# GATB/dsk

Measured on AMD Instinct MI355X. Metric: distinct k-mers counted/sec (whole node), k=31, higher is better.
Workload: dtype u64

## Files before the change

dsk_amd/csrc/dskgpu.hip:

```cpp
#include <algorithm>
#include <cstdio>
#include <cstring>
#include <cstdlib>
#include <cmath>
#include <string>
#include <vector>

#include <thread>
#include <system_error>
#include "engine.h"
#include "kernels.h"
#include "superkmer.h"
#include "rawparse.h"

#include <rocprim/device/device_radix_sort.hpp>

#define DSKGPU_VERSION "dskgpu 0.1 (gfx950)"

namespace {

thread_local std::string g_create_err;

__global__ __launch_bounds__(1024) void k_place_probe(unsigned long long* __restrict__ out, unsigned long long n) {
    const unsigned long long per_block = n / gridDim.x, per_stream = per_block / 512;
    unsigned long long* base = out + (unsigned long long)blockIdx.x * per_block;
    const int r = threadIdx.x >> 5, l = threadIdx.x & 31;
    for (unsigned long long off = 0; off + 32 <= per_stream; off += 32)
        for (int p = r; p < 512; p += 32) base[(unsigned long long)p * per_stream + off + l] = off;
}
int g_place_k = -1;
float place_probe_ms(void* p, size_t bytes) {
    hipEvent_t a, b;
    if (hipEventCreate(&a) != hipSuccess || hipEventCreate(&b) != hipSuccess) return 0.f;
    float best = 1e30f;
    for (int i = 0; i < 3; ++i) {
        (void)hipEventRecord(a, 0);
        hipLaunchKernelGGL(k_place_probe, dim3(256), dim3(1024), 0, 0, static_cast<unsigned long long*>(p), (unsigned long long)(bytes / 8));
        (void)hipEventRecord(b, 0);
        (void)hipEventSynchronize(b);
        float ms = 0.f; (void)hipEventElapsedTime(&ms, a, b);
        if (i && ms < best) best = ms;
    }
    (void)hipEventDestroy(a); (void)hipEventDestroy(b);
    return best;
}
}

hipError_t placed_malloc(void** out, size_t bytes) {
    if (g_place_k < 0) { const char* e = getenv("DSKGPU_PLACE"); g_place_k = e ? atoi(e) : 0; }
    size_t free_b = 0, total_b = 0;
    if (g_place_k < 2 || bytes < (size_t(1) << 28) || hipMemGetInfo(&free_b, &total_b) != hipSuccess) return hipMalloc(out, bytes);
    const int K = (int)std::min<size_t>((size_t)g_place_k, free_b / 2 / bytes);
    if (K < 2) return hipMalloc(out, bytes);
    std::vector<void*> cand; std::vector<float> ms;
    for (int i = 0; i < K; ++i) {
        void* q = nullptr;
        if (hipMalloc(&q, bytes) != hipSuccess) { (void)hipGetLastError(); break; }
        static const size_t probe_max = getenv("DSKGPU_PLACE_GB") ? (size_t)(atof(getenv("DSKGPU_PLACE_GB")) * (1ull << 30)) : ~size_t(0);
        cand.push_back(q); ms.push_back(place_probe_ms(q, std::min(bytes, probe_max)));
    }
    if (cand.empty()) return hipErrorOutOfMemory;
    size_t best = 0;
    for (size_t i = 1; i < cand.size(); ++i) if (ms[i] < ms[best]) best = i;
    for (size_t i = 0; i < cand.size(); ++i) if (i != best) (void)hipFree(cand[i]);
    if (getenv("DSKGPU_VERBOSE")) {
        fprintf(stderr, "[dskgpu] placement of %.2f GB: probe ms", bytes * 1e-9);
        for (size_t i = 0; i < cand.size(); ++i) fprintf(stderr, " %.3f%s", ms[i], i == best ? "*" : "");
        fprintf(stderr, "\n");
    }
    *out = cand[best];
    return hipSuccess;
}

namespace {

__global__ void k_gather_back(const u32* __restrict__ sc, const u32* __restrict__ nsolid_total, const u32* __restrict__ nk, const u64* __restrict__ gstats,
                              u64* __restrict__ out) {
    if (threadIdx.x == 0) {
        out[0] = sc[SC_OVERFLOW]; out[1] = *nsolid_total; out[2] = nk ? *nk : 0u; out[3] = sc[SC_OVF2]; out[4] = sc[SC_OVF1]; out[5] = sc[SC_EXT];
        out[6] = gstats[0]; out[7] = gstats[1]; out[8] = gstats[2]; out[9] = gstats[3];
    }
}
struct ScalarSet { u32 v[SC_COUNT]; };
__global__ __launch_bounds__(256) void k_setup_pass(u32* __restrict__ sc, ScalarSet h, u64* __restrict__ ghist, u32 nh, u64* __restrict__ gstats, u32 nstats,
                                                    u32* __restrict__ zero, u64 nzero) {
    const u32 t = blockIdx.x * 256 + threadIdx.x;
    if (t < SC_COUNT) sc[t] = h.v[t];
    if (t < nstats) gstats[t] = 0ull;
    for (u32 i = t; i < nh; i += gridDim.x * 256) ghist[i] = 0ull;
    for (u64 i = t; i < nzero; i += (u64)gridDim.x * 256) zero[i] = 0u;
}
}

namespace {

#define LAND_BYTES (64u << 10)
void* landing(dskgpu_ctx* ctx, size_t bytes) {
    if (bytes > LAND_BYTES) return nullptr;
    if (!ctx->land && hipHostMalloc(reinterpret_cast<void**>(&ctx->land), LAND_BYTES, hipHostMallocDefault) != hipSuccess) { ctx->land = nullptr; (void)hipGetLastError(); }
    return ctx->land;
}

bool sentinel_is_a_kmer(int W, unsigned k) {
    u64 v[4] = {0, 0, 0, 0};
    if (W == 1) v[0] = kunmix(~0ull);
    else if (W == 2) { KN<2> x; x.w[0] = x.w[1] = ~0ull; kunmixN(x); v[0] = x.w[0]; v[1] = x.w[1]; }
    else { KN<4> x; for (int i = 0; i < 4; ++i) x.w[i] = ~0ull; kunmixN(x); for (int i = 0; i < 4; ++i) v[i] = x.w[i]; }
    auto base = [&](const u64* a, unsigned i) { return (unsigned)((a[i >> 5] >> (2 * (i & 31))) & 3u); };
    for (unsigned i = k; i < 128; ++i) if (base(v, i)) return false;
    u64 r[4] = {0, 0, 0, 0};
    for (unsigned i = 0; i < k; ++i) { const unsigned c = base(v, i) ^ 2u, j = k - 1 - i; r[j >> 5] |= (u64)c << (2 * (j & 31)); }
    for (int x = 3; x >= 0; --x) if (v[x] != r[x]) return v[x] < r[x];
    return true;
}


int run_encode(dskgpu_ctx* ctx, const uint8_t* d_bytes, u64 n, u64* nwords_out) {
    const u64 nwords = (n + 31) / 32;
    ctx->enc_fresh = false;
    CK(ctx->packed.ensure((nwords + 1) * 8));
    CK(ctx->inval.ensure((nwords + 1) * 4));
    if (const int rc = encode_into(ctx, d_bytes, n, ctx->packed.as<u64>(), ctx->inval.as<u32>())) return rc;
    *nwords_out = nwords;
    return DSKGPU_OK;
}

int encode_current(dskgpu_ctx* ctx, u64* nwords_out) {
    if (ctx->enc_keep) { *nwords_out = (ctx->n_bytes + 31) / 32; ctx->enc_fresh = false; return DSKGPU_OK; }
    if (!ctx->d_reads && ctx->n_bytes) return fail(ctx, DSKGPU_E_STATE, "the reads were released (dskgpu_encode_reads) and their 2-bit form has been overwritten: set the reads again");
    return run_encode(ctx, ctx->d_reads, ctx->n_bytes, nwords_out);
}

}

int encode_into(dskgpu_ctx* ctx, const uint8_t* d_bytes, u64 n, u64* packed, u32* inval) {
    const u64 nwords = (n + 31) / 32;
    if (!nwords) return DSKGPU_OK;
    const u64 nb = (nwords + 255) / 256;
    const unsigned grid = (unsigned)std::min<u64>(nb, (u64)ctx->num_cu * 16);
    if ((reinterpret_cast<uintptr_t>(d_bytes) & 15) == 0)
        hipLaunchKernelGGL(k_encode<true>, dim3(grid), dim3(256), 0, ctx->stream, d_bytes, n, packed, inval, nwords);
    else
        hipLaunchKernelGGL(k_encode<false>, dim3(grid), dim3(256), 0, ctx->stream, d_bytes, n, packed, inval, nwords);
    CKL("k_encode");
    return DSKGPU_OK;
}

int run_scan(dskgpu_ctx* ctx, u32* a, const u32* d_len, u64 max_len) {
    const u64 nb = std::max<u64>(1, (max_len + SCAN_BLK - 1) / SCAN_BLK);
    CK(ctx->sums.ensure((nb + 1) * 4));
    hipLaunchKernelGGL(k_scan_reduce, dim3((unsigned)nb), dim3(SCAN_NT), 0, ctx->stream, a, d_len, ctx->sums.as<u32>());
    hipLaunchKernelGGL(k_scan_sums, dim3(1), dim3(1024), 0, ctx->stream, ctx->sums.as<u32>(), d_len, a);
    hipLaunchKernelGGL(k_scan_apply, dim3((unsigned)nb), dim3(SCAN_NT), 0, ctx->stream, a, d_len, ctx->sums.as<u32>());
    CKL("k_scan");
    return DSKGPU_OK;
}

int allow_big_lds(dskgpu_ctx* ctx, const void* fn, int bytes) {
    for (const void* f : ctx->big_lds_fns) if (f == fn) return DSKGPU_OK;
    CK(hipFuncSetAttribute(fn, hipFuncAttributeMaxDynamicSharedMemorySize, bytes));
    ctx->big_lds_fns.push_back(fn);
    return DSKGPU_OK;
}

namespace {

size_t scatter_lds(int W, u32 P, bool opt = false) { return (size_t)SC_NT * (16 / W) * 8 * W + (size_t)P * (opt ? 20 : 16) + 4 + 17 * 4 + 16 + (opt ? 8 + L0_MAX_PASSES * 8 : 0); }

template <int W, int SRC, int MODE>
int launch_hist_m(dskgpu_ctx* ctx, const typename KeyT<W>::T* keys, const ChunkDesc* descs, const u32* d_nch,
                  u64 max_chunks, u32* matrix, DigitSpec ds, u32 P) {
    const unsigned grid = (unsigned)std::max<u64>(1, std::min<u64>(max_chunks, (u64)ctx->num_cu));
    hipLaunchKernelGGL((k_hist<W, SRC, MODE>), dim3(grid), dim3(SC_NT), 0, ctx->stream, ctx->packed.as<u64>(),
                       ctx->inval.as<u32>(), keys, descs, d_nch, matrix, (int)ctx->cfg.kmer_size, ds, P);
    CKL("k_hist");
    return DSKGPU_OK;
}
template <int W, int SRC>
int launch_hist(dskgpu_ctx* ctx, const typename KeyT<W>::T* keys, const ChunkDesc* descs, const u32* d_nch,
                u64 max_chunks, u32* matrix, DigitSpec ds, u32 P) {
    const bool mp = ds.mode == 1 && ds.npass > 1;
    if (SRC == 0) return ds.mode == 0 ? launch_hist_m<W, 0, 0>(ctx, keys, descs, d_nch, max_chunks, matrix, ds, P)
                       : mp ? launch_hist_m<W, 0, 3>(ctx, keys, descs, d_nch, max_chunks, matrix, ds, P)
                            : launch_hist_m<W, 0, 1>(ctx, keys, descs, d_nch, max_chunks, matrix, ds, P);
    return ds.mode == 2 ? launch_hist_m<W, 1, 2>(ctx, keys, descs, d_nch, max_chunks, matrix, ds, P)
                   : mp ? launch_hist_m<W, 1, 3>(ctx, keys, descs, d_nch, max_chunks, matrix, ds, P)
                        : launch_hist_m<W, 1, 1>(ctx, keys, descs, d_nch, max_chunks, matrix, ds, P);
}

unsigned scatter_grid(const dskgpu_ctx* ctx, int W, u32 P, u64 max_chunks, bool opt = false) {
    const size_t lds = scatter_lds(W, P, opt);
    const u64 per_cu = std::max<u64>(1, std::min<u64>(2048 / SC_NT, (160 * 1024) / lds));
    return (unsigned)std::max<u64>(1, std::min<u64>(max_chunks, (u64)ctx->num_cu * per_cu));
}
template <int W, int SRC, int MODE, bool OPT = false, bool HEAVY = false>
int launch_scatter_m(dskgpu_ctx* ctx, const typename KeyT<W>::T* keys, const ChunkDesc* descs, const u32* d_nch,
                     u64 max_chunks, const u32* scanned, typename KeyT<W>::T* out, DigitSpec ds, u32 P, Opt1Spec o1 = Opt1Spec{nullptr, 0u, 0u, nullptr, nullptr, 0u, nullptr, nullptr, nullptr, 0u, nullptr, 0ull, {0ull, 0ull, 0ull, 0ull}, 0u}) {
    const size_t lds = scatter_lds(W, P, OPT && !o1.uslice);
    const unsigned grid = scatter_grid(ctx, W, P, max_chunks, OPT && !o1.uslice);
    { const int e = allow_big_lds(ctx, reinterpret_cast<const void*>(&k_scatter<W, SRC, MODE, OPT, HEAVY>)); if (e) return e; }
    hipLaunchKernelGGL((k_scatter<W, SRC, MODE, OPT, HEAVY>), dim3(grid), dim3(SC_NT), lds, ctx->stream, SRC == 2 ? ctx->rec_src : ctx->packed.as<u64>(),
                       SRC == 2 ? nullptr : ctx->inval.as<u32>(), keys, descs, d_nch, scanned, out, (int)ctx->cfg.kmer_size, ds, P, o1);
    CKL("k_scatter");
    return DSKGPU_OK;
}
template <int W, int MODE, bool OPT = false, bool SLICED = false>
int launch_scatter_al(dskgpu_ctx* ctx, const typename KeyT<W>::T* keys, const ChunkDesc* descs, const u32* d_nch,
                      u64 max_chunks, const u32* scanned, typename KeyT<W>::T* out, DigitSpec ds, u32 P, OptSpec os = OptSpec{0u, nullptr, nullptr, nullptr, 0u, 0u, 0ull, 0u, 0u, nullptr, nullptr, nullptr, nullptr, nullptr, nullptr}) {
    const size_t lds = ascatter_lds(W, P);
    const unsigned grid = (unsigned)std::max<u64>(1, std::min<u64>(max_chunks, (u64)ctx->num_cu));
    { const int e = allow_big_lds(ctx, reinterpret_cast<const void*>(&k_scatter_al<W, MODE, OPT, SLICED>)); if (e) return e; }
    hipLaunchKernelGGL((k_scatter_al<W, MODE, OPT, SLICED>), dim3(grid), dim3(SC_NT), lds, ctx->stream, keys, descs, d_nch, scanned, out, ds, P, os);
    CKL("k_scatter_al");
    return DSKGPU_OK;
}

template <int W, int SRC>
int launch_scatter(dskgpu_ctx* ctx, const typename KeyT<W>::T* keys, const ChunkDesc* descs, const u32* d_nch,
                   u64 max_chunks, const u32* scanned, typename KeyT<W>::T* out, DigitSpec ds, u32 P) {
    const bool mp = ds.mode == 1 && ds.npass > 1;
    if (SRC == 1 && ascatter_lds(W, P) <= 160 * 1024 && !ctx->tune.no_aligned)
        return ds.mode == 2 ? launch_scatter_al<W, 2>(ctx, keys, descs, d_nch, max_chunks, scanned, out, ds, P)
                       : mp ? launch_scatter_al<W, 3>(ctx, keys, descs, d_nch, max_chunks, scanned, out, ds, P)
                            : launch_scatter_al<W, 1>(ctx, keys, descs, d_nch, max_chunks, scanned, out, ds, P);
    if (SRC == 0) return ds.mode == 0 ? launch_scatter_m<W, 0, 0>(ctx, keys, descs, d_nch, max_chunks, scanned, out, ds, P)
                       : mp ? launch_scatter_m<W, 0, 3>(ctx, keys, descs, d_nch, max_chunks, scanned, out, ds, P)
                            : launch_scatter_m<W, 0, 1>(ctx, keys, descs, d_nch, max_chunks, scanned, out, ds, P);
    return ds.mode == 2 ? launch_scatter_m<W, 1, 2>(ctx, keys, descs, d_nch, max_chunks, scanned, out, ds, P)
                   : mp ? launch_scatter_m<W, 1, 3>(ctx, keys, descs, d_nch, max_chunks, scanned, out, ds, P)
                        : launch_scatter_m<W, 1, 1>(ctx, keys, descs, d_nch, max_chunks, scanned, out, ds, P);
}

inline void launch_count_impl(dskgpu_ctx* ctx, unsigned grid, u64* keys, u64* solid_keys, u32* solid_ab, u32* ovf, const CountParams& cp) {
    if (cp.cap && cp.cap <= CNT_V3_KEYS * CNT_NT) {
        hipLaunchKernelGGL((k_count1v3<CNT_NT, CNT_KPT, CNT_V3_KEYS>), dim3(grid), dim3(CNT_NT), 0, ctx->stream, keys, solid_keys, solid_ab,
                           ctx->nsolid.as<u32>(), ctx->ghist.as<u64>(), ctx->gstats.as<u64>(), ovf, cp, cp.subcnt);
        return;
    }
    if (cp.cap) hipLaunchKernelGGL(k_count1<true>, dim3(grid), dim3(CNT_NT), 0, ctx->stream, keys, solid_keys, ctx->fstart.as<u32>(), solid_ab,
                                   ctx->nsolid.as<u32>(), ctx->ghist.as<u64>(), ctx->gstats.as<u64>(), ovf, cp, cp.subcnt);
    else hipLaunchKernelGGL(k_count1<false>, dim3(grid), dim3(CNT_NT), 0, ctx->stream, keys, solid_keys, ctx->fstart.as<u32>(), solid_ab,
                            ctx->nsolid.as<u32>(), ctx->ghist.as<u64>(), ctx->gstats.as<u64>(), ovf, cp, (const u32*)ctx->fstart.as<u32>());
}
template <int W>
inline void launch_count_impl(dskgpu_ctx* ctx, unsigned grid, KN<W>* keys, KN<W>* solid_keys, u32* solid_ab, u32* ovf, const CountParams& cp) {
    if constexpr (W == 2) {
        if (cp.cap && cp.cap <= C2V_NKEYS * CNT_NT && !ctx->mw_v3_off) {
            CountParams c2 = cp; c2.maxload = std::min<u32>(cp.maxload, C2V_MAXLOAD);
            hipLaunchKernelGGL((k_count2v3<CNT_NT, C2V_KPT, C2V_NKEYS>), dim3(grid), dim3(CNT_NT), 0, ctx->stream, (const K2*)keys, solid_keys, solid_ab,
                               ctx->nsolid.as<u32>(), ctx->ghist.as<u64>(), ctx->gstats.as<u64>(), ovf, c2, cp.subcnt);
            return;
        }
    }
    if (cp.cap) hipLaunchKernelGGL((k_count_mw<W, true>), dim3(grid), dim3(CNT_NT), 0, ctx->stream, keys, solid_keys, ctx->fstart.as<u32>(), solid_ab,
                                   ctx->nsolid.as<u32>(), ctx->ghist.as<u64>(), ctx->gstats.as<u64>(), ovf, cp);
    else hipLaunchKernelGGL((k_count_mw<W, false>), dim3(grid), dim3(CNT_NT), 0, ctx->stream, keys, solid_keys, ctx->fstart.as<u32>(), solid_ab,
                            ctx->nsolid.as<u32>(), ctx->ghist.as<u64>(), ctx->gstats.as<u64>(), ovf, cp);
}
template <int W>
inline void launch_count(dskgpu_ctx* ctx, unsigned grid, typename KeyT<W>::T* keys, typename KeyT<W>::T* solid_keys, u32* solid_ab, u32* ovf, const CountParams& cp) {
    launch_count_impl(ctx, grid, keys, solid_keys, solid_ab, ovf, cp);
}

struct Plan {
    int levels;
    u32 P1, P2, F;
    DigitSpec d1, d2;
};

#define TARGET_KEYS 2900
#define TARGET_KEYS2 2560
#ifndef TARGET_KEYS4
#define TARGET_KEYS4 640
#endif
#ifndef OPT_GROUPS4
#define OPT_GROUPS4 OPT_GROUPS
#endif
#define MAX_LEVEL_BINS 2048
#define ONE_LEVEL_BINS 1024
#define CH2 65536u
#define OPT_GROUPS 545u
#define OPT_GROUPS2 1023u
inline u32 opt_groups(int W) { return W == 2 ? (AL_G2 == 8 ? 1022u : OPT_GROUPS2) : (W == 1 && AL_G1 == 16) ? 546u : W == 4 ? OPT_GROUPS4 : OPT_GROUPS; }
inline u64 target_keys(int W) { return W == 1 ? TARGET_KEYS : W == 2 ? TARGET_KEYS2 : TARGET_KEYS4; }
#define OPT_CAP 4360u

bool make_plan(u64 n_upper, int extra_bits, int W, u32 num_cu, Plan* pl) {
    const u64 target = target_keys(W);
    u64 F = ((n_upper + target - 1) / target) << extra_bits;
    if (F < 2) F = 2;
    if (F <= ONE_LEVEL_BINS) { pl->levels = 1; pl->P1 = (u32)F; pl->P2 = 1; }
    else {
        u64 p2max = MAX_LEVEL_BINS; while (p2max > 64 && ascatter_lds(W, (u32)p2max) > 160 * 1024) --p2max;
        u64 p1 = 1; while (p1 * p1 < F) ++p1;
        const bool large = F >= (u64)num_cu * 64;
        if (large) {
            p1 = std::max<u64>((F + p2max - 2) / (p2max - 1), num_cu);
            p1 = (p1 + num_cu - 1) / num_cu * num_cu;
            if (p1 > MAX_LEVEL_BINS - 8) p1 = MAX_LEVEL_BINS - 8;
        }
        u64 p2 = (F + p1 - 1) / p1;
        if (p2 % 2 == 0 && p2 + 1 <= p2max) ++p2;
        if (p1 > MAX_LEVEL_BINS || p2 > MAX_LEVEL_BINS) return false;
        pl->levels = 2; pl->P1 = (u32)p1; pl->P2 = (u32)p2;
    }
    pl->F = pl->P1 * pl->P2;
    pl->d1 = DigitSpec{1u, pl->P1, 0u, 1u, 1u, 0u};
    pl->d2 = DigitSpec{2u, pl->P1, pl->P2, 1u, 1u, 0u};
    return true;
}

void build_descs1(dskgpu_ctx* ctx, u64 n_units_total, u64 tile, u64 max_chunks, u32* nch_out) {
    const u64 ntiles = std::max<u64>(1, (n_units_total + tile - 1) / tile);
    u64 nch = std::min<u64>(ntiles, max_chunks);
    const u64 tpc = (ntiles + nch - 1) / nch;
    nch = (ntiles + tpc - 1) / tpc;
    ctx->h_descs1.resize(nch);
    for (u64 c = 0; c < nch; ++c) {
        ChunkDesc d;
        d.begin = c * tpc * tile;
        d.end = std::min<u64>(n_units_total, (c + 1) * tpc * tile);
        if (d.begin > d.end) d.begin = d.end;
        d.flat_base = (u32)c;
        d.stride = (u32)nch;
        ctx->h_descs1[c] = d;
    }
    *nch_out = (u32)nch;
}

void build_descs1_slices(dskgpu_ctx* ctx, u64 tile, u64 max_chunks, u32* nch_out) {
    const size_t S = ctx->rec_slice_end.size();
    ctx->h_descs1.clear(); ctx->h_slice_chunk.assign(S + 1, 0);
    const u64 per_slice = std::max<u64>(1, max_chunks / S);
    u64 rb = 0;
    for (size_t sl = 0; sl < S; ++sl) {
        const u64 re = ctx->rec_slice_end[sl];
        ctx->h_slice_chunk[sl] = (u32)ctx->h_descs1.size();
        if (re > rb) {
            const u64 ntiles = (re - rb + tile - 1) / tile;
            u64 nch = std::min<u64>(ntiles, per_slice);
            const u64 tpc = (ntiles + nch - 1) / nch;
            nch = (ntiles + tpc - 1) / tpc;
            for (u64 c = 0; c < nch; ++c) {
                ChunkDesc d;
                d.begin = rb + c * tpc * tile; d.end = std::min<u64>(re, rb + (c + 1) * tpc * tile);
                d.flat_base = 0; d.stride = 0;
                ctx->h_descs1.push_back(d);
            }
        }
        rb = re;
    }
    ctx->h_slice_chunk[S] = (u32)ctx->h_descs1.size();
    for (auto& d : ctx->h_descs1) d.stride = (u32)ctx->h_descs1.size();
    *nch_out = (u32)ctx->h_descs1.size();
}

#define REC_RESIZE 1001
int rec_gate_upto(dskgpu_ctx* ctx, u32 upto) {
    if (!ctx->rec_gate) return DSKGPU_OK;
    const u32 n = (u32)ctx->rec_slice_end.size();
    for (; ctx->rec_gated < std::min(upto, n); ++ctx->rec_gated)
        if (ctx->rec_gate(ctx->rec_gate_user, ctx->rec_gated) != 0) ctx->rec_gate_failed = true;
    return ctx->rec_gate_failed ? fail(ctx, DSKGPU_E_STATE, "a slice of the exchange did not arrive (the caller's gate failed)") : DSKGPU_OK;
}
int rec_gate_all(dskgpu_ctx* ctx) { return rec_gate_upto(ctx, 0xFFFFFFFFu); }

int sk_sizes(dskgpu_ctx* ctx, u64* total_out) {
    const u64 nrec = ctx->rec_n; const u32 R = ctx->sk_sp.R;
    { const int e = rec_gate_all(ctx); if (e) return e; }
    u64 nch = std::min<u64>((nrec + SKX_NT - 1) / SKX_NT, (u64)ctx->num_cu * 16);
    u64 rpc = (nrec + nch - 1) / nch;
    rpc = (rpc + SKX_NT - 1) / SKX_NT * SKX_NT;
    nch = (nrec + rpc - 1) / rpc;
    if (rpc * SK_MAXN >= 0xFFFFFFFFull) return fail(ctx, DSKGPU_E_ARG, "too many records per chunk");
    CK(ctx->sk_sums.ensure(nch * 4)); CK(ctx->sk_cbase.ensure(nch * 8));
    ctx->h_sk_sums.assign(nch, 0); ctx->h_sk_cbase.assign(nch, 0);
    hipLaunchKernelGGL(k_sk_count, dim3((unsigned)nch), dim3(SKX_NT), 0, ctx->stream, ctx->rec_src, nrec, R, (u32)rpc, ctx->sk_sums.as<u32>());
    CKL("k_sk_count");
    CK(hipMemcpyAsync(ctx->h_sk_sums.data(), ctx->sk_sums.p, nch * 4, hipMemcpyDeviceToHost, ctx->stream));
    CK(hipStreamSynchronize(ctx->stream));
    u64 total = 0;
    for (u64 c = 0; c < nch; ++c) { ctx->h_sk_cbase[c] = total; total += ctx->h_sk_sums[c]; }
    CK(hipMemcpyAsync(ctx->sk_cbase.p, ctx->h_sk_cbase.data(), nch * 8, hipMemcpyHostToDevice, ctx->stream));
    ctx->rec_nch = nch; ctx->rec_rpc = rpc; ctx->rec_sized = true;
    *total_out = total;
    return DSKGPU_OK;
}

template <int W>
int expand_records(dskgpu_ctx* ctx, u64 total) {
    typedef typename KeyT<W>::T Key;
    if (ctx->rec_expanded) return DSKGPU_OK;
    if (!ctx->rec_sized) {
        u64 real = 0;
        const int e = sk_sizes(ctx, &real);
        if (e) return e;
        if (real != total && ctx->rec_hint_est) { ctx->rec_hint = real; return REC_RESIZE; }
        if (real != total) return fail(ctx, DSKGPU_E_ARG, "dskgpu_mg_count_sized: n_kmers does not match the k-mers inside the records");
    }
    { const int e = rec_gate_all(ctx); if (e) return e; }
    CK(ctx->sk_keys.ensure((total + 1) * sizeof(Key)));
    hipLaunchKernelGGL(k_sk_expand<W>, dim3((unsigned)ctx->rec_nch), dim3(SKX_NT), 0, ctx->stream, ctx->rec_src, ctx->rec_n, ctx->sk_sp.R,
                       (int)ctx->cfg.kmer_size, (u32)ctx->rec_rpc, ctx->sk_cbase.as<u64>(), ctx->sk_keys.as<Key>());
    CKL("k_sk_expand");
    ctx->rec_expanded = true;
    ctx->mark("mg_expand");
    return DSKGPU_OK;
}
template <> int expand_records<4>(dskgpu_ctx*, u64) { return DSKGPU_E_STATE; }

template <int W> struct HvLayout { static constexpr size_t keys = 0, counts = (size_t)HV_KEYS * W, rows = (size_t)HV_KEYS * (W + 1), ab = (size_t)HV_KEYS * (2 * W + 1), words = (size_t)HV_KEYS * (2 * W + 2); };
template <int W>
int find_heavy(dskgpu_ctx* ctx, bool from_reads, const typename KeyT<W>::T* d_keys_in, u32 nts, const Plan& pl, std::vector<double>& load, u32* nheavy_out) {
    typedef typename KeyT<W>::T Key;
    struct HK { u64 w[W]; bool operator<(const HK& o) const { for (int x = W - 1; x >= 0; --x) if (w[x] != o.w[x]) return w[x] < o.w[x]; return false; }
                bool operator==(const HK& o) const { for (int x = 0; x < W; ++x) if (w[x] != o.w[x]) return false; return true; } };
    static_assert(sizeof(HK) == sizeof(Key), "host mirror of a device key");
    *nheavy_out = 0;
    const u32 P1 = pl.P1;
    std::vector<double> sorted(load);
    std::nth_element(sorted.begin(), sorted.begin() + P1 / 2, sorted.end());
    const double median = sorted[P1 / 2];
    std::vector<u32> flagged;
    for (u32 b = 0; b < P1; ++b) if (load[b] > 1.2 * median + 4096.0) flagged.push_back(b);
    if (ctx->tune.verbose) fprintf(stderr, "[dskgpu] find_heavy: median load %.0f, %zu bins above 1.2 x\n", median, flagged.size());
    if (flagged.empty()) return DSKGPU_OK;
    std::sort(flagged.begin(), flagged.end(), [&](u32 a, u32 b) { return load[a] > load[b]; });
    if (flagged.size() > HV_SLOTS) flagged.resize(HV_SLOTS);
    ctx->h_hv_lut.assign(P1, 0xFF);
    for (size_t f = 0; f < flagged.size(); ++f) ctx->h_hv_lut[flagged[f]] = (unsigned char)f;
    const size_t nf = flagged.size();
    CK(ctx->hv_lut.ensure(P1));
    const unsigned grid = (unsigned)std::min<u64>(nts, (u64)ctx->num_cu * 2);
    const size_t per_slot = (size_t)grid * HV_BLOCK_KEYS;
    CK(ctx->hv_collect.ensure((size_t)HV_SLOTS * per_slot * sizeof(Key) + (size_t)HV_SLOTS * grid * 4 + HV_SLOTS * 4));
    u32* d_kept = reinterpret_cast<u32*>(ctx->hv_collect.as<Key>() + (size_t)HV_SLOTS * per_slot);
    u32* d_step = d_kept + (size_t)HV_SLOTS * grid;
    ctx->h_hv_step.assign(HV_SLOTS, 1);
    for (size_t f = 0; f < flagged.size(); ++f) ctx->h_hv_step[f] = (u32)std::max<u64>(1, ctx->h_mom[2 * (size_t)flagged[f]] / HV_COLLECT);
    CK(hipMemcpyAsync(ctx->hv_lut.p, ctx->h_hv_lut.data(), P1, hipMemcpyHostToDevice, ctx->stream));
    CK(hipMemcpyAsync(d_step, ctx->h_hv_step.data(), HV_SLOTS * 4, hipMemcpyHostToDevice, ctx->stream));
    u32* sc = ctx->scalars.as<u32>();
    const bool mp = pl.d1.npass > 1;
    auto launch = [&](auto kern) {
        hipLaunchKernelGGL(kern, dim3(grid), dim3(SC_NT), 0, ctx->stream, (const u64*)ctx->packed.as<u64>(), (const u32*)ctx->inval.as<u32>(), d_keys_in,
                           (const ChunkDesc*)ctx->smp_descs.as<ChunkDesc>(), (const u32*)(sc + SC_NCH_S), (int)ctx->cfg.kmer_size, pl.d1, P1,
                           (const unsigned char*)ctx->hv_lut.as<unsigned char>(), d_kept, ctx->hv_collect.as<Key>(), (const u32*)d_step);
    };
    if (from_reads) { if (mp) launch(k_collect_heavy<W, 0, 3>); else launch(k_collect_heavy<W, 0, 1>); }
    else { if (mp) launch(k_collect_heavy<W, 1, 3>); else launch(k_collect_heavy<W, 1, 1>); }
    CKL("k_collect_heavy");
    ctx->h_hv_cnt.resize(nf * grid);
    ctx->h_hv_coll.resize(nf * per_slot * W);
    CK(hipMemcpyAsync(ctx->h_hv_cnt.data(), d_kept, nf * grid * 4, hipMemcpyDeviceToHost, ctx->stream));
    CK(hipMemcpyAsync(ctx->h_hv_coll.data(), ctx->hv_collect.p, nf * per_slot * sizeof(Key), hipMemcpyDeviceToHost, ctx->stream));
    CK(hipStreamSynchronize(ctx->stream));
    struct Cand { double est; HK key; u32 bin; };
    std::vector<Cand> cands;
    for (size_t f = 0; f < nf; ++f) {
        HK* kk = reinterpret_cast<HK*>(ctx->h_hv_coll.data()) + f * per_slot;
        u32 n = 0;
        for (unsigned g = 0; g < grid; ++g) {
            const u32 c = std::min<u32>(ctx->h_hv_cnt[f * grid + g], HV_BLOCK_KEYS);
            for (u32 i = 0; i < c; ++i) kk[n++] = kk[(size_t)g * HV_BLOCK_KEYS + i];
        }
        if (n < 256) continue;
        std::sort(kk, kk + n);
        const u32 bin = flagged[f];
        u32 found = 0;
        for (u32 i = 0; i < n;) {
            u32 j = i + 1;
            while (j < n && kk[j] == kk[i]) ++j;
            if ((u64)(j - i) * 20 >= n) { cands.push_back({load[bin] * (double)(j - i) / (double)n, kk[i], bin}); ++found; }
            i = j;
        }
        if (ctx->tune.verbose) fprintf(stderr, "[dskgpu]   bin %u load %.0f: %u keys collected, %u dominant\n", bin, load[bin], n, found);
    }
    std::sort(cands.begin(), cands.end(), [](const Cand& a, const Cand& b) { return a.est > b.est; });
    if (cands.size() > HV_KEYS) cands.resize(HV_KEYS);
    ctx->h_hv_keys.assign((size_t)HV_KEYS * W, DSK_EMPTY);
    for (size_t x = 0; x < cands.size(); ++x) {
        for (int y = 0; y < W; ++y) ctx->h_hv_keys[x * W + y] = cands[x].key.w[y];
        load[cands[x].bin] -= cands[x].est;
    }
    u32 nheavy = (u32)cands.size();
    if (nheavy) {
        CK(ctx->hv_buf.ensure(HvLayout<W>::words * 8));
        u64* hvb = ctx->hv_buf.as<u64>();
        CK(hipMemsetAsync(hvb + HvLayout<W>::keys, 0xFF, (size_t)HV_KEYS * W * 8, ctx->stream));
        CK(hipMemsetAsync(hvb + HvLayout<W>::counts, 0, HV_KEYS * 8, ctx->stream));
        CK(hipMemcpyAsync(hvb + HvLayout<W>::keys, ctx->h_hv_keys.data(), (size_t)HV_KEYS * W * 8, hipMemcpyHostToDevice, ctx->stream));
    }
    *nheavy_out = nheavy;
    return DSKGPU_OK;
}

template <int W> struct KeySource { bool from_reads, from_rec; const typename KeyT<W>::T* keys; u64 nkeys, nwords; };

template <int W>
struct PassState {
    typedef typename KeyT<W>::T Key;
    KeySource<W>& src;
    u32 pass, npass; u64 cap;
    u64 nvalid;
    u32* sc;
    Plan pl{};
    u32 opt_cap = 0, max_ext = 0; u64 nregions = 0;
    bool opt1 = false; Opt1Spec o1{}; unsigned grid1 = 0;
    u32 nch1 = 0, nheavy = 0;
    std::vector<double> load, spread;
    Key* fkeys = nullptr;
    DevBuf* scratch = nullptr;
    Key* solid_keys = nullptr; u32* solid_ab = nullptr;
    u32 flags = 0, nsolid = 0, nkeys = 0, ovf2 = 0, ovf1 = 0, ext = 0; u64 stats[4] = {0, 0, 0, 0};
    bool too_big = false; u64 rows = 0;
};

template <int W>
int upload_descs1(dskgpu_ctx* ctx, PassState<W>& ps) {
    const KeySource<W>& src = ps.src;
    const u64 max_chunks1 = (u64)ctx->num_cu * 8;
    if (src.from_reads) build_descs1(ctx, src.nwords, Tile<W>::WORDS, max_chunks1, &ps.nch1);
    else if (src.from_rec && ctx->rec_slice_end.size() > 1) build_descs1_slices(ctx, RecTile<W>::NR, max_chunks1, &ps.nch1);
    else if (src.from_rec) build_descs1(ctx, ctx->rec_n, RecTile<W>::NR, max_chunks1, &ps.nch1);
    else build_descs1(ctx, src.nkeys, Tile<W>::KEYS, max_chunks1, &ps.nch1);
    CK(ctx->descs1.ensure(ctx->h_descs1.size() * sizeof(ChunkDesc)));
    CK(hipMemcpyAsync(ctx->descs1.p, ctx->h_descs1.data(), ctx->h_descs1.size() * sizeof(ChunkDesc), hipMemcpyHostToDevice, ctx->stream));
    return DSKGPU_OK;
}

template <int W>
int records_to_keys(dskgpu_ctx* ctx, PassState<W>& ps) {
    const int e = expand_records<W>(ctx, ps.src.nkeys);
    if (e) return e;
    ps.src.keys = ctx->sk_keys.template as<typename KeyT<W>::T>(); ps.src.from_rec = false;
    return upload_descs1(ctx, ps);
}

template <class Hist>
int positional_sample(dskgpu_ctx* ctx, u64 units, u64 tile, u32 P, Hist&& hist, u64* ntiles_out, u64* nts_out, u64* stot_out) {
    u32* sc = ctx->scalars.as<u32>();
    const u64 ntiles = std::max<u64>(1, (units + tile - 1) / tile);
    const u64 nts = std::min<u64>(ntiles, 1024);
    ctx->h_descs_s.resize(nts);
    for (u64 i = 0; i < nts; ++i) {
        const u64 t = i * ntiles / nts;
        ChunkDesc d; d.begin = t * tile; d.end = std::min<u64>(units, (t + 1) * tile); d.flat_base = (u32)i; d.stride = (u32)nts;
        ctx->h_descs_s[i] = d;
    }
    const u64 Ms = (u64)P * nts;
    CK(ctx->smp_descs.ensure(nts * sizeof(ChunkDesc)));
    CK(ctx->smp_mat.ensure((Ms + 4) * 4 + (size_t)P * 16));
    CK(hipMemcpyAsync(ctx->smp_descs.p, ctx->h_descs_s.data(), nts * sizeof(ChunkDesc), hipMemcpyHostToDevice, ctx->stream));
    ctx->h_sc[SC_NCH_S] = (u32)nts;
    CK(hipMemcpyAsync(sc + SC_NCH_S, &ctx->h_sc[SC_NCH_S], 4, hipMemcpyHostToDevice, ctx->stream));
    { const int e = hist(ctx->smp_descs.as<ChunkDesc>(), (const u32*)(sc + SC_NCH_S), nts, ctx->smp_mat.as<u32>()); if (e) return e; }
    u64* mom = reinterpret_cast<u64*>(ctx->smp_mat.as<u32>() + ((Ms + 2) & ~(u64)1));
    hipLaunchKernelGGL(k_bin_moments, dim3((P + 3) / 4), dim3(256), 0, ctx->stream, (const u32*)ctx->smp_mat.as<u32>(), (u32)nts, P, mom);
    CKL("k_bin_moments");
    ctx->h_mom.resize((size_t)P * 2);
    void* lz = landing(ctx, (size_t)P * 16);
    CK(hipMemcpyAsync(lz ? lz : (void*)ctx->h_mom.data(), mom, (size_t)P * 16, hipMemcpyDeviceToHost, ctx->stream));
    CK(hipStreamSynchronize(ctx->stream));
    if (lz) std::memcpy(ctx->h_mom.data(), lz, (size_t)P * 16);
    u64 stot = 0;
    for (u32 b = 0; b < P; ++b) stot += ctx->h_mom[2 * b];
    *ntiles_out = ntiles; *nts_out = nts; *stot_out = stot;
    return DSKGPU_OK;
}

template <int W>
int pass_plan(dskgpu_ctx* ctx, PassState<W>& ps, int extra_bits) {
    typedef typename KeyT<W>::T Key;
    Plan& pl = ps.pl;
    const u64 plan_n = (ps.src.from_reads && ctx->have_nvalid) ? std::min<u64>(ps.cap, ps.npass == 1 ? ps.nvalid + 1 : ps.nvalid / ps.npass + ps.nvalid / ps.npass / 50 + 4096) : ps.cap;
    if (!make_plan(plan_n, extra_bits, W, (u32)ctx->num_cu, &pl))
        return fail(ctx, DSKGPU_E_OVERFLOW, "cannot partition finer (table overflow persists)");
    pl.d1.world = pl.d2.world = ctx->cfg.world_size; pl.d1.npass = pl.d2.npass = ps.npass; pl.d1.pass = pl.d2.pass = ps.pass;
    { const int e = upload_descs1(ctx, ps); if (e) return e; }
    if (pl.levels == 2 && ctx->sentinel_ok && !ctx->opt2_off && !ctx->tune.no_opt2 && ascatter_lds(W, pl.P2) <= 160 * 1024)
        ps.opt_cap = opt_groups(W) * (8u / W);
    if (ps.opt_cap && ctx->tune.opt_cap) ps.opt_cap = ctx->tune.opt_cap;
    if (W > 1 && (u64)pl.F * ps.opt_cap >= 0xFFFF0000ull) ps.opt_cap = 0;
    const u32 opt_cap = ps.opt_cap;
    if (opt_cap && W <= 2) {
        u64 want = std::min<u64>((u64)pl.F / 8 + 4096, 0x7FFFFFFFull / opt_cap - 1);
        if (ctx->tune.max_ext >= 0) want = (u64)ctx->tune.max_ext;
        if (W > 1) { const u64 room = 0xFFFF0000ull / opt_cap; want = room > (u64)pl.F + 1 ? std::min<u64>(want, room - pl.F - 1) : 0; }
        ps.max_ext = (u32)want;
    }
    ps.nregions = (u64)pl.F + ps.max_ext;
    if (!opt_cap) { CK(ctx->bufA.ensure((ps.cap + 1) * sizeof(Key))); CK(ctx->bufB.ensure((ps.cap + 1) * sizeof(Key))); }
    if (opt_cap) {
        const u64 slots = (u64)pl.F * opt_cap + ATile<W>::KEYS + 16;
        CK(ctx->bufA.ensure(std::max<u64>(W == 1 ? slots * 4 : slots * sizeof(Key), (ps.cap + 1) * sizeof(Key))));
        if (W > 1) CK(ctx->abund2.ensure(slots * 4));
    }
    ps.opt1 = opt_cap && !ctx->opt1_off && !ctx->tune.no_opt1 && (ps.npass == 1 || ps.src.from_reads || W <= 2);
    if (ps.src.from_rec && (!ps.opt1 || W > 2 || ctx->tune.no_recsrc)) { const int e = records_to_keys(ctx, ps); if (e) return e; }
    if (ps.opt1 && scatter_lds(W, pl.P1, false) > 160 * 1024) ps.opt1 = false;
    return DSKGPU_OK;
}

template <int W>
int pass_layout1(dskgpu_ctx* ctx, PassState<W>& ps) {
    typedef typename KeyT<W>::T Key;
    const KeySource<W>& src = ps.src;
    const Plan& pl = ps.pl;
    Opt1Spec& o1 = ps.o1;
    o1 = Opt1Spec{nullptr, 0u, 0u, ps.sc + SC_OVF1, nullptr, ctx->sk_sp.R, ctx->gstats.as<u64>() + 2, nullptr, nullptr, 0u, nullptr, 0ull, {0ull, 0ull, 0ull, 0ull}, 0u};
    const bool uniform1 = scatter_lds(W, pl.P1, true) > 160 * 1024;
    if (ps.opt1) {
        const u32 nch1 = ps.nch1;
        const unsigned grid1 = ps.grid1 = scatter_grid(ctx, W, pl.P1, nch1, !uniform1);
        const u64 cpb = (nch1 + grid1 - 1) / grid1;
        double share = (double)cpb / (double)nch1;
        if (src.from_rec && ctx->rec_slice_end.size() > 1) {
            share = 0.0;
            u64 rb = 0;
            for (size_t sl = 0; sl < ctx->rec_slice_end.size(); ++sl) {
                const u64 re = ctx->rec_slice_end[sl], nc = ctx->h_slice_chunk[sl + 1] - ctx->h_slice_chunk[sl];
                if (nc) share += (double)((nc + grid1 - 1) / grid1) / (double)nc * (double)(re - rb) / (double)ctx->rec_n;
                rb = re;
            }
        }
        const double pass_keys = (double)(ps.nvalid / ps.npass);
        ps.load.assign(pl.P1, pass_keys / pl.P1);
        ps.spread.assign(pl.P1, 0.0);
        bool sampled = false;
        const Key* d_keys_s = src.keys;
        double smp_density = 1.0;
        bool rec_sample_ok = ctx->sentinel_ok;
        u64 rec_units = 0;
        if constexpr (W <= 2) {
          if (src.from_rec && !ctx->tune.no_sample && !uniform1) {
            const u64 nrec_s = ctx->rec_slice_end.size() > 1 ? ctx->rec_slice_end[0] : ctx->rec_n;
            const u64 NR = RecTile<W>::NR;
            const u64 nchk_all = (nrec_s + NR - 1) / NR;
            const u64 nchk = std::min<u64>(nchk_all, 256);
            if (nchk == 0) rec_sample_ok = false;
            else {
                { const int e = rec_gate_upto(ctx, 1); if (e) return e; }
                std::vector<u64>& cbeg = ctx->h_cbeg;
                cbeg.resize(nchk);
                for (u64 i = 0; i < nchk; ++i) cbeg[i] = (i * nchk_all / nchk) * NR;
                rec_units = nchk * NR * SK_MAXN;
                CK(ctx->smp_keys.ensure(rec_units * sizeof(Key) + nchk * 8 + 64));
                u64* d_cbeg = reinterpret_cast<u64*>(ctx->smp_keys.as<char>() + rec_units * sizeof(Key));
                CK(hipMemcpyAsync(d_cbeg, cbeg.data(), nchk * 8, hipMemcpyHostToDevice, ctx->stream));
                hipLaunchKernelGGL(k_sk_sample_keys<W>, dim3((unsigned)nchk), dim3(SKX_NT), 0, ctx->stream, ctx->rec_src, ctx->rec_n, ctx->sk_sp.R, (int)ctx->cfg.kmer_size,
                                   (const u64*)d_cbeg, (u32)NR, ctx->smp_keys.as<Key>());
                CKL("k_sk_sample_keys");
                d_keys_s = ctx->smp_keys.as<Key>();
            }
          }
        }
        const bool smp_rec = src.from_rec && rec_units != 0;
        if ((!src.from_rec || smp_rec) && rec_sample_ok && !ctx->tune.no_sample && !uniform1) {
            const u64 units = src.from_reads ? src.nwords : smp_rec ? rec_units : src.nkeys, tile = src.from_reads ? Tile<W>::WORDS : Tile<W>::KEYS;
            auto hist = [&](const ChunkDesc* dd, const u32* d_nch, u64 n, u32* mat) {
                return src.from_reads ? launch_hist<W, 0>(ctx, nullptr, dd, d_nch, n, mat, pl.d1, pl.P1) : launch_hist<W, 1>(ctx, d_keys_s, dd, d_nch, n, mat, pl.d1, pl.P1);
            };
            u64 ntiles = 0, nts = 0, stot = 0;
            { const int e = positional_sample(ctx, units, tile, pl.P1, hist, &ntiles, &nts, &stot); if (e) return e; }
            if (stot >= (u64)pl.P1 * 64) {
                const double scale = (src.from_reads && ps.npass > 1) ? (double)ntiles / (double)nts : pass_keys / (double)stot;
                if (smp_rec) smp_density = std::max(0.05, (double)stot / ((double)nts * (double)Tile<W>::KEYS));
                const double tiles_per_block = smp_rec ? pass_keys * share / (double)Tile<W>::KEYS : (double)ntiles * share;
                for (u32 b = 0; b < pl.P1; ++b) {
                    const double sum = (double)ctx->h_mom[2 * b], sq = (double)ctx->h_mom[2 * b + 1];
                    const double mean = sum / (double)nts, var = std::max(mean, sq / (double)nts - mean * mean);
                    ps.load[b] = sum * scale;
                    ps.spread[b] = 5.0 * std::sqrt(tiles_per_block * var / smp_density) + 4.0 * std::sqrt((double)nts * var) * scale * share;
                }
                sampled = true;
            }
            if constexpr (W <= 2) {
                if (sampled && ps.opt_cap && !ctx->tune.no_heavy) { const int e = find_heavy<W>(ctx, src.from_reads, d_keys_s, (u32)nts, pl, ps.load, &ps.nheavy); if (e) return e; }
            }
            ctx->mark("sample1");
        }
        ctx->h_boff.resize(pl.P1 + 1);
        u64 area = 0;
        if (uniform1) o1.uslice = 1u;
        for (u32 b = 0; b < pl.P1; ++b) {
            double sl = ps.load[b] * share;
            const double few = (src.from_rec && share * (double)nch1 < 16.0) ? 0.08 : 0.0;
            sl += sampled ? ps.spread[b] + sl * 0.01 + 64.0 : sl * (0.06 + few) + 160.0;
            u64 slice = ((u64)sl + 8) & ~7ull;
            if (uniform1) o1.uslice = (u32)slice;
            if (ctx->tune.opt_slice) slice = ctx->tune.opt_slice;
            ctx->h_boff[b] = (u32)std::min<u64>(area, 0xFFFFFFFFull); area += slice;
        }
        ctx->h_boff[pl.P1] = (u32)std::min<u64>(area, 0xFFFFFFFFull);
        const u64 tail = 2 * Tile<W>::KEYS;
        const u64 cells = (u64)pl.P1 * grid1;
        if (ctx->tune.verbose) fprintf(stderr, "[dskgpu] pass %u/%u: P1 %u P2 %u, %u level-1 blocks, area %llu keys per block (%.2f GB of slices), sampled %d, keys %llu, %u chunks, share %.6f, %zu slices\n", ps.pass, ps.npass, pl.P1, pl.P2, grid1,
                                       (unsigned long long)area, (double)area * grid1 * sizeof(Key) * 1e-9, (int)sampled, (unsigned long long)ps.nvalid, nch1, share, ctx->rec_slice_end.size());
        if (area < 8 || area * grid1 + tail >= 0xFFFF0000ull) ps.opt1 = false;
        else {
            o1.area = (u32)area; o1.dump = (u32)(area * grid1);
            CK(ctx->boff.ensure(((size_t)pl.P1 + 1) * 4));
            CK(hipMemcpyAsync(ctx->boff.p, ctx->h_boff.data(), ((size_t)pl.P1 + 1) * 4, hipMemcpyHostToDevice, ctx->stream));
            o1.boff = ctx->boff.as<u32>();
            CK(ctx->mat1.ensure((cells + 1) * 4));
            o1.fill = ctx->mat1.as<u32>();
            if (grid1 + 1 > SLICED_MAX) ps.opt1 = false;
            CK(ctx->bufA.ensure((area * grid1 + tail + 1) * sizeof(Key)));
        }
    }
    if (src.from_rec && !ps.opt1) { const int e = records_to_keys(ctx, ps); if (e) return e; }
    return DSKGPU_OK;
}

template <int W, int SRC, int MODE, bool HEAVY>
int scatter1_m(dskgpu_ctx* ctx, const PassState<W>& ps, const ChunkDesc* dd1, const u32* d_nch) {
    return launch_scatter_m<W, SRC, MODE, true, HEAVY>(ctx, SRC == 1 ? ps.src.keys : nullptr, dd1, d_nch, ps.nch1, nullptr, ctx->bufA.template as<typename KeyT<W>::T>(),
                                                       ps.pl.d1, ps.pl.P1, ps.o1);
}
template <int W>
int launch_scatter1(dskgpu_ctx* ctx, const PassState<W>& ps, const ChunkDesc* dd1, const u32* d_nch) {
    const bool mp = ps.npass > 1, heavy = ps.nheavy != 0, rec = ps.src.from_rec, reads = ps.src.from_reads;
    if constexpr (W <= 2) {
        if (rec && heavy) return mp ? scatter1_m<W, 2, 3, true>(ctx, ps, dd1, d_nch) : scatter1_m<W, 2, 1, true>(ctx, ps, dd1, d_nch);
        if (rec) return mp ? scatter1_m<W, 2, 3, false>(ctx, ps, dd1, d_nch) : scatter1_m<W, 2, 1, false>(ctx, ps, dd1, d_nch);
        if (heavy && reads) return mp ? scatter1_m<W, 0, 3, true>(ctx, ps, dd1, d_nch) : scatter1_m<W, 0, 1, true>(ctx, ps, dd1, d_nch);
        if (heavy) return mp ? scatter1_m<W, 1, 3, true>(ctx, ps, dd1, d_nch) : scatter1_m<W, 1, 1, true>(ctx, ps, dd1, d_nch);
        if (!reads && mp) return scatter1_m<W, 1, 3, false>(ctx, ps, dd1, d_nch);
    } else if (rec || heavy || (!reads && mp)) return DSKGPU_E_STATE;
    if (reads) return mp ? scatter1_m<W, 0, 3, false>(ctx, ps, dd1, d_nch) : scatter1_m<W, 0, 1, false>(ctx, ps, dd1, d_nch);
    return scatter1_m<W, 1, 1, false>(ctx, ps, dd1, d_nch);
}

template <int W>
int pass_scatter1(dskgpu_ctx* ctx, PassState<W>& ps) {
    typedef typename KeyT<W>::T Key;
    const KeySource<W>& src = ps.src;
    const Plan& pl = ps.pl;
    const u32 nch1 = ps.nch1;
    const u64 M1 = (u64)pl.P1 * nch1;
    u32* h_sc = ctx->h_sc;
    std::memset(h_sc, 0, sizeof(ctx->h_sc));
    h_sc[SC_NCH1] = nch1; h_sc[SC_MLEN1] = (u32)M1; h_sc[SC_F] = pl.F;
    if (ps.opt1) h_sc[SC_NCH2] = pl.P1;
    h_sc[SC_WORK2] = (u32)std::min<u64>(pl.P1, (u64)ctx->num_cu);
    {
        static_assert(sizeof(ctx->h_sc) == sizeof(ScalarSet), "scalar block");
        ScalarSet hs; std::memcpy(hs.v, h_sc, sizeof hs.v);
        const u32 nh = ctx->cfg.histo_max + 1;
        u64 nzero = 0;
        if (pl.levels == 2 && ps.opt_cap) { nzero = ps.nregions + 1; CK(ctx->mat2.ensure((size_t)nzero * 4)); }
        const u64 work = std::max<u64>(nh, nzero);
        hipLaunchKernelGGL(k_setup_pass, dim3((unsigned)std::min<u64>(1024, (work + 255) / 256)), dim3(256), 0, ctx->stream, ps.sc, hs, ctx->ghist.as<u64>(), nh, ctx->gstats.as<u64>(), 4u,
                           nzero ? ctx->mat2.as<u32>() : (u32*)nullptr, nzero);
        CKL("k_setup_pass");
    }
    ctx->mark("setup");
    int rc;
    const ChunkDesc* dd1 = ctx->descs1.as<ChunkDesc>();
    if (ps.opt1) {
        Opt1Spec& o1 = ps.o1;
        if constexpr (W <= 2) { if (ps.nheavy) { o1.hv_keys = ctx->hv_buf.as<u64>() + HvLayout<W>::keys; o1.hv_cnt = reinterpret_cast<unsigned long long*>(ctx->hv_buf.as<u64>() + HvLayout<W>::counts); } }
        if (src.from_rec && ctx->rec_slice_end.size() > 1) {
            const size_t S = ctx->rec_slice_end.size();
            CK(ctx->cur_state.ensure((size_t)ps.grid1 * pl.P1 * 4));
            o1.cur_state = ctx->cur_state.as<u32>();
            rc = DSKGPU_OK;
            for (size_t sl = 0; sl < S && rc == DSKGPU_OK; ++sl) {
                if ((rc = rec_gate_upto(ctx, (u32)sl + 1))) break;
                o1.g0 = ctx->h_slice_chunk[sl]; o1.gn = ctx->h_slice_chunk[sl + 1] - ctx->h_slice_chunk[sl];
                o1.resume = sl > 0 ? 1u : 0u; o1.last = sl + 1 == S ? 1u : 0u;
                rc = launch_scatter1<W>(ctx, ps, dd1, ps.sc + SC_NCH1);
            }
        }
        else if (src.from_rec) { if (!(rc = rec_gate_all(ctx))) rc = launch_scatter1<W>(ctx, ps, dd1, ps.sc + SC_NCH1); }
        else rc = launch_scatter1<W>(ctx, ps, dd1, ps.sc + SC_NCH1);
        if (rc) return rc;
        ctx->mark("scatter1");
        return DSKGPU_OK;
    }
    CK(ctx->mat1.ensure((M1 + 1) * 4));
    if (src.from_reads) rc = launch_hist<W, 0>(ctx, nullptr, dd1, ps.sc + SC_NCH1, nch1, ctx->mat1.as<u32>(), pl.d1, pl.P1);
    else rc = launch_hist<W, 1>(ctx, src.keys, dd1, ps.sc + SC_NCH1, nch1, ctx->mat1.as<u32>(), pl.d1, pl.P1);
    if (rc) return rc;
    ctx->mark("hist1");
    if ((rc = run_scan(ctx, ctx->mat1.as<u32>(), ps.sc + SC_MLEN1, M1))) return rc;
    ctx->mark("scan1");
    if (ps.npass > 1) {
        CK(hipMemcpyAsync(&ps.nkeys, ctx->mat1.as<u32>() + M1, 4, hipMemcpyDeviceToHost, ctx->stream));
        CK(hipStreamSynchronize(ctx->stream));
        if ((u64)ps.nkeys > ps.cap) { ps.too_big = true; return DSKGPU_OK; }
    }
    if (src.from_reads) rc = launch_scatter<W, 0>(ctx, nullptr, dd1, ps.sc + SC_NCH1, nch1, ctx->mat1.as<u32>(), ctx->bufA.as<Key>(), pl.d1, pl.P1);
    else rc = launch_scatter<W, 1>(ctx, src.keys, dd1, ps.sc + SC_NCH1, nch1, ctx->mat1.as<u32>(), ctx->bufA.as<Key>(), pl.d1, pl.P1);
    if (rc) return rc;
    ctx->mark("scatter1");
    return DSKGPU_OK;
}

template <int W>
int pass_scatter2(dskgpu_ctx* ctx, PassState<W>& ps) {
    const Plan& pl = ps.pl;
    int rc;
    ps.fkeys = ctx->bufA.as<typename KeyT<W>::T>();
    ps.scratch = &ctx->bufB;
    CK(ctx->fstart.ensure(((size_t)pl.F + 2) * 4));
    CK(ctx->nsolid.ensure(((size_t)pl.F + 2) * 4));
    if (pl.levels == 2 && ps.opt_cap) {
        CK(ctx->bufB.ensure((ps.nregions * ps.opt_cap + ATile<W>::KEYS + 16) * sizeof(typename KeyT<W>::T)));
        CK(ctx->descs2.ensure(((size_t)pl.P1 * 2 + 1) * sizeof(ChunkDesc)));
        CK(ctx->seg.ensure((size_t)pl.P1 * sizeof(SegInfo)));
        CK(ctx->mat2.ensure(((size_t)ps.nregions + 1) * 4));
        CK(ctx->chain_next.ensure(((size_t)ps.nregions + 1 + ps.max_ext + 1) * 4));
        if (ps.opt1) {
            ctx->h_descs2.resize(pl.P1);
            std::vector<u32> order(pl.P1);
            for (u32 sgm = 0; sgm < pl.P1; ++sgm) order[sgm] = sgm;
            double mean_work = 0.0; for (double w : ps.load) mean_work += w; mean_work = std::max(1.0, mean_work / pl.P1);
            auto wclass = [&](u32 a) { return (long long)(ps.load[a] / (0.05 * mean_work)); };
            std::stable_sort(order.begin(), order.end(), [&](u32 a, u32 b) { return wclass(a) > wclass(b); });
            for (u32 i = 0; i < pl.P1; ++i) {
                const u32 sgm = order[i];
                ChunkDesc d; d.begin = ctx->h_boff[sgm]; d.end = ctx->h_boff[sgm + 1]; d.flat_base = sgm * pl.P2; d.stride = 1;
                ctx->h_descs2[i] = d;
            }
            CK(hipMemcpyAsync(ctx->descs2.p, ctx->h_descs2.data(), (size_t)pl.P1 * sizeof(ChunkDesc), hipMemcpyHostToDevice, ctx->stream));
        } else {
            hipLaunchKernelGGL(k_plan, dim3(1), dim3(1024), 0, ctx->stream, ctx->mat1.as<u32>(), ps.nch1, pl.P1, 0x7FFFFFFFu, pl.P2,
                               ctx->seg.as<SegInfo>(), ctx->descs2.as<ChunkDesc>(), ps.sc + SC_NCH2, ps.sc + SC_MLEN2, 1u);
            CKL("k_plan");
        }
        ctx->mark("plan2");
        OptSpec os{ps.opt_cap, ctx->mat2.as<u32>(), ps.sc + SC_OVF2, ps.opt1 ? ps.o1.fill : nullptr, 0u, ps.grid1, (u64)ps.o1.area,
                   pl.F, ps.max_ext, ctx->chain_next.as<u32>(), ps.sc + SC_EXT, ctx->chain_next.as<u32>() + ps.nregions + 1, ps.sc + SC_NCHAINED,
                   ps.sc + SC_WORK2, nullptr};
        if (ctx->tune.verbose && ps.opt1) { CK(ctx->dbg.ensure((size_t)pl.P1 * 24)); os.dbg = ctx->dbg.as<unsigned long long>(); }
        if (ps.opt1) rc = launch_scatter_al<W, 2, true, true>(ctx, ctx->bufA.as<typename KeyT<W>::T>(), ctx->descs2.as<ChunkDesc>(), ps.sc + SC_NCH2, (u64)pl.P1 * 2, nullptr,
                                                              ctx->bufB.as<typename KeyT<W>::T>(), pl.d2, pl.P2, os);
        else rc = launch_scatter_al<W, 2, true, false>(ctx, ctx->bufA.as<typename KeyT<W>::T>(), ctx->descs2.as<ChunkDesc>(), ps.sc + SC_NCH2, (u64)pl.P1 * 2, nullptr,
                                                       ctx->bufB.as<typename KeyT<W>::T>(), pl.d2, pl.P2, os);
        if (rc) return rc;
        ctx->mark("scatter2");
        if (ctx->tune.verbose && ps.opt1) {
            std::vector<unsigned long long> t((size_t)pl.P1 * 3);
            CK(hipMemcpyAsync(t.data(), ctx->dbg.p, t.size() * 8, hipMemcpyDeviceToHost, ctx->stream));
            CK(hipStreamSynchronize(ctx->stream));
            unsigned long long t0 = ~0ull, t1 = 0; for (u32 i = 0; i < pl.P1; ++i) { t0 = std::min(t0, t[3 * i]); t1 = std::max(t1, t[3 * i + 1]); }
            fprintf(stderr, "[dskgpu] level 2: %u segments, %.3f ms first start -> last end\n", pl.P1, (t1 - t0) * 1e-5);
            for (u32 i = 0; i < pl.P1; ++i)
                if (i < 6 || i + 3 >= pl.P1 || t[3 * i + 1] + 20000 > t1)
                    fprintf(stderr, "[dskgpu]   desc %u (segment %u, load %.0f) block %llu: %.3f .. %.3f ms\n", i, (u32)(ctx->h_descs2[i].flat_base / pl.P2),
                            ps.load[ctx->h_descs2[i].flat_base / pl.P2], t[3 * i + 2], (t[3 * i] - t0) * 1e-5, (t[3 * i + 1] - t0) * 1e-5);
        }
        ps.fkeys = ctx->bufB.as<typename KeyT<W>::T>();
        ps.scratch = &ctx->bufA;
    } else if (pl.levels == 2) {
        const u64 max_chunks2 = ps.cap / CH2 + pl.P1 + 1;
        const u64 M2 = max_chunks2 * pl.P2;
        if (M2 >= 0xFFFFFFFFull) return fail(ctx, DSKGPU_E_ARG, "level-2 matrix too large");
        CK(ctx->descs2.ensure(max_chunks2 * sizeof(ChunkDesc)));
        CK(ctx->seg.ensure((size_t)pl.P1 * sizeof(SegInfo)));
        CK(ctx->mat2.ensure((M2 + 1) * 4));
        hipLaunchKernelGGL(k_plan, dim3(1), dim3(1024), 0, ctx->stream, ctx->mat1.as<u32>(), ps.nch1, pl.P1, CH2, pl.P2,
                           ctx->seg.as<SegInfo>(), ctx->descs2.as<ChunkDesc>(), ps.sc + SC_NCH2, ps.sc + SC_MLEN2, 0u);
        CKL("k_plan");
        ctx->mark("plan2");
        const ChunkDesc* dd2 = ctx->descs2.as<ChunkDesc>();
        if ((rc = launch_hist<W, 1>(ctx, ctx->bufA.as<typename KeyT<W>::T>(), dd2, ps.sc + SC_NCH2, max_chunks2, ctx->mat2.as<u32>(), pl.d2, pl.P2))) return rc;
        ctx->mark("hist2");
        if ((rc = run_scan(ctx, ctx->mat2.as<u32>(), ps.sc + SC_MLEN2, M2))) return rc;
        ctx->mark("scan2");
        if ((rc = launch_scatter<W, 1>(ctx, ctx->bufA.as<typename KeyT<W>::T>(), dd2, ps.sc + SC_NCH2, max_chunks2, ctx->mat2.as<u32>(), ctx->bufB.as<typename KeyT<W>::T>(), pl.d2, pl.P2))) return rc;
        ctx->mark("scatter2");
        ps.fkeys = ctx->bufB.as<typename KeyT<W>::T>();
        ps.scratch = &ctx->bufA;
        hipLaunchKernelGGL(k_final_offsets, dim3((pl.F + 256) / 256), dim3(256), 0, ctx->stream, ctx->mat2.as<u32>(),
                           ctx->seg.as<SegInfo>(), pl.P2, 0u, ps.sc + SC_MLEN2, ctx->fstart.as<u32>(), pl.F);
    } else {
        hipLaunchKernelGGL(k_final_offsets, dim3((pl.F + 256) / 256), dim3(256), 0, ctx->stream, ctx->mat1.as<u32>(),
                           (const SegInfo*)nullptr, pl.P1, ps.nch1, ps.sc + SC_MLEN1, ctx->fstart.as<u32>(), pl.F);
    }
    CKL("k_final_offsets");
    ctx->mark("offsets");
    return DSKGPU_OK;
}

template <int W>
int count_and_sizes(dskgpu_ctx* ctx, PassState<W>& ps, const CountParams& cp) {
    typedef typename KeyT<W>::T Key;
    const Plan& pl = ps.pl;
    const unsigned cgrid = (unsigned)std::min<u64>(pl.F, (u64)ctx->num_cu * 2);
    launch_count<W>(ctx, cgrid, ps.fkeys, ps.solid_keys, ps.solid_ab, ps.sc + SC_OVERFLOW, cp);
    CKL("k_count");
    if constexpr (W <= 2) {
        if (ps.opt_cap && ps.max_ext) {
            auto kern = [] { if constexpr (W == 1) return k_count_chained; else return k_count_chained_mw<2>; }();
            hipLaunchKernelGGL(kern, dim3((unsigned)std::min<u64>(ps.max_ext, (u64)ctx->num_cu * 2)), dim3(CNT_NT), 0, ctx->stream, ps.fkeys, ps.solid_keys, ps.solid_ab,
                               ctx->nsolid.as<u32>(), ctx->ghist.as<u64>(), ctx->gstats.as<u64>(), ps.sc + SC_OVERFLOW, cp, (const u32*)cp.subcnt,
                               (const u32*)ctx->chain_next.as<u32>(), (const u32*)(ctx->chain_next.as<u32>() + ps.nregions + 1), (const u32*)(ps.sc + SC_NCHAINED), ps.max_ext);
            CKL(W == 1 ? "k_count_chained" : "k_count_chained_mw");
        }
        if (ps.nheavy) {
            const u32 slots = HV_KEYS;
            u64* hvb = ctx->hv_buf.as<u64>();
            hipLaunchKernelGGL(k_heavy_rows<W>, dim3((slots + 255) / 256), dim3(256), 0, ctx->stream, reinterpret_cast<const Key*>(hvb + HvLayout<W>::keys),
                               (const unsigned long long*)(hvb + HvLayout<W>::counts), slots, cp.amin, cp.amax, cp.histo_max, ctx->ghist.as<u64>(), ctx->gstats.as<u64>(),
                               hvb + HvLayout<W>::rows, reinterpret_cast<u32*>(hvb + HvLayout<W>::ab));
            CKL("k_heavy_rows");
        }
    }
    ctx->mark("count");
    if (int e = run_scan(ctx, ctx->nsolid.as<u32>(), ps.sc + SC_F, pl.F)) return e;
    ctx->mark("scan_solid");
    CK(ctx->back_dev.ensure(16 * 8));
    if (!ctx->back_host) CK(hipHostMalloc(reinterpret_cast<void**>(&ctx->back_host), 16 * 8, hipHostMallocDefault));
    const u32* nkp = ps.opt1 ? nullptr : (ps.opt_cap ? ctx->mat1.as<u32>() + (u64)pl.P1 * ps.nch1 : ctx->fstart.as<u32>() + pl.F);
    hipLaunchKernelGGL(k_gather_back, dim3(1), dim3(64), 0, ctx->stream, (const u32*)ps.sc, (const u32*)(ctx->nsolid.as<u32>() + pl.F), nkp,
                       (const u64*)ctx->gstats.as<u64>(), ctx->back_dev.as<u64>());
    CKL("k_gather_back");
    CK(hipMemcpyAsync(ctx->back_host, ctx->back_dev.p, 10 * 8, hipMemcpyDeviceToHost, ctx->stream));
    CK(hipStreamSynchronize(ctx->stream));
    const u64* bh = ctx->back_host;
    ps.flags = (u32)bh[0]; ps.nsolid = (u32)bh[1]; if (!ps.opt1) ps.nkeys = (u32)bh[2];
    ps.ovf2 = (u32)bh[3]; ps.ovf1 = (u32)bh[4]; ps.ext = (u32)bh[5];
    for (int x = 0; x < 4; ++x) ps.stats[x] = bh[6 + x];
    return DSKGPU_OK;
}

template <int W>
int pass_count(dskgpu_ctx* ctx, PassState<W>& ps) {
    CountParams cp;
    cp.F = ps.pl.F;
    cp.maxload = W == 1 ? CNT_MAXLOAD : C2_MAXLOAD;
    if (ctx->tune.table_maxload) cp.maxload = std::min<u32>(cp.maxload, ctx->tune.table_maxload);
    cp.amin = ctx->cfg.abundance_min; cp.amax = ctx->cfg.abundance_max; cp.histo_max = ctx->cfg.histo_max;
    cp.cap = ps.opt_cap; cp.subcnt = ps.opt_cap ? ctx->mat2.as<u32>() : nullptr;
    ps.solid_keys = W == 1 ? ps.fkeys : ps.scratch->template as<typename KeyT<W>::T>();
    ps.solid_ab = W == 1 ? ps.scratch->template as<u32>() : ctx->abund2.as<u32>();
    if constexpr (W == 2) CK(hipMemcpyAsync(ctx->gstats.as<u64>() + 3, ctx->gstats.as<u64>() + 2, 8, hipMemcpyDeviceToDevice, ctx->stream));
    if (int e = count_and_sizes<W>(ctx, ps, cp)) return e;
    if constexpr (W == 2) {
        if ((ps.flags & (CNT_OVF_VERIFY | CNT_OVF_SENTINEL)) && !((ps.opt_cap && ps.ovf2) || (ps.opt1 && ps.ovf1))) {
            if (ctx->tune.verbose) fprintf(stderr, "[dskgpu] pass %u/%u: the top-word table met k-mers it cannot tell apart (flags %u): counting again with k_count_mw\n", ps.pass, ps.npass, ps.flags);
            ctx->mw_v3_off = true;
            ctx->stats.n_retries += 1;
            CK(hipMemsetAsync(ctx->ghist.p, 0, ((size_t)ctx->cfg.histo_max + 1) * 8, ctx->stream));
            CK(hipMemsetAsync(ctx->gstats.p, 0, 2 * 8, ctx->stream));
            CK(hipMemcpyAsync(ctx->gstats.as<u64>() + 2, ctx->gstats.as<u64>() + 3, 8, hipMemcpyDeviceToDevice, ctx->stream));
            CK(hipMemsetAsync(ps.sc + SC_OVERFLOW, 0, 4, ctx->stream));
            if (int e = count_and_sizes<W>(ctx, ps, cp)) return e;
        }
    }
    if (ps.opt1) ps.nkeys = (u32)ps.stats[2];
    return DSKGPU_OK;
}

template <int W>
SparseRows sparse_rows(dskgpu_ctx* ctx, const PassState<W>& ps, const RowsOut& ro, const u32* rows_ab, u32 n_tail) {
    SparseRows r;
    r.W = W; r.keys = ps.solid_keys; r.ab = (const u32*)ps.solid_ab; r.soff = ctx->nsolid.as<u32>(); r.fstart = ctx->fstart.as<u32>(); r.cap = ps.opt_cap; r.F = ps.pl.F;
    r.n_sparse = ps.nsolid; r.n_tail = W <= 2 ? n_tail : 0u;
    if (r.n_tail) { for (int x = 0; x < W; ++x) r.tail_w.w[x] = ro.w[x] + r.n_sparse; r.tail_ab = rows_ab + r.n_sparse; }
    return r;
}

template <int W>
int pass_rows(dskgpu_ctx* ctx, PassState<W>& ps) {
    typedef typename KeyT<W>::T Key;
    const Plan& pl = ps.pl;
    const u32 h_nsolid = ps.nsolid;
    const u64 nhs = ps.nheavy ? ps.stats[1] : 0;
    const u64 ns = ps.rows = h_nsolid + nhs;
    const bool to_sink = ctx->sink.active && ctx->sink.rows + ns + 1 <= ctx->sink.cap;
    RowsOut ro{};
    u32* rows_ab = nullptr;
    if (to_sink) {
        rows_ab = ctx->sink.ab + ctx->sink.rows;
        for (int x = 0; x < W; ++x) ro.w[x] = ctx->sink.w[x] + ctx->sink.rows;
        ctx->sink.took = true;
    } else {
        CK(ctx->out_ab.ensure((ns + 1) * 4));
        rows_ab = ctx->out_ab.as<u32>();
        for (int x = 0; x < W; ++x) { CK(ctx->out_w[x].ensure((ns + 1) * 8)); ro.w[x] = ctx->out_w[x].as<u64>(); }
    }
    if constexpr (W <= 2) {
      if (nhs) {
        for (int x = 0; x < W; ++x)
            CK(hipMemcpyAsync(ro.w[x] + h_nsolid, ctx->hv_buf.as<u64>() + HvLayout<W>::rows + (size_t)x * HV_KEYS, nhs * 8, hipMemcpyDeviceToDevice, ctx->stream));
        CK(hipMemcpyAsync(rows_ab + h_nsolid, ctx->hv_buf.as<u64>() + HvLayout<W>::ab, nhs * 4, hipMemcpyDeviceToDevice, ctx->stream));
      }
    }
    ctx->stats.n_heavy += ps.nheavy;
    bool sparse_sort = false;
    if constexpr (W <= 2) {
        sparse_sort = ps.npass == 1 && ctx->job_passes == 1 && ns > 0 && ns <= rs_max_rows(ctx) && !(ctx->cfg.flags & DSKGPU_F_NO_SORT) &&
                      !ctx->tune.rs_slab_rows && !ctx->bank_job.active && (W == 1 || 2u * ctx->cfg.kmer_size > 64u);
    } else {
        sparse_sort = (ctx->cfg.flags & DSKGPU_F_PARTITION_ORDER) && ps.npass == 1 && ctx->job_passes == 1 && ns > 0 && ns < 0xFFFF0000ull &&
                      !(ctx->cfg.flags & DSKGPU_F_NO_SORT) && !ctx->tune.rs_slab_rows && !ctx->bank_job.active;
    }
    if (sparse_sort) ctx->sp_rows = sparse_rows<W>(ctx, ps, ro, rows_ab, (u32)nhs);
    PartPasses& mp = ctx->rs.mp;
    bool mp_part = false;
    {
        mp_part = !sparse_sort && ctx->job_passes > 1 && mp.ok && ns > 0 && h_nsolid < 0xFFFF0000ull && (W == 1 || 2u * ctx->cfg.kmer_size > 64u);
        if (!sparse_sort && ctx->job_passes > 1 && ns > 0 && !mp_part) mp.ok = false;
        if (mp_part) {
            const SparseRows rows = sparse_rows<W>(ctx, ps, ro, rows_ab, (u32)nhs);
            if (mp.part_off.ensure_keep(((size_t)mp.off_used + part_sort_nparts(rows) + 2) * 4, (size_t)mp.off_used * 4, ctx->stream)) return fail(ctx, DSKGPU_E_NOMEM, "partition offsets");
            u32 np = 0;
            if (const int prc = launch_part_sort(ctx, rows, ro, rows_ab, mp.part_off.as<u32>() + mp.off_used, mp.flag.as<u32>(), &np)) return prc;
            mp.passes.push_back(PartPasses::Pass{mp.row_base, np, mp.off_used});
            mp.off_used += np + 1;
        }
    }
    if (!sparse_sort && !mp_part) {
        hipLaunchKernelGGL(k_compact<W>, dim3((pl.F + 3) / 4), dim3(256), 0, ctx->stream, (const Key*)ps.solid_keys, (const u32*)ps.solid_ab,
                           ctx->fstart.as<u32>(), ctx->nsolid.as<u32>(), pl.F, ro, rows_ab, ps.opt_cap);
        CKL("k_compact");
    }
    ctx->mark("compact");
    ctx->stats.n_ext_regions += std::min<u32>(ps.ext, ps.max_ext);
    return DSKGPU_OK;
}

struct PassResult { u64 rows = 0, kmers = 0, distinct = 0, keys_seen = 0; Plan plan{}; bool too_big = false; };

template <int W>
int run_one_pass(dskgpu_ctx* ctx, bool from_reads, const typename KeyT<W>::T* d_keys_in, u64 nkeys_in, u64 nwords,
                 u32 pass, u32 npass, u64 cap, PassResult* res) {
    ctx->take_sparse_rows();
    KeySource<W> src{from_reads, !from_reads && d_keys_in == nullptr, d_keys_in, nkeys_in, nwords};
    const u64 nvalid = from_reads ? ctx->h_nvalid : nkeys_in;
    int extra_bits = 0, table_retries = 0;
    for (;;) {
        PassState<W> ps{src, pass, npass, cap, nvalid, ctx->scalars.as<u32>()};
        int e;
        if ((e = pass_plan<W>(ctx, ps, extra_bits)) || (e = pass_layout1<W>(ctx, ps)) || (e = pass_scatter1<W>(ctx, ps))) return e;
        if (ps.too_big) { ctx->resolve_marks(); res->too_big = true; res->keys_seen = ps.nkeys; return DSKGPU_OK; }
        if ((e = pass_scatter2<W>(ctx, ps)) || (e = pass_count<W>(ctx, ps))) return e;
        const bool ovf1 = ps.opt1 && ps.ovf1, ovf2 = ps.opt_cap && ps.ovf2;
        if (ovf1 || ovf2) {
            ctx->resolve_marks();
            if (ctx->tune.verbose) fprintf(stderr, "[dskgpu] pass %u/%u: %s overflowed: the exact path takes over\n", pass, npass, ovf1 ? "a level-1 slice" : "the level-2 extension pool");
            if (ovf1) ctx->opt1_off = true;
            else { ctx->opt2_off = true; ctx->opt1_off = true; }
            ctx->stats.n_retries += 1;
            ctx->mark("start");
            continue;
        }
        if (ps.flags & 1u) {
            ctx->resolve_marks();
            if (table_retries >= 3) return fail(ctx, DSKGPU_E_OVERFLOW, "hash table overflow after 3 retries");
            ++table_retries; extra_bits += 1;
            ctx->stats.n_retries += 1;
            ctx->mark("start");
            continue;
        }
        if ((e = pass_rows<W>(ctx, ps))) return e;
        res->rows = ps.rows; res->kmers = res->keys_seen = ps.nkeys; res->distinct = ps.stats[0]; res->plan = ps.pl;
        return DSKGPU_OK;
    }
}

int level0_materialise(dskgpu_ctx* ctx, u64 nwords, u32 lo, u32 npass, u64 reserve_bytes, u32* G_out, u64 (&region_keys)[L0_MAX_PASSES], u64 (&obase)[L0_MAX_PASSES]) {
    *G_out = 0;
    const u64 nper = ctx->h_nvalid / npass + 1;
    u32 nch1 = 0;
    build_descs1(ctx, nwords, Tile<1>::WORDS, (u64)ctx->num_cu * 8, &nch1);
    const unsigned grid = (unsigned)std::max<u64>(1, std::min<u64>(nch1, (u64)ctx->num_cu));
    const u64 cpb = (nch1 + grid - 1) / grid;
    const double share = (double)cpb / (double)nch1;
    const u64 tail = 2 * Tile<1>::KEYS;
    const u64 uslice = (((u64)((double)nper * share * 1.02) + 4096) + 7) & ~7ull;
    const u64 uregion = uslice * grid + tail;
    if (uregion >= 0xFFFF0000ull) return DSKGPU_OK;
    size_t free_b = 0, total_b = 0;
    CK(hipMemGetInfo(&free_b, &total_b));
    const u64 have = ctx->bufA.cap + ctx->bufB.cap + ctx->l0buf.cap;
    const u64 need = nper * 30ull + (4ull << 30) + reserve_bytes;
    const u64 room = free_b + have > need ? free_b + have - need : 0;
    u32 G = (u32)std::min<u64>(std::min<u64>(L0_MAX_PASSES, npass - lo), room / (uregion * 8));
    if (ctx->tune.l0_passes) G = std::min<u32>(std::min<u32>(ctx->tune.l0_passes, L0_MAX_PASSES), npass - lo);
    if (G < 2 && !(ctx->tune.l0_passes)) return DSKGPU_OK;
    if (G == 0) return DSKGPU_OK;
    CK(ctx->descs1.ensure(ctx->h_descs1.size() * sizeof(ChunkDesc)));
    CK(hipMemcpyAsync(ctx->descs1.p, ctx->h_descs1.data(), ctx->h_descs1.size() * sizeof(ChunkDesc), hipMemcpyHostToDevice, ctx->stream));
    u32* sc = ctx->scalars.as<u32>();
    DigitSpec ds{4u, G, 0u, ctx->cfg.world_size, npass, lo};
    std::vector<u64> slice(G, uslice);
    if (!ctx->tune.no_sample) {
        auto hist = [&](const ChunkDesc* dd, const u32* d_nch, u64 n, u32* mat) { return launch_hist_m<1, 0, 4>(ctx, nullptr, dd, d_nch, n, mat, ds, G); };
        u64 ntiles = 0, nts = 0, stot = 0;
        { const int e = positional_sample(ctx, nwords, Tile<1>::WORDS, G, hist, &ntiles, &nts, &stot); if (e) return e; }
        if (stot >= (u64)G * 4096) {
            const double scale = (double)ntiles / (double)nts, tiles_per_block = (double)ntiles * share;
            for (u32 b = 0; b < G; ++b) {
                const double sum = (double)ctx->h_mom[2 * b], sq = (double)ctx->h_mom[2 * b + 1];
                const double mean = sum / (double)nts, var = std::max(mean, sq / (double)nts - mean * mean);
                const double sl = sum * scale * share * 1.01 + 5.0 * std::sqrt(tiles_per_block * var) + 4.0 * std::sqrt((double)nts * var) * scale * share + 64.0;
                slice[b] = ((u64)sl + 8) & ~7ull;
            }
        }
        ctx->mark("sample0");
    }
    for (;;) {
        u64 tot = 0; bool ok = true;
        for (u32 b = 0; b < G; ++b) { const u64 region = slice[b] * grid + tail; if (region >= 0xFFFF0000ull) ok = false; obase[b] = tot; region_keys[b] = slice[b] * grid; tot += region; }
        if (ok && (tot * 8 <= room || ctx->tune.l0_passes)) { CK(ctx->l0buf.ensure(tot * 8 + 64)); break; }
        if (--G < 2) return DSKGPU_OK;
    }
    ds.pa = G;
    ctx->h_sc[SC_NCH1] = nch1; ctx->h_sc[SC_OVF1] = 0;
    CK(hipMemcpyAsync(sc + SC_NCH1, &ctx->h_sc[SC_NCH1], 4, hipMemcpyHostToDevice, ctx->stream));
    CK(hipMemsetAsync(sc + SC_OVF1, 0, 4, ctx->stream));
    ctx->h_boff.assign(L0_MAX_PASSES + 1 + 3 + 2 * L0_MAX_PASSES, 0);
    u64 hob[L0_MAX_PASSES];
    for (u32 i = 0; i < L0_MAX_PASSES; ++i) { ctx->h_boff[i] = (u32)slice[std::min(i, G - 1)]; hob[i] = obase[std::min(i, G - 1)]; }
    std::memcpy(&ctx->h_boff[L0_MAX_PASSES + 4], hob, sizeof hob);
    CK(ctx->boff.ensure(ctx->h_boff.size() * 4));
    CK(hipMemcpyAsync(ctx->boff.p, ctx->h_boff.data(), ctx->h_boff.size() * 4, hipMemcpyHostToDevice, ctx->stream));
    const u32* d_slen = ctx->boff.as<u32>();
    const u64* d_obase = reinterpret_cast<const u64*>(ctx->boff.as<u32>() + L0_MAX_PASSES + 4);
    hipLaunchKernelGGL(k_level0, dim3(grid), dim3(SC_NT), 0, ctx->stream, (const u64*)ctx->packed.as<u64>(), (const u32*)ctx->inval.as<u32>(), (const ChunkDesc*)ctx->descs1.as<ChunkDesc>(),
                       (const u32*)(sc + SC_NCH1), ctx->l0buf.as<u64>(), (int)ctx->cfg.kmer_size, ds, G, d_slen, d_obase, sc + SC_OVF1);
    CKL("k_level0");
    ctx->mark("level0");
    CK(hipMemcpyAsync(&ctx->h_ovf1, sc + SC_OVF1, 4, hipMemcpyDeviceToHost, ctx->stream));
    CK(hipStreamSynchronize(ctx->stream));
    if (ctx->tune.verbose) {
        u64 tot = 0; for (u32 b = 0; b < G; ++b) tot += region_keys[b];
        fprintf(stderr, "[dskgpu] level 0: passes %u..%u of %u materialised, %.2f GB in all (%.2f GB free before)%s\n", lo, lo + G - 1, npass, (double)tot * 8e-9, (double)free_b * 1e-9,
                ctx->h_ovf1 ? " -- a slice overflowed: these passes read the reads" : "");
    }
    if (ctx->h_ovf1) return DSKGPU_OK;
    *G_out = G;
    return DSKGPU_OK;
}

void sk_geometry(dskgpu_ctx* ctx, u64 nwords);
#define SK_DISPATCH(ctx_, SP_, CALL) do { \
        if (!(ctx_)->tune.sk_generic && (SP_).k == 31 && (SP_).m == 10) { CALL(31, 10); } \
        else if (!(ctx_)->tune.sk_generic && (SP_).k == 63 && (SP_).m == 10) { CALL(63, 10); } \
        else { CALL(0, 0); } } while (0)
int upload_table(dskgpu_ctx* ctx);
struct RecL0 { u32 G = 0; u64 nch = 0; u32 slice[SK_MAX_OWNERS] = {0}; u64 region[SK_MAX_OWNERS] = {0}; };
#define REC_L0_NO 2001

int rec_l0_prepare(dskgpu_ctx* ctx, u64 nwords, u32 G, RecL0* rl) {
    SkParams& sp = ctx->sk_sp;
    sk_geometry(ctx, nwords);
    sp.G = G; sp.olo = 0; sp.ohi = G; sp.oslice = nullptr; sp.obase = nullptr;
    const u64 nch = sp.nchunks, tpc = sp.tiles_per_chunk;
    const u32 step = tpc >= 16 ? 16u : 1u;
    {
        SkParams ss = sp; ss.sample_step = step; ss.table = nullptr;
        CK(ctx->sk_load.ensure((size_t)SK_BUCKETS * 8));
        CK(hipMemsetAsync(ctx->sk_load.p, 0, (size_t)SK_BUCKETS * 8, ctx->stream));
#define SK_CALL(K_, M_) hipLaunchKernelGGL((k_sk_sample<K_, M_>), dim3(ss.nchunks), dim3(SK_NT), 0, ctx->stream, ctx->packed.as<u64>(), ctx->inval.as<u32>(), ss, ctx->sk_load.as<unsigned long long>())
        SK_DISPATCH(ctx, ss, SK_CALL);
#undef SK_CALL
        CKL("k_sk_sample");
        std::vector<uint64_t> loads(SK_BUCKETS);
        CK(hipMemcpyAsync(loads.data(), ctx->sk_load.p, (size_t)SK_BUCKETS * 8, hipMemcpyDeviceToHost, ctx->stream));
        CK(hipStreamSynchronize(ctx->stream));
        ctx->h_table.resize(SK_BUCKETS);
        dskgpu_mg_make_table(loads.data(), G, ctx->h_table.data());
        ctx->table_dirty = true;
        const int rc = upload_table(ctx);
        if (rc) return rc;
    }
    const u64 M = (u64)G * nch;
    CK(ctx->mat1.ensure((M + 1) * 4));
    CK(ctx->sk_sent.ensure(3 * SK_MAX_OWNERS * 8));
    CK(hipMemsetAsync(ctx->sk_sent.as<u64>() + SK_MAX_OWNERS, 0, SK_MAX_OWNERS * 8, ctx->stream));
    sp.sample_step = step;
#define SK_CALL(K_, M_) hipLaunchKernelGGL((k_sk_hist<K_, M_>), dim3((unsigned)nch), dim3(SK_NT), 0, ctx->stream, ctx->packed.as<u64>(), ctx->inval.as<u32>(), sp, ctx->mat1.as<u32>(), \
                                          ctx->sk_sent.as<unsigned long long>() + SK_MAX_OWNERS)
    SK_DISPATCH(ctx, sp, SK_CALL);
#undef SK_CALL
    CKL("k_sk_hist");
    std::vector<u32> cells(M);
    CK(hipMemcpyAsync(cells.data(), ctx->mat1.p, M * 4, hipMemcpyDeviceToHost, ctx->stream));
    CK(hipStreamSynchronize(ctx->stream));
    const u64 sampled_tiles = (tpc + step - 1) / step;
    rl->G = G; rl->nch = nch;
    for (u32 o = 0; o < G; ++o) {
        u64 tot = 0, mx = 0;
        for (u64 c = 0; c < nch; ++c) { const u64 v = cells[(size_t)o * nch + c]; tot += v; mx = std::max(mx, v); }
        u64 sl;
        if (step == 1) sl = mx + 8;
        else { sl = tot * tpc / (sampled_tiles * nch) + 1; sl += sl * 2 / 25 + 128; }
        if (ctx->tune.sk_slice) sl = ctx->tune.sk_slice;
        if (sl * nch >= 0xFFFF0000ull) return REC_L0_NO;
        rl->slice[o] = (u32)sl; rl->region[o] = sl * nch;
    }
    ctx->mark("level0_size");
    return DSKGPU_OK;
}

int rec_l0_sweep(dskgpu_ctx* ctx, const RecL0& rl, u32 olo, u32 ohi, u64 (&base_words)[SK_MAX_OWNERS]) {
    SkParams sp = ctx->sk_sp;
    u64 obase[SK_MAX_OWNERS] = {0}; u32 osl[SK_MAX_OWNERS] = {0};
    u64 tot = 0;
    for (u32 o = 0; o < rl.G; ++o) { osl[o] = rl.slice[o]; obase[o] = tot; if (o >= olo && o < ohi) tot += rl.region[o]; base_words[o] = obase[o] * sp.R; }
    CK(ctx->l0buf.ensure(tot * sp.R * 8 + 64));
    CK(ctx->sk_lay.ensure(SK_MAX_OWNERS * 12));
    CK(hipMemcpyAsync(ctx->sk_lay.p, obase, sizeof obase, hipMemcpyHostToDevice, ctx->stream));
    CK(hipMemcpyAsync(ctx->sk_lay.as<u64>() + SK_MAX_OWNERS, osl, sizeof osl, hipMemcpyHostToDevice, ctx->stream));
    sp.olo = olo; sp.ohi = ohi; sp.obase = ctx->sk_lay.as<unsigned long long>(); sp.oslice = reinterpret_cast<const u32*>(ctx->sk_lay.as<u64>() + SK_MAX_OWNERS);
    sp.c0 = 0; sp.c0g = 0; sp.clen = (u32)rl.nch; sp.rbase = 0; sp.slice = 0;
    u32* sc = ctx->scalars.as<u32>();
    CK(hipMemsetAsync(ctx->sk_sent.p, 0, SK_MAX_OWNERS * 8, ctx->stream));
    CK(hipMemsetAsync(sc + SC_OVF1, 0, 4, ctx->stream));
#define SK_CALL(K_, M_) hipLaunchKernelGGL((k_sk_scatter<true, K_, M_>), dim3(sp.nchunks), dim3(SK_NT), 0, ctx->stream, ctx->packed.as<u64>(), ctx->inval.as<u32>(), sp, \
                                          (const unsigned long long*)nullptr, ctx->l0buf.as<u64>(), sc + SC_OVF1, ctx->sk_sent.as<unsigned long long>())
    SK_DISPATCH(ctx, sp, SK_CALL);
#undef SK_CALL
    CKL("k_sk_scatter(passes)");
    ctx->mark("level0");
    CK(hipMemcpyAsync(&ctx->h_ovf1, sc + SC_OVF1, 4, hipMemcpyDeviceToHost, ctx->stream));
    CK(hipMemcpyAsync(ctx->h_sk_sent, ctx->sk_sent.p, SK_MAX_OWNERS * 8, hipMemcpyDeviceToHost, ctx->stream));
    CK(hipStreamSynchronize(ctx->stream));
    if (ctx->tune.verbose) fprintf(stderr, "[dskgpu] level 0 (records): passes %u..%u of %u materialised, %.2f GB%s\n", olo, ohi - 1, rl.G, (double)tot * sp.R * 8e-9,
                                   ctx->h_ovf1 ? " -- a slice overflowed: starting over on the key-array path" : "");
    return ctx->h_ovf1 ? REC_L0_NO : DSKGPU_OK;
}

template <int W>
int run_pipeline(dskgpu_ctx* ctx, bool from_reads, const typename KeyT<W>::T* d_keys_in, u64 nkeys_in) {
    typedef typename KeyT<W>::T Key;
    ctx->drop_result();
    ctx->sink = dskgpu_ctx::RowSink{};
    if (from_reads) { ctx->st_names.clear(); ctx->st_ms.clear(); }
    ctx->marks.clear(); ctx->ev_used = 0;
    const u64 n_upper = from_reads ? ctx->n_bytes : nkeys_in;
    u64 nwords = 0;
    ctx->mark("start");
    if (from_reads) {
        int rc = encode_current(ctx, &nwords);
        if (rc) return rc;
        ctx->mark("encode");
    }
    CK(ctx->scalars.ensure(SC_COUNT * 4));
    CK(ctx->ghist.ensure(((size_t)ctx->cfg.histo_max + 1 + 2) * 8));
    CK(ctx->gstats.ensure(4 * 8));
    ctx->have_nvalid = false;
    if (from_reads && nwords) {
        CK(hipMemsetAsync(ctx->gstats.p, 0, 4 * 8, ctx->stream));
        hipLaunchKernelGGL(k_count_valid, dim3((unsigned)std::min<u64>((nwords + 255) / 256, (u64)ctx->num_cu * 8)), dim3(256), 0, ctx->stream,
                           ctx->inval.as<u32>(), nwords, (int)ctx->cfg.kmer_size, ctx->gstats.as<u64>() + 3);
        CKL("k_count_valid");
        {
            void* lz = landing(ctx, 8);
            CK(hipMemcpyAsync(lz ? lz : (void*)&ctx->h_nvalid, ctx->gstats.as<u64>() + 3, 8, hipMemcpyDeviceToHost, ctx->stream));
            CK(hipStreamSynchronize(ctx->stream));
            if (lz) std::memcpy(&ctx->h_nvalid, lz, 8);
        }
        ctx->have_nvalid = true;
    }
    const u64 max_keys = ctx->max_keys_per_pass ? ctx->max_keys_per_pass : 0xD0000000ull;
    const u64 n_keys = (from_reads && ctx->have_nvalid) ? std::max<u64>(1, ctx->h_nvalid) : n_upper;
    u64 pass_keys = max_keys;
    if (W == 1 && from_reads && ctx->have_nvalid && n_keys > max_keys && !ctx->max_keys_per_pass && !ctx->tune.no_level0)
        pass_keys = ctx->tune.mp_pass_mkeys ? (u64)ctx->tune.mp_pass_mkeys * 1000000ull : 1000000000ull;
    const u64 hard_max = W == 2 && !ctx->max_keys_per_pass ? std::min<u64>(max_keys, 2400000000ull) : max_keys;
    u32 npass = (u32)std::max<u64>(1, (n_keys + pass_keys - 1) / pass_keys);
    bool rec_l0 = W <= 2 && from_reads && ctx->have_nvalid && ctx->sk_mode && ctx->cfg.world_size == 1 && !ctx->tune.no_level0 && !ctx->tune.l0_keys && !ctx->rec_l0_off &&
                  (npass > 1 || n_keys > hard_max);
    RecL0 rl;
    struct SenderStateGuard {
        dskgpu_ctx* c; SkParams sp; std::vector<uint8_t> table; bool armed = false;
        ~SenderStateGuard() { if (armed) { c->sk_sp = sp; c->h_table.swap(table); c->table_dirty = true; c->sk_prepared = false; c->enc_fresh = false; } }
    } sender_guard{ctx, ctx->sk_sp, ctx->h_table};
    if (rec_l0) {
        sender_guard.armed = true;
        u64 want = ctx->max_keys_per_pass ? max_keys : ctx->tune.mp_pass_mkeys ? (u64)ctx->tune.mp_pass_mkeys * 1000000ull : (W == 1 ? 1200000000ull : 1000000000ull);
        u64 G = (n_keys + want - 1) / want;
        if (G < 2) G = 2;
        if (G > SK_MAX_OWNERS) G = SK_MAX_OWNERS;
        if (n_keys / G + n_keys / G / 7 > hard_max && !ctx->max_keys_per_pass) rec_l0 = false;
        else {
            const int rc = rec_l0_prepare(ctx, nwords, (u32)G, &rl);
            if (rc == REC_L0_NO) rec_l0 = false; else if (rc) return rc;
            else npass = (u32)G;
        }
    }
    u64 cap_floor = 0;
    for (;;) {
        if (npass > 4096) return fail(ctx, DSKGPU_E_OVERFLOW, "too many passes (one k-mer alone exceeds a pass)");
        const u64 cap = npass == 1 ? n_upper : std::min<u64>(n_upper, std::max<u64>(cap_floor, n_keys / npass + n_keys / npass / 16 + (1u << 20)));
        if (cap >= 0xFFFF0000ull) { npass *= 2; cap_floor = 0; continue; }
        if (W > 1) CK(ctx->abund2.ensure((cap + 1) * 4));
        ctx->hist.assign((size_t)ctx->cfg.histo_max + 1, 0);
        std::vector<u64> pass_hist(ctx->hist.size());
        u64 tot_rows = 0, tot_kmers = 0, tot_distinct = 0;
        Plan pl{};
        bool too_big = false; u64 seen = 0;
        u32 l0_lo = 0, l0_n = 0; u64 l0_keys[L0_MAX_PASSES] = {0}; u64 l0_base[L0_MAX_PASSES] = {0};
        bool l0_try = W == 1 && from_reads && npass > 1 && ctx->have_nvalid && !ctx->tune.no_level0 && !rec_l0;
        u32 r_hi = 0; u64 r_base[SK_MAX_OWNERS] = {0};
        bool restart = false;
        u64 sweeps = 0;
        bool rows_sized = false;
        ctx->job_passes = npass;
        PartPasses& mp = ctx->rs.mp;
        mp.passes.clear(); mp.off_used = 0;
        mp.ok = npass > 1 && (ctx->cfg.flags & DSKGPU_F_PARTITION_ORDER) && !(ctx->cfg.flags & DSKGPU_F_NO_SORT) && !ctx->bank_job.active;
        if (mp.ok) { CK(mp.flag.ensure(256)); CK(hipMemsetAsync(mp.flag.p, 0, 4, ctx->stream)); }
        for (u32 p = 0; p < npass; ++p) {
            PassResult r{};
            r.plan = pl;
            int rc;
            mp.row_base = tot_rows;
            ctx->sink = dskgpu_ctx::RowSink{};
            if (npass > 1 && rows_sized) {
                ctx->sink.active = true; ctx->sink.rows = tot_rows; ctx->sink.ab = ctx->acc_ab.as<u32>();
                u64 cap_rows = ctx->acc_ab.cap / 4;
                for (int x = 0; x < W; ++x) { ctx->sink.w[x] = ctx->acc_w[x].as<u64>(); cap_rows = std::min<u64>(cap_rows, ctx->acc_w[x].cap / 8); }
                ctx->sink.cap = cap_rows;
            }
            if (npass > 1) { ctx->opt1_off = false; ctx->opt2_off = false; ctx->mw_v3_off = false; }
            if (rec_l0) {
                if (p >= r_hi) {
                    size_t free_b = 0, total_b = 0;
                    CK(hipMemGetInfo(&free_b, &total_b));
                    const u64 nper = n_keys / npass + 1;
                    const u64 have = ctx->bufA.cap + ctx->bufB.cap + ctx->l0buf.cap;
                    const u64 rows_have = ctx->acc_ab.cap + ctx->acc_w[0].cap + (W > 1 ? ctx->acc_w[1].cap : 0);
                    const u64 rows_want = rows_sized ? 0 : n_keys / 16 * (8ull * W + 4);
                    const u64 need = nper * (W == 1 ? 30ull : 50ull) + (4ull << 30) + (rows_want > rows_have ? rows_want - rows_have : 0);
                    const u64 room = free_b + have > need ? free_b + have - need : 0;
                    const u64 R8 = (u64)ctx->sk_sp.R * 8;
                    u64 left = 0; for (u32 o = p; o < npass; ++o) left += rl.region[o] * R8;
                    const u64 nsw = std::max<u64>(1, (left + std::max<u64>(room, 1) - 1) / std::max<u64>(room, 1));
                    const u64 target = (left + nsw - 1) / nsw;
                    u64 acc = 0; u32 hi = p;
                    while (hi < npass && (hi == p || (acc + rl.region[hi] * R8 <= room && acc < target))) { acc += rl.region[hi] * R8; ++hi; }
                    if (ctx->tune.l0_passes) hi = std::min<u32>(npass, p + ctx->tune.l0_passes);
                    rc = rec_l0_sweep(ctx, rl, p, hi, r_base);
                    if (rc == REC_L0_NO) { restart = true; break; }
                    if (rc) return rc;
                    r_hi = hi; ++sweeps;
                }
                const u64 nk_in = ctx->h_sk_sent[p];
                ctx->rec_src = ctx->l0buf.as<u64>() + r_base[p]; ctx->rec_n = rl.region[p]; ctx->rec_expanded = false; ctx->rec_sized = false;
                ctx->rec_hint = 0; ctx->rec_hint_est = false; ctx->rec_slice_end.clear(); ctx->rec_gate = nullptr;
                if (nk_in == 0) { rc = DSKGPU_OK; CK(hipMemsetAsync(ctx->ghist.p, 0, ((size_t)ctx->cfg.histo_max + 1) * 8, ctx->stream)); }
                else rc = run_one_pass<W>(ctx, false, nullptr, nk_in, 0, 0u, 1u, nk_in, &r);
                ctx->rec_src = nullptr;
            } else
            if (l0_try && p >= l0_lo + l0_n) {
                const u64 reserve = rows_sized ? 0 : n_keys / 16 * 12;
                if constexpr (W == 1) { if ((rc = level0_materialise(ctx, nwords, p, npass, reserve, &l0_n, l0_keys, l0_base))) return rc; }
                l0_lo = p;
                if (l0_n == 0) l0_try = false;
                else ++sweeps;
            }
            if (rec_l0) {  }
            else if (l0_try && p < l0_lo + l0_n) {
                const u64 nk_in = l0_keys[p - l0_lo];
                rc = run_one_pass<W>(ctx, false, reinterpret_cast<const Key*>(ctx->l0buf.as<u64>() + l0_base[p - l0_lo]), nk_in, 0, 0u, 1u, nk_in, &r);
            } else { rc = run_one_pass<W>(ctx, from_reads, d_keys_in, nkeys_in, nwords, p, npass, cap, &r); if (from_reads) ++sweeps; }
            if (rc) return rc;
            if (r.too_big) { too_big = true; seen = r.keys_seen; break; }
            pl = r.plan;
            const u64 ns = r.rows;
            tot_kmers += r.kmers; tot_distinct += r.distinct;
            if (npass > 1) {
                CK(hipMemcpyAsync(pass_hist.data(), ctx->ghist.p, pass_hist.size() * 8, hipMemcpyDeviceToHost, ctx->stream));
                const u64 want_rows = std::max<u64>(tot_rows + ns + 1, p == 0 ? (ns + ns / 8 + 1024) * npass : 0);
                const bool took = ctx->sink.took;
                const u64 keep_rows = tot_rows + (took ? ns : 0);
                ctx->sink = dskgpu_ctx::RowSink{};
                auto grow_rows = [&]() {
                    bool ok = ctx->acc_ab.ensure_keep(want_rows * 4, keep_rows * 4, ctx->stream) == 0;
                    for (int x = 0; x < W && ok; ++x) ok = ctx->acc_w[x].ensure_keep(want_rows * 8, keep_rows * 8, ctx->stream) == 0;
                    return ok;
                };
                if (!grow_rows()) {
                    (void)hipGetLastError();
                    if (l0_n && ctx->l0buf.p) { ctx->l0buf.release(); l0_n = p + 1 - l0_lo; }
                    if (rec_l0 && ctx->l0buf.p) { ctx->l0buf.release(); r_hi = p + 1; }
                    if (!grow_rows()) return fail(ctx, DSKGPU_E_NOMEM, "row accumulation");
                }
                rows_sized = true;
                if (ns && !took) {
                    CK(hipMemcpyAsync(ctx->acc_ab.as<u32>() + tot_rows, ctx->out_ab.p, ns * 4, hipMemcpyDeviceToDevice, ctx->stream));
                    for (int x = 0; x < W; ++x)
                        CK(hipMemcpyAsync(ctx->acc_w[x].as<u64>() + tot_rows, ctx->out_w[x].p, ns * 8, hipMemcpyDeviceToDevice, ctx->stream));
                }
                CK(hipStreamSynchronize(ctx->stream));
                for (size_t i = 0; i < pass_hist.size(); ++i) ctx->hist[i] += pass_hist[i];
                ctx->resolve_marks();
                ctx->mark("start");
            }
            tot_rows += ns;
        }
        if (rec_l0) { ctx->sk_prepared = false; ctx->enc_fresh = false; }
        if (restart) {
            ctx->rec_l0_off = true;
            ctx->resolve_marks();
            return run_pipeline<W>(ctx, from_reads, d_keys_in, nkeys_in);
        }
        if (too_big) {
            if (seen + (1u << 20) < 0xFFFF0000ull && seen > cap_floor) cap_floor = seen + (1u << 20); else { npass *= 2; cap_floor = 0; }
// ... 357 lines not shown
            CK(ctx->srt_tmp.ensure(tmp));
            CK(rocprim::radix_sort_pairs(ctx->srt_tmp.p, tmp, ctx->u_w[0].as<u64>(), ctx->s_w[0].as<u64>(), ctx->u_val.as<u64>(), ctx->s_val.as<u64>(), (size_t)nu, 0u, end_bit, ctx->stream));
        } else {
            const u64* rows[4] = {nullptr, nullptr, nullptr, nullptr};
            for (int x = 0; x < W; ++x) rows[x] = ctx->u_w[x].as<u64>();
            if ((rc = sort_index_multiword(ctx, rows, nu, W))) return rc;
            const u32* idx = ctx->srt_idx.as<u32>();
            for (int x = 0; x < W; ++x) {
                CK(ctx->s_w[x].ensure((nu + 1) * 8));
                hipLaunchKernelGGL(k_gather<u64>, dim3(gb), dim3(256), 0, ctx->stream, ctx->s_w[x].as<u64>(), ctx->u_w[x].as<u64>(), idx, nu);
            }
            CK(ctx->s_val.ensure((nu + 1) * 8));
            hipLaunchKernelGGL(k_gather<u64>, dim3(gb), dim3(256), 0, ctx->stream, ctx->s_val.as<u64>(), ctx->u_val.as<u64>(), idx, nu);
        }
        CKL("bank sort");
    }
    const size_t nh = (size_t)ctx->cfg.histo_max + 1;
    CK(ctx->m_flag.ensure((nu + 2) * 4)); CK(ctx->m_pos.ensure((nu + 2) * 4)); CK(ctx->m_sum.ensure((nu + 2) * 4));
    CK(ctx->gh2d.ensure(nh * 11 * 8));
    CK(hipMemsetAsync(ctx->ghist.p, 0, nh * 8, ctx->stream));
    CK(hipMemsetAsync(ctx->gh2d.p, 0, nh * 11 * 8, ctx->stream));
    CK(hipMemsetAsync(ctx->gstats.p, 0, 32, ctx->stream));
    MergeParams mp{B, ctx->cfg.solidity_kind, ctx->cfg.solidity_custom, ctx->cfg.abundance_min, ctx->cfg.abundance_max, ctx->cfg.histo_max,
                   (ctx->cfg.flags & DSKGPU_F_HISTO2D) ? 1u : 0u};
    u64 n_solid = 0;
    if (nu) {
        RowsIn ri{}; RowsOut ro{};
        for (int x = 0; x < W; ++x) ri.w[x] = ctx->s_w[x].as<u64>();
        hipLaunchKernelGGL(k_merge_banks<W>, dim3(gb), dim3(256), 0, ctx->stream, ri,
                           ctx->s_val.as<u64>(), nu, mp, ctx->m_flag.as<u32>(), ctx->m_sum.as<u32>(), ctx->ghist.as<u64>(), ctx->gh2d.as<u64>(), ctx->gstats.as<u64>());
        hipLaunchKernelGGL(k_copy_u32, dim3(gb), dim3(256), 0, ctx->stream, ctx->m_pos.as<u32>(), ctx->m_flag.as<u32>(), nu);
        CKL("k_merge_banks");
        ctx->h_sc[SC_F] = (u32)nu;
        CK(hipMemcpyAsync(ctx->scalars.as<u32>() + SC_F, &ctx->h_sc[SC_F], 4, hipMemcpyHostToDevice, ctx->stream));
        if ((rc = run_scan(ctx, ctx->m_pos.as<u32>(), ctx->scalars.as<u32>() + SC_F, nu))) return rc;
        CK(hipMemcpyAsync(&ctx->h_back[1], ctx->m_pos.as<u32>() + nu, 4, hipMemcpyDeviceToHost, ctx->stream));
        CK(hipStreamSynchronize(ctx->stream));
        n_solid = ctx->h_back[1];
        CK(ctx->out_ab.ensure((n_solid + 1) * 4));
        for (int x = 0; x < W; ++x) { CK(ctx->out_w[x].ensure((n_solid + 1) * 8)); ro.w[x] = ctx->out_w[x].as<u64>(); }
        hipLaunchKernelGGL(k_pick_rows<W>, dim3(gb), dim3(256), 0, ctx->stream, ri,
                           ctx->m_sum.as<u32>(), ctx->m_flag.as<u32>(), ctx->m_pos.as<u32>(), nu, ro, ctx->out_ab.as<u32>());
        CKL("k_pick_rows");
    }
    ctx->hist.assign(nh, 0); ctx->hist2d.assign(nh * 11, 0);
    CK(hipMemcpyAsync(ctx->hist.data(), ctx->ghist.p, nh * 8, hipMemcpyDeviceToHost, ctx->stream));
    CK(hipMemcpyAsync(ctx->hist2d.data(), ctx->gh2d.p, nh * 11 * 8, hipMemcpyDeviceToHost, ctx->stream));
    CK(hipMemcpyAsync(&ctx->h_stats[0], ctx->gstats.p, 32, hipMemcpyDeviceToHost, ctx->stream));
    CK(hipStreamSynchronize(ctx->stream));
    for (int x = 0; x < 4; ++x) ctx->res_w[x] = x < W ? ctx->out_w[x].as<u64>() : nullptr;
    ctx->res_ab = ctx->out_ab.as<u32>();
    ctx->n_rows = n_solid;
    ctx->stats.n_bytes = total; ctx->stats.n_kmers = tot_kmers; ctx->stats.n_distinct = ctx->h_stats[0]; ctx->stats.n_solid = n_solid;
    ctx->stats.n_passes = passes; ctx->stats.n_retries = retries;
    ctx->stats.n_partitions = ctx->cfg.nb_partitions ? ctx->cfg.nb_partitions : 4u;
    ctx->have_result = true;
    return DSKGPU_OK;
}
template <int W>
int run_banks(dskgpu_ctx* ctx) {
    int rc = banks_begin(ctx);
    if (rc) return rc;
    const u32 B = (u32)ctx->bank_job.ends.size();
    for (u32 b = 0; b < B; ++b) {
        banks_select(ctx, b);
        if ((rc = run_pipeline<W>(ctx, true, nullptr, 0)) || (rc = banks_add<W>(ctx, b))) { banks_abort(ctx); return rc; }
    }
    return banks_finish<W>(ctx);
}

}

__attribute__((visibility("hidden"))) bool dskgpu_i_per_bank(dskgpu_ctx* ctx) {
    const bool banks = ctx->bank_ends.size() > 1 || (!ctx->bank_ends.empty() && ctx->bank_ends.back() < ctx->n_bytes);
    return banks && (ctx->cfg.solidity_kind != DSKGPU_SOLIDITY_SUM || (ctx->cfg.flags & DSKGPU_F_HISTO2D));
}
__attribute__((visibility("hidden"))) uint32_t dskgpu_i_banks(dskgpu_ctx* ctx) { return banks_of(ctx); }
__attribute__((visibility("hidden"))) int dskgpu_i_banks_begin(dskgpu_ctx* ctx) { return banks_begin(ctx); }
__attribute__((visibility("hidden"))) void dskgpu_i_banks_select(dskgpu_ctx* ctx, uint32_t b) { banks_select(ctx, b); }
__attribute__((visibility("hidden"))) void dskgpu_i_banks_abort(dskgpu_ctx* ctx) { banks_abort(ctx); }
__attribute__((visibility("hidden"))) int dskgpu_i_banks_add(dskgpu_ctx* ctx, uint32_t b) {
    return ctx->W == 1 ? banks_add<1>(ctx, b) : ctx->W == 2 ? banks_add<2>(ctx, b) : banks_add<4>(ctx, b);
}
__attribute__((visibility("hidden"))) int dskgpu_i_banks_finish(dskgpu_ctx* ctx) {
    return ctx->W == 1 ? banks_finish<1>(ctx) : ctx->W == 2 ? banks_finish<2>(ctx) : banks_finish<4>(ctx);
}

static_assert(((size_t)32 << 20) / RP_BLOCK <= (size_t)RP_NT * RP_SCAN_PER, "k_rp_scan walks the block summaries of one staging piece (PIN_CHUNK) with RP_SCAN_PER per thread");
template <int FMT>
static void launch_raw_chunk(dskgpu_ctx* ctx, u32 n, uint8_t* out) {
    const u32 nb = (n + RP_BLOCK - 1) / RP_BLOCK;
    const unsigned char* in = ctx->raw_in.as<unsigned char>();
    RawState* st = ctx->raw_state.as<RawState>();
    hipLaunchKernelGGL((k_rp_count<FMT>), dim3(nb), dim3(RP_NT), 0, ctx->stream, in, n, ctx->raw_blk.as<RpBlock>());
    hipLaunchKernelGGL((k_rp_scan<FMT>), dim3(1), dim3(RP_NT), 0, ctx->stream, in, n, nb, ctx->raw_blk.as<RpBlock>(), st,
                       ctx->raw_boff.as<unsigned long long>(), ctx->raw_bstate.as<u32>(), out);
    hipLaunchKernelGGL((k_rp_write<FMT>), dim3(nb), dim3(RP_NT), 0, ctx->stream, in, n, ctx->raw_boff.as<unsigned long long>(),
                       ctx->raw_bstate.as<u32>(), st, out);
}

extern "C" {

const char* dskgpu_version(void) { return DSKGPU_VERSION; }

int dskgpu_device_count(void) { int n = 0; return hipGetDeviceCount(&n) == hipSuccess ? n : 0; }

const char* dskgpu_last_error(const dskgpu_ctx* ctx) { return ctx ? ctx->err.c_str() : g_create_err.c_str(); }

int dskgpu_create(const dskgpu_config* cfg, dskgpu_ctx** out) {
    if (!cfg || !out) { g_create_err = "null argument"; return DSKGPU_E_ARG; }
    *out = nullptr;
    if (cfg->kmer_size < 1 || cfg->kmer_size > 128) { g_create_err = "kmer_size must be in 1..128"; return DSKGPU_E_ARG; }
    if (cfg->solidity_kind > DSKGPU_SOLIDITY_CUSTOM) { g_create_err = "unknown solidity_kind"; return DSKGPU_E_ARG; }
    if (g_place_k < 0) { const char* e = getenv("DSKGPU_PLACE"); g_place_k = e ? atoi(e) : 0; }
    if ((cfg->flags & DSKGPU_F_PLACE) && g_place_k < 2) g_place_k = 8;
    const u32 ws = cfg->world_size ? cfg->world_size : 1;
    if ((ws & (ws - 1)) != 0 || ws > 64 || cfg->rank >= ws) { g_create_err = "world_size must be a power of two <= 64 and rank < world_size"; return DSKGPU_E_ARG; }
    int ndev = 0;
    hipError_t e = hipGetDeviceCount(&ndev);
    if (e != hipSuccess || ndev == 0) { g_create_err = std::string("no HIP device: ") + hipGetErrorString(e); return DSKGPU_E_DEVICE; }
    if (cfg->device < 0 || cfg->device >= ndev) { g_create_err = "bad device ordinal"; return DSKGPU_E_ARG; }
    e = hipSetDevice(cfg->device);
    if (e != hipSuccess) { g_create_err = std::string("hipSetDevice: ") + hipGetErrorString(e); return DSKGPU_E_DEVICE; }
    dskgpu_ctx* ctx = new dskgpu_ctx();
    ctx->cfg = *cfg;
    ctx->cfg.world_size = ws;
    if (ctx->cfg.histo_max == 0) ctx->cfg.histo_max = 10000;
    if (ctx->cfg.abundance_max == 0) ctx->cfg.abundance_max = 0x7FFFFFFFu;
    if (ctx->cfg.minimizer_size == 0) ctx->cfg.minimizer_size = 10;
    ctx->W = cfg->kmer_size <= 32 ? 1 : cfg->kmer_size <= 64 ? 2 : 4;
    ctx->words_out = (int)((cfg->kmer_size + 31) / 32);
    ctx->sentinel_ok = !sentinel_is_a_kmer(ctx->W, cfg->kmer_size);
    ctx->max_keys_per_pass = (u64)cfg->max_pass_mkeys * 1000000ull;
    ctx->tune.read();
    ctx->sk_mode = cfg->kmer_size >= 20 && cfg->kmer_size <= 64 && !(cfg->flags & DSKGPU_F_MG_EXPLICIT);
    if (ctx->sk_mode) {
        ctx->sk_sp.k = cfg->kmer_size; ctx->sk_sp.G = ws;
        ctx->sk_sp.m = std::min<u32>(std::min<u32>(ctx->cfg.minimizer_size, 16u), cfg->kmer_size - 15u);
        ctx->sk_sp.R = sk_record_words(cfg->kmer_size);
    }
    { int cus = 0; if (hipDeviceGetAttribute(&cus, hipDeviceAttributeMultiprocessorCount, cfg->device) == hipSuccess && cus > 0) ctx->num_cu = cus; }
    e = hipStreamCreateWithFlags(&ctx->stream, hipStreamNonBlocking);
    if (e != hipSuccess) { g_create_err = std::string("hipStreamCreate: ") + hipGetErrorString(e); delete ctx; return DSKGPU_E_DEVICE; }
    ctx->own_stream = true;
    *out = ctx;
    return DSKGPU_OK;
}

void dskgpu_destroy(dskgpu_ctx* ctx) {
    if (!ctx) return;
    (void)hipSetDevice(ctx->cfg.device);
    (void)hipStreamSynchronize(ctx->stream);
    DevBuf* bufs[] = {&ctx->reads_own, &ctx->raw_in, &ctx->raw_blk, &ctx->raw_boff, &ctx->raw_bstate, &ctx->raw_state, &ctx->packed, &ctx->inval, &ctx->bufA, &ctx->bufB, &ctx->mat1, &ctx->mat2, &ctx->sums,
                      &ctx->descs1, &ctx->descs2, &ctx->seg, &ctx->fstart, &ctx->nsolid, &ctx->scalars, &ctx->ghist, &ctx->gstats, &ctx->chain_next, &ctx->smp_mat, &ctx->smp_descs, &ctx->boff, &ctx->hv_lut, &ctx->hv_collect, &ctx->hv_buf, &ctx->dbg, &ctx->l0buf,
                      &ctx->out_ab, &ctx->srt_ab, &ctx->srt_tmp,
                      &ctx->srt_idx, &ctx->srt_idx2, &ctx->srt_k, &ctx->srt_k2, &ctx->abund2, &ctx->acc_ab, &ctx->u_val,
                      &ctx->s_val, &ctx->m_flag, &ctx->m_pos, &ctx->m_sum, &ctx->gh2d,
                      &ctx->sk_sums, &ctx->sk_cbase, &ctx->sk_keys, &ctx->sk_table, &ctx->sk_load, &ctx->sk_sent, &ctx->cur_state, &ctx->smp_keys, &ctx->sk_lay, &ctx->sk_cb64, &ctx->back_dev};
    if (ctx->back_host) (void)hipHostFree(ctx->back_host);
    ctx->rs.release();
    ctx->query.release();
    ctx->unitigs.release();
    if (ctx->land) (void)hipHostFree(ctx->land);
    for (DevBuf* b : bufs) b->release();
    for (int i = 0; i < 4; ++i) { ctx->out_w[i].release(); ctx->srt_w[i].release(); ctx->acc_w[i].release(); ctx->u_w[i].release(); ctx->s_w[i].release(); }
    for (hipEvent_t e : ctx->ev_pool) (void)hipEventDestroy(e);
    for (int i = 0; i < 2; ++i) { if (ctx->pin[i]) (void)hipHostFree(ctx->pin[i]); if (ctx->pin_ev[i]) (void)hipEventDestroy(ctx->pin_ev[i]); }
    if (ctx->own_stream) (void)hipStreamDestroy(ctx->stream);
    delete ctx;
}

int dskgpu_set_stream(dskgpu_ctx* ctx, void* hip_stream) {
    if (!ctx) return DSKGPU_E_ARG;
    CK(hipSetDevice(ctx->cfg.device));
    CK(hipStreamSynchronize(ctx->stream));
    if (hip_stream) {
        if (ctx->own_stream) { (void)hipStreamDestroy(ctx->stream); ctx->own_stream = false; }
        ctx->stream = reinterpret_cast<hipStream_t>(hip_stream);
    } else if (!ctx->own_stream) {
        CK(hipStreamCreateWithFlags(&ctx->stream, hipStreamNonBlocking));
        ctx->own_stream = true;
    }
    return DSKGPU_OK;
}

#define PIN_CHUNK ((size_t)32 << 20)
static_assert(PIN_CHUNK == ((size_t)32 << 20), "launch_raw_chunk's capacity check is written for 32 MB pieces");
static void stage_copy(void* dst, const void* src, size_t n) {
    const unsigned T = n >= ((size_t)16 << 20) ? 8u : n >= ((size_t)8 << 20) ? 4u : n >= ((size_t)2 << 20) ? 2u : 1u;
    if (T == 1) { std::memcpy(dst, src, n); return; }
    const size_t per = (((n + T - 1) / T) + 4095) & ~(size_t)4095;
    auto part = [=](unsigned t) { const size_t a = (size_t)t * per; if (a < n) std::memcpy((char*)dst + a, (const char*)src + a, std::min(per, n - a)); };
    std::thread th[7];
    unsigned started = 1;
    try { for (; started < T; ++started) th[started - 1] = std::thread(part, started); }
    catch (const std::system_error&) {}
    part(0);
    for (unsigned t = started; t < T; ++t) part(t);
    for (unsigned t = 1; t < started; ++t) th[t - 1].join();
}

static int ensure_pinned(dskgpu_ctx* ctx) {
    if (ctx->pin[0] && ctx->pin[1]) return DSKGPU_OK;
    for (int i = 0; i < 2; ++i) {
        if (!ctx->pin[i]) CK(hipHostMalloc(&ctx->pin[i], PIN_CHUNK, hipHostMallocDefault));
        if (!ctx->pin_ev[i]) CK(hipEventCreateWithFlags(&ctx->pin_ev[i], hipEventDisableTiming));
    }
    return DSKGPU_OK;
}

static int raw_finish(dskgpu_ctx* ctx, u64* lines);
int dskgpu_push_reads(dskgpu_ctx* ctx, const char* bytes, uint64_t nbytes) {
    if (!ctx || (!bytes && nbytes)) return DSKGPU_E_ARG;
    CK(hipSetDevice(ctx->cfg.device));
    if (ctx->raw_pending) { const int e = raw_finish(ctx, nullptr); if (e) return e; }
    const u64 need = ctx->reads_len + nbytes + 1;
    if (need > ctx->reads_own.cap) {
        DevBuf nb;
        CK(nb.ensure(std::max<u64>(need, std::max<u64>(ctx->reads_own.cap * 2, (u64)256 << 20))));
        if (ctx->reads_len) CK(hipMemcpyAsync(nb.p, ctx->reads_own.p, ctx->reads_len, hipMemcpyDeviceToDevice, ctx->stream));
        CK(hipStreamSynchronize(ctx->stream));
        ctx->reads_own.release();
        ctx->reads_own = nb;
    }
    uint8_t* dst = ctx->reads_own.as<uint8_t>();
    if (nbytes) {
        const size_t CH = PIN_CHUNK;
        { const int e = ensure_pinned(ctx); if (e) return e; }
        for (u64 off = 0; off < nbytes; off += CH, ctx->pin_next ^= 1) {
            const int slot = ctx->pin_next;
            const size_t len = (size_t)std::min<u64>(CH, nbytes - off);
            if (ctx->pin_used[slot]) CK(hipEventSynchronize(ctx->pin_ev[slot]));
            stage_copy(ctx->pin[slot], bytes + off, len);
            CK(hipMemcpyAsync(dst + ctx->reads_len + off, ctx->pin[slot], len, hipMemcpyHostToDevice, ctx->stream));
            CK(hipEventRecord(ctx->pin_ev[slot], ctx->stream));
            ctx->pin_used[slot] = true;
        }
    }
    CK(hipMemsetAsync(dst + ctx->reads_len + nbytes, '\n', 1, ctx->stream));
    ctx->reads_len += nbytes + 1;
    ctx->d_reads = dst; ctx->n_bytes = ctx->reads_len; ctx->enc_keep = false; ctx->enc_fresh = false; ctx->sk_prepared = false; ctx->sk_exact = false; ctx->opt2_off = false; ctx->opt1_off = false; ctx->mw_v3_off = false; ctx->rec_l0_off = false; ctx->last_rows = 0;
    return DSKGPU_OK;
}

static int raw_finish(dskgpu_ctx* ctx, u64* lines) {
    if (!ctx->raw_pending) return DSKGPU_OK;
    RawState s;
    CK(hipMemcpyAsync(&s, ctx->raw_state.p, sizeof(RawState), hipMemcpyDeviceToHost, ctx->stream));
    CK(hipStreamSynchronize(ctx->stream));
    ctx->raw_pending = false;
    uint8_t* dst = ctx->reads_own.as<uint8_t>();
    if (!rp_file_ok(s)) s.bad = 1;
    if (s.bad) {
        ctx->reads_len = ctx->raw_base;
        ctx->d_reads = dst; ctx->n_bytes = ctx->reads_len;
        return fail(ctx, DSKGPU_E_FORMAT, "dskgpu_push_raw: the text is not 4-line FASTQ / FASTA as declared (the raw pushes were dropped: parse on the host and push the reads)");
    }
    if (s.out_len + 1 > ctx->reads_own.cap) return fail(ctx, DSKGPU_E_STATE, "dskgpu_push_raw: stream longer than its bound");
    CK(hipMemsetAsync(dst + s.out_len, '\n', 1, ctx->stream));
    ctx->reads_len = s.out_len + 1;
    if (lines) *lines = s.recs;
    ctx->d_reads = dst; ctx->n_bytes = ctx->reads_len; ctx->enc_keep = false; ctx->enc_fresh = false; ctx->sk_prepared = false; ctx->sk_exact = false; ctx->opt2_off = false; ctx->opt1_off = false; ctx->mw_v3_off = false; ctx->rec_l0_off = false; ctx->last_rows = 0;
    return DSKGPU_OK;
}
#define RAW_SYNC(ctx) do { if ((ctx)->raw_pending) { const int e_ = raw_finish(ctx, nullptr); if (e_) return e_; } } while (0)

int dskgpu_raw_finish(dskgpu_ctx* ctx, uint64_t* stream_bytes, uint64_t* records) {
    if (!ctx) return DSKGPU_E_ARG;
    CK(hipSetDevice(ctx->cfg.device));
    u64 ln = 0;
    const int rc = raw_finish(ctx, &ln);
    if (stream_bytes) *stream_bytes = ctx->reads_len;
    if (records) *records = ln;
    return rc;
}

int dskgpu_push_raw(dskgpu_ctx* ctx, const char* text, uint64_t nbytes, int format, int new_file) {
    if (!ctx || (!text && nbytes) || (format != DSKGPU_RAW_FASTA && format != DSKGPU_RAW_FASTQ)) return DSKGPU_E_ARG;
    CK(hipSetDevice(ctx->cfg.device));
    if (!ctx->raw_pending) {
        CK(ctx->raw_state.ensure(sizeof(RawState)));
        CK(ctx->raw_in.ensure(PIN_CHUNK));
        const u64 maxb = PIN_CHUNK / RP_BLOCK;
        CK(ctx->raw_blk.ensure(maxb * sizeof(RpBlock)));
        CK(ctx->raw_boff.ensure(maxb * 8));
        CK(ctx->raw_bstate.ensure((maxb + 1) * 4));
        ctx->raw_base = ctx->raw_ub = ctx->reads_len;
        hipLaunchKernelGGL(k_rp_init, dim3(1), dim3(1), 0, ctx->stream, ctx->raw_state.as<RawState>(), (unsigned long long)ctx->reads_len);
        CKL("k_rp_init");
        ctx->raw_pending = true;
    } else if (new_file) {
        hipLaunchKernelGGL(k_rp_fresh, dim3(1), dim3(1), 0, ctx->stream, ctx->raw_state.as<RawState>());
        CKL("k_rp_fresh");
    }
    const u64 need = ctx->raw_ub + nbytes + 2;
    if (need > ctx->reads_own.cap) {
        DevBuf nb;
        CK(nb.ensure(std::max<u64>(need, std::max<u64>(ctx->reads_own.cap * 2, (u64)256 << 20))));
        if (ctx->raw_ub) CK(hipMemcpyAsync(nb.p, ctx->reads_own.p, ctx->raw_ub, hipMemcpyDeviceToDevice, ctx->stream));
        CK(hipStreamSynchronize(ctx->stream));
        ctx->reads_own.release();
        ctx->reads_own = nb;
    }
    uint8_t* out = ctx->reads_own.as<uint8_t>();
    if (nbytes) {
        const size_t CH = PIN_CHUNK;
        { const int e = ensure_pinned(ctx); if (e) return e; }
        for (u64 off = 0; off < nbytes; off += CH, ctx->pin_next ^= 1) {
            const int slot = ctx->pin_next;
            const size_t len = (size_t)std::min<u64>(CH, nbytes - off);
            if (ctx->pin_used[slot]) CK(hipEventSynchronize(ctx->pin_ev[slot]));
            stage_copy(ctx->pin[slot], text + off, len);
            CK(hipMemcpyAsync(ctx->raw_in.p, ctx->pin[slot], len, hipMemcpyHostToDevice, ctx->stream));
            CK(hipEventRecord(ctx->pin_ev[slot], ctx->stream));
            ctx->pin_used[slot] = true;
            if (format == DSKGPU_RAW_FASTQ) launch_raw_chunk<RP_FASTQ>(ctx, (u32)len, out);
// ... 427 lines not shown
```

dsk_amd/csrc/engine.h:

```cpp
#pragma once
#include <algorithm>
#include <cstring>
#include <string>
#include <vector>

#include "../../include/dskgpu.h"
#include "layouts.h"

hipError_t placed_malloc(void** out, size_t bytes);

struct DevBuf {
    void* p = nullptr;
    size_t cap = 0;
    hipError_t ensure(size_t bytes) {
        if (bytes <= cap) return hipSuccess;
        size_t want = ((p ? bytes + bytes / 16 : bytes) + 255) & ~size_t(255);
        if (p) { (void)hipFree(p); p = nullptr; cap = 0; }
        hipError_t e = placed_malloc(&p, want);
        if (e == hipSuccess) cap = want; else p = nullptr;
        return e;
    }
    int ensure_keep(size_t bytes, size_t keep, hipStream_t stream) {
        if (bytes <= cap) return 0;
        void* np = nullptr;
        size_t want = ((std::max(bytes, cap + cap / 2) + 255) & ~size_t(255));
        if (hipMalloc(&np, want) != hipSuccess) return -1;
        if (keep && p) {
            if (hipMemcpyAsync(np, p, keep, hipMemcpyDeviceToDevice, stream) != hipSuccess || hipStreamSynchronize(stream) != hipSuccess) { (void)hipFree(np); return -1; }
        }
        if (p) (void)hipFree(p);
        p = np; cap = want;
        return 0;
    }
    void release() { if (p) (void)hipFree(p); p = nullptr; cap = 0; }
    template <class T> T* as() const { return reinterpret_cast<T*>(p); }
};

enum Scalar { SC_NCH1 = 0, SC_MLEN1, SC_NCH2, SC_MLEN2, SC_OVERFLOW, SC_F, SC_SORTFLAG, SC_OVF2, SC_OVF1, SC_RSLEN, SC_RSWORK, SC_RSWORK2, SC_RSTIES, SC_EXT, SC_NCHAINED, SC_NCH_S, SC_MLEN_S, SC_WORK2, SC_COUNT = 24 };

struct Stage { const char* name; hipEvent_t ev; };

struct Tuning {
    bool no_opt1 = false, no_opt2 = false;
    bool no_aligned = false;
    u32 rs_heavy = 0;
    u32 rs_bbits = 0;
    u32 rs_block_rows = 0;
    bool sk_exact = false, no_recsrc = false;
    u32 opt_cap = 0;
    u64 opt_slice = 0;
    u64 sk_slice = 0, sk_minslice = 2000;
    u32 table_maxload = 0;
    long long max_ext = -1;
    bool no_sample = false;
    bool no_heavy = false;
    bool verbose = false;
    bool no_level0 = false; u32 l0_passes = 0;
    u64 rs_max_rows = 0;
    u32 ps_maxc = 0;
    bool sk_generic = false;
    bool l0_keys = false;
    u32 mp_pass_mkeys = 0;
    u64 rs_slab_rows = 0;
    bool unitig_stages = false;
    void read() {
        auto on = [](const char* n) { return getenv(n) != nullptr; };
        auto num = [](const char* n, u64 dflt) { const char* e = getenv(n); return e ? (u64)atoll(e) : dflt; };
        no_opt1 = on("DSKGPU_NO_OPT1"); no_opt2 = on("DSKGPU_NO_OPT2"); no_aligned = on("DSKGPU_NO_ALIGNED");
        sk_exact = on("DSKGPU_SK_EXACT");
        no_recsrc = on("DSKGPU_NO_RECSRC");
        opt_cap = (u32)num("DSKGPU_OPT_CAP", 0) & ~7u; opt_slice = num("DSKGPU_OPT_SLICE", 0) & ~7ull;
        sk_slice = num("DSKGPU_SK_SLICE", 0); sk_minslice = num("DSKGPU_SK_MINSLICE", 2000);
        table_maxload = (u32)num("DSKGPU_TABLE_MAXLOAD", 0);
        max_ext = getenv("DSKGPU_MAX_EXT") ? atoll(getenv("DSKGPU_MAX_EXT")) : -1;
        no_sample = on("DSKGPU_NO_SAMPLE"); no_heavy = on("DSKGPU_NO_HEAVY"); verbose = on("DSKGPU_VERBOSE"); no_level0 = on("DSKGPU_NO_LEVEL0"); l0_passes = (u32)num("DSKGPU_L0_PASSES", 0); mp_pass_mkeys = (u32)num("DSKGPU_MP_PASS_MKEYS", 0); rs_max_rows = num("DSKGPU_RS_MAX_ROWS", 0); l0_keys = on("DSKGPU_L0_KEYS"); sk_generic = on("DSKGPU_SK_GENERIC"); ps_maxc = (u32)num("DSKGPU_PS_MAXC", 0);
        rs_slab_rows = num("DSKGPU_RS_SLAB_ROWS", 0);
        unitig_stages = on("DSKGPU_UNITIG_STAGES");
        rs_block_rows = (u32)num("DSKGPU_RS_BLOCK_ROWS", 0); rs_bbits = (u32)num("DSKGPU_RS_BBITS", 0); rs_heavy = (u32)num("DSKGPU_RS_HEAVY", 0);
    }
};

struct SparseRows {
    int W = 0;
    const void* keys = nullptr; const u32 *ab = nullptr, *soff = nullptr, *fstart = nullptr; u32 cap = 0, F = 0;
    u64 n_sparse = 0; u32 n_tail = 0; RowsIn tail_w{}; const u32* tail_ab = nullptr;
    template <class S> S as(u32 qpc = 0) const { return S{static_cast<decltype(S::keys)>(keys), ab, soff, fstart, cap, F, qpc}; }
    Rows2C tail2() const { return Rows2C{tail_w.w[1], tail_w.w[0], tail_ab}; }
};

struct PartPasses {
    struct Pass { u64 row_base; u32 nparts, off_index; };
    std::vector<Pass> passes; DevBuf part_off, flag; u32 off_used = 0; bool ok = false; u64 row_base = 0;
    std::vector<u32> h_off;
};

struct RowSort {
    DevBuf fix_list;
    DevBuf g[4];
    DevBuf del, lens;
    std::vector<u64> h_del; std::vector<u32> h_lens, h_lin;
    DevBuf ovs;
    u32 flag = 0, listed = 0;
    u64* hist_pin = nullptr; size_t hist_pin_n = 0;
    bool part_mode = false; u32 n_parts = 0; u32* h_part_off = nullptr; size_t h_part_cap = 0; DevBuf part_off;
    std::vector<u64> h_part_off64;
    PartPasses mp;
    void release() {
        for (DevBuf* b : {&fix_list, &g[0], &g[1], &g[2], &g[3], &del, &lens, &ovs, &part_off, &mp.part_off, &mp.flag}) b->release();
        if (hist_pin) (void)hipHostFree(hist_pin);
        if (h_part_off) (void)hipHostFree(h_part_off);
        hist_pin = nullptr; h_part_off = nullptr;
    }
};

struct Query {
    DevBuf table, packed, inval, deg;
    u64 cap = 0;
    bool valid = false;
    void release() { table.release(); packed.release(); inval.release(); deg.release(); cap = 0; valid = false; }
};

struct Unitigs {
    DevBuf unitig, pos, offsets, ab_sum, kind;
    DevBuf ends, e_offsets, e_targets;
    dskgpu_unitig_stats stats{};
    dskgpu_unitig_edge_stats e_stats{};
    bool valid = false;
    bool e_valid = false;
    void release_edges() { for (DevBuf* b : {&ends, &e_offsets, &e_targets}) b->release(); e_stats = dskgpu_unitig_edge_stats{}; e_valid = false; }
    void release() { for (DevBuf* b : {&unitig, &pos, &offsets, &ab_sum, &kind}) b->release(); stats = dskgpu_unitig_stats{}; valid = false; release_edges(); }
};

struct BankJob { dskgpu_config cfg; const uint8_t* base; u64 total; std::vector<u64> ends; u64 nu, tot_kmers; u32 passes, retries; bool active = false; };

struct dskgpu_ctx {
    dskgpu_config cfg{};
    BankJob bank_job{};
    Tuning tune;
    int W = 1;
    int words_out = 1;
    hipStream_t stream = nullptr;
    bool own_stream = false;
    int num_cu = 256;
    std::string err;

    DevBuf reads_own; u64 reads_len = 0;
    void* pin[2] = {nullptr, nullptr}; hipEvent_t pin_ev[2] = {nullptr, nullptr}; bool pin_used[2] = {false, false}; int pin_next = 0;
    const uint8_t* d_reads = nullptr; u64 n_bytes = 0;
    DevBuf raw_in, raw_blk, raw_boff, raw_bstate, raw_state;
    bool raw_pending = false; u64 raw_base = 0, raw_ub = 0;

    DevBuf packed, inval;
    DevBuf bufA, bufB;
    DevBuf mat1, mat2, sums, descs1, descs2, seg, fstart, nsolid, scalars, ghist, gstats, chain_next;
    RowSort rs;
    DevBuf smp_keys;
    DevBuf smp_mat, smp_descs, boff;
    DevBuf dbg, l0buf; DevBuf hv_lut, hv_collect, hv_buf;
    std::vector<unsigned char> h_hv_lut; std::vector<u32> h_hv_cnt, h_hv_step; std::vector<u64> h_hv_coll, h_hv_keys;
    std::vector<ChunkDesc> h_descs_s, h_descs1, h_descs2; std::vector<u64> h_cbeg; std::vector<u32> h_boff; std::vector<u64> h_mom;
    DevBuf out_w[4], srt_w[4], acc_w[4];
    DevBuf out_ab, srt_ab, srt_tmp, srt_idx, srt_idx2, srt_k, srt_k2, abund2, acc_ab;
    u64 max_keys_per_pass = 0;
    std::vector<u64> bank_ends;
    DevBuf u_w[4], s_w[4], u_val, s_val, m_flag, m_pos, m_sum, gh2d;
    std::vector<u64> hist2d;
    std::vector<u32> h_starts;
    std::vector<u64> h_rstart;
    std::vector<u32> h_sk_cells;
    std::vector<u64> h_sk_cb64;
    DevBuf sk_cb64;
    bool enc_keep = false;
    bool enc_fresh = false;
    bool sk_mode = false, sk_prepared = false;
    bool sk_slices = false;
    bool sk_exact = false;
    SkParams sk_sp{};
    DevBuf sk_sums, sk_cbase, sk_keys, sk_table, sk_load, sk_sent, sk_lay;
    u64 last_rows = 0;
    bool rec_l0_off = false;
    u64 h_sk_sent[SK_MAX_OWNERS] = {0};
    u64 h_sk_est[SK_MAX_OWNERS] = {0};
    u32 sk_nslices = 0;
    u64 rec_hint = 0;
    bool rec_hint_est = false;
    std::vector<u64> rec_slice_end;
    dskgpu_slice_gate rec_gate = nullptr; void* rec_gate_user = nullptr; u32 rec_gated = 0;
    bool rec_gate_failed = false;
    std::vector<u32> h_slice_chunk;
    DevBuf cur_state;
    bool rec_sized = false;
    std::vector<uint8_t> h_table;
    bool table_dirty = true;
    std::vector<u32> h_sk_sums; std::vector<u64> h_sk_cbase;
    const u64* rec_src = nullptr; u64 rec_n = 0; u64 rec_nch = 0, rec_rpc = 0; bool rec_expanded = false;
    u64* land = nullptr;
    DevBuf back_dev; u64* back_host = nullptr;
    u32 h_back[3] = {0}; u64 h_stats[4] = {0}; u32 h_ovf1 = 0; u64 h_nvalid = 0; bool have_nvalid = false;
    bool sentinel_ok = true;
    bool opt1_off = false;
    bool mw_v3_off = false;
    bool opt2_off = false;
    std::vector<const void*> big_lds_fns;
    u32 h_sc[SC_COUNT] = {0};

    u32 job_passes = 1;
    SparseRows sp_rows;
    SparseRows take_sparse_rows() { const SparseRows r = sp_rows; sp_rows = SparseRows{}; return r; }
    struct RowSink { bool active = false, took = false; u32* ab = nullptr; u64* w[4] = {nullptr, nullptr, nullptr, nullptr}; u64 rows = 0, cap = 0; } sink;
    bool have_result = false;
    u64 n_rows = 0;
    const u64* res_w[4] = {nullptr, nullptr, nullptr, nullptr}; const u32* res_ab = nullptr;
    dskgpu_stats stats{};
    std::vector<u64> hist;
    Query query;
    Unitigs unitigs;
    void drop_result() { have_result = false; query.release(); unitigs.release(); }

    std::vector<Stage> marks;
    std::vector<hipEvent_t> ev_pool; size_t ev_used = 0;
    std::vector<const char*> st_names; std::vector<float> st_ms;

    void mark(const char* name) {
        if (!(cfg.flags & DSKGPU_F_TIMING)) return;
        if (ev_used == ev_pool.size()) { hipEvent_t e; (void)hipEventCreate(&e); ev_pool.push_back(e); }
        hipEvent_t e = ev_pool[ev_used++];
        (void)hipEventRecord(e, stream);
        marks.push_back({name, e});
    }
    void resolve_marks() {
        for (size_t i = 0; i + 1 < marks.size(); ++i) {
            float ms = 0; (void)hipEventElapsedTime(&ms, marks[i].ev, marks[i + 1].ev);
            size_t at = 0;
            while (at < st_names.size() && std::strcmp(st_names[at], marks[i + 1].name) != 0) ++at;
            if (at == st_names.size()) { st_names.push_back(marks[i + 1].name); st_ms.push_back(ms); } else st_ms[at] += ms;
        }
        marks.clear(); ev_used = 0;
    }
};

#define CK(expr)                                                                             \
    do {                                                                                     \
        hipError_t e_ = (expr);                                                              \
        if (e_ != hipSuccess) {                                                              \
            ctx->err = std::string(#expr) + ": " + hipGetErrorString(e_);                    \
            return (e_ == hipErrorOutOfMemory) ? DSKGPU_E_NOMEM : DSKGPU_E_DEVICE;           \
        }                                                                                    \
    } while (0)

#define CKL(what)                                                                            \
    do {                                                                                     \
        hipError_t e_ = hipGetLastError();                                                   \
        if (e_ != hipSuccess) {                                                              \
            ctx->err = std::string(what) + ": " + hipGetErrorString(e_);                     \
            return DSKGPU_E_DEVICE;                                                          \
        }                                                                                    \
    } while (0)

inline int fail(dskgpu_ctx* ctx, int code, const std::string& msg) { ctx->err = msg; return code; }

int encode_into(dskgpu_ctx* ctx, const uint8_t* d_bytes, u64 n, u64* packed, u32* inval);
int run_scan(dskgpu_ctx* ctx, u32* a, const u32* d_len, u64 max_len);
int allow_big_lds(dskgpu_ctx* ctx, const void* fn, int bytes = 160 * 1024);

int order_rows(dskgpu_ctx* ctx, u64 n, u32 npass);
u64 rs_max_rows(const dskgpu_ctx* ctx);
int sort_index_multiword(dskgpu_ctx* ctx, const u64* const* rows, u64 n, int W);
u32 part_sort_nparts(const SparseRows& rows);
int launch_part_sort(dskgpu_ctx* ctx, const SparseRows& rows, RowsOut out, u32* out_ab, u32* d_part_off, u32* d_flag, u32* nparts_out);
u32 rows_partitions(const dskgpu_ctx* ctx);
void rows_partition_range(const dskgpu_ctx* ctx, u32 p, u64* b, u64* e);

struct QTable;
int ensure_index(dskgpu_ctx* ctx);
QTable query_table(const dskgpu_ctx* ctx);
int query_ensure(dskgpu_ctx* ctx, DevBuf& b, size_t bytes, const char* what);
void query_begin(dskgpu_ctx* ctx);
int query_finish(dskgpu_ctx* ctx);
```

dsk_amd/csrc/kernels.h:

```cpp
#pragma once
#include "layouts.h"

#ifndef SC_NT
#define SC_NT 1024
#endif
template <int W> struct Tile {
    static constexpr int KPT = 16 / W;
    static constexpr int KEYS = SC_NT * KPT;
    static constexpr int WORDS = KEYS / 32;
};
#define MAX_BINS 2048


template <bool ALIGNED>
__global__ __launch_bounds__(256) void k_encode(const uint8_t* __restrict__ s, u64 n,
                                                u64* __restrict__ packed, u32* __restrict__ inval, u64 nwords) {
    const u64 stride = (u64)gridDim.x * blockDim.x;
    for (u64 w = (u64)blockIdx.x * blockDim.x + threadIdx.x; w < nwords; w += stride) {
        const u64 base = w * 32;
        u32 x[8];
        if (ALIGNED && base + 32 <= n) {
            const uint4 a = *reinterpret_cast<const uint4*>(s + base);
            const uint4 b = *reinterpret_cast<const uint4*>(s + base + 16);
            x[0] = a.x; x[1] = a.y; x[2] = a.z; x[3] = a.w; x[4] = b.x; x[5] = b.y; x[6] = b.z; x[7] = b.w;
        } else {
#pragma unroll
            for (int q = 0; q < 8; ++q) {
                u32 v = 0;
#pragma unroll
                for (int b = 0; b < 4; ++b) {
                    const u64 p = base + q * 4 + b;
                    const u32 c = p < n ? s[p] : (u32)'\n';
                    v |= c << (8 * b);
                }
                x[q] = v;
            }
        }
        u64 pk = 0; u32 iv = 0;
        constexpr u32 BASES = (1u << 1) | (1u << 3) | (1u << 7) | (1u << 20);
#pragma unroll
        for (int q = 0; q < 8; ++q) {
            const u32 xx = x[q];
            const u32 codes = ((((xx >> 1) & 0x03030303u) * 0x40100401u) >> 24);
            const u32 hi = (xx & 0xC0C0C0C0u) ^ 0x40404040u;
            u32 ok = 0;
#pragma unroll
            for (int b = 0; b < 4; ++b) ok |= ((BASES >> ((xx >> (8 * b)) & 31u)) & 1u) << (8 * b);
            const u32 hz = (((hi & 0x7F7F7F7Fu) + 0x7F7F7F7Fu) | hi) >> 7;
            const u32 good = ok & ~hz & 0x01010101u;
            const u32 bad4 = (((good ^ 0x01010101u) * 0x08040201u) >> 24) & 0xFu;
            pk |= (u64)codes << (56 - 8 * q);
            iv |= bad4 << (28 - 4 * q);
        }
        packed[w] = pk;
        inval[w] = iv;
    }
}

template <int W> struct KeyT { typedef KN<W> T; };
template <> struct KeyT<1> { typedef u64 T; };

__device__ __forceinline__ u64 digit_word(u64 h) { return h; }
template <int W> __device__ __forceinline__ u64 digit_word(const KN<W>& h) { return h.w[W - 1]; }

struct DigitSpec { u32 mode, pa, pb, world, npass, pass; };
__device__ __forceinline__ u32 key_pass(u64 w, const DigitSpec& ds) {
    const u32 frac = (((u32)(w >> 12) & 0xFFFFFu) * ds.world) & 0xFFFFFu;
    return (frac * ds.npass) >> 20;
}
template <int MODE>
__device__ __forceinline__ u32 key_digit(u64 w, const DigitSpec& ds) {
    if (MODE == 1 || MODE == 3) return __umulhi((u32)(w >> 32), ds.pa);
    if (MODE == 2) return __umulhi((u32)(w >> 32) * ds.pa, ds.pb);
    if (MODE == 4) return key_pass(w, ds) - ds.pass;
    return (((u32)(w >> 12) & 0xFFFFFu) * ds.pa) >> 20;
}
template <int MODE>
__device__ __forceinline__ bool key_in_pass(u64 w, const DigitSpec& ds) {
    if (MODE == 3) return key_pass(w, ds) == ds.pass;
    if (MODE == 4) return key_pass(w, ds) - ds.pass < ds.pa;
    return true;
}

template <int NP>
__device__ __forceinline__ u32 gen_kmers_multi(const u64* __restrict__ packed, const u32* __restrict__ inval, u64 wi, int t0, int k, K2 (&c)[NP]) {
    return gen_kmers2<NP>(packed, inval, wi, t0, k, c);
}
template <int W, int NP>
__device__ __forceinline__ u32 gen_kmers_multi(const u64* __restrict__ packed, const u32* __restrict__ inval, u64 wi, int t0, int k, KN<W> (&c)[NP]) {
    return gen_kmersN<W, NP>(packed, inval, wi, t0, k, c);
}

template <int W>
__device__ __forceinline__ u32 tile_keys_reads(const u64* __restrict__ packed, const u32* __restrict__ inval,
                                               u64 w0, u64 wend, int k, KN<W> (&h)[Tile<W>::KPT]) {
    constexpr int KPT = Tile<W>::KPT, TPW = 32 / KPT;
    const u64 wi = w0 + (threadIdx.x / TPW);
    if (wi >= wend) return 0u;
    const u32 vm = gen_kmers_multi(packed, inval, wi, (int)(threadIdx.x % TPW) * KPT, k, h);
#pragma unroll
    for (int j = 0; j < KPT; ++j) kmixN(h[j]);
    return vm;
}
__device__ __forceinline__ u32 tile_keys_reads(const u64* __restrict__ packed, const u32* __restrict__ inval,
                                               u64 w0, u64 wend, int k, u64 (&h)[16]) {
    const u64 wi = w0 + (threadIdx.x >> 1);
    if (wi >= wend) return 0u;
    const u32 vm = gen_kmers1<16>(packed, inval, wi, (threadIdx.x & 1) * 16, k, h);
#pragma unroll
    for (int j = 0; j < 16; ++j) h[j] = kmix(h[j]);
    return vm;
}

__device__ __forceinline__ bool is_pad_key(u64 h) { return h == DSK_EMPTY; }
template <int W> __device__ __forceinline__ bool is_pad_key(const KN<W>& h) {
    bool e = true;
#pragma unroll
    for (int x = 0; x < W; ++x) e = e && (h.w[x] == DSK_EMPTY);
    return e;
}
__device__ __forceinline__ bool keys_same(u64 a, u64 b) { return a == b; }
template <int W> __device__ __forceinline__ bool keys_same(const KN<W>& a, const KN<W>& b) { return key_eq(a, b); }
template <int W>
__device__ __forceinline__ u32 tile_keys_array(const typename KeyT<W>::T* __restrict__ in, u64 k0, u64 kend,
                                               typename KeyT<W>::T (&h)[Tile<W>::KPT]) {
    const typename KeyT<W>::T* base = in + k0;
    const u64 left = kend - k0;
    const u32 n = left < (u64)Tile<W>::KEYS ? (u32)left : (u32)Tile<W>::KEYS;
    u32 vm = 0;
#pragma unroll
    for (int j = 0; j < Tile<W>::KPT; ++j) {
        const u32 o = threadIdx.x + (u32)j * SC_NT;
        const bool ok = o < n;
        h[j] = base[ok ? o : n - 1];
        vm |= ((ok && !is_pad_key(h[j])) ? 1u : 0u) << j;
    }
    return vm;
}

template <int W, int SRC, int MODE>
__global__ __launch_bounds__(SC_NT) void k_hist(const u64* __restrict__ packed, const u32* __restrict__ inval,
                                                const typename KeyT<W>::T* __restrict__ keys,
                                                const ChunkDesc* __restrict__ descs, const u32* __restrict__ d_nchunks,
                                                u32* __restrict__ matrix, int k, DigitSpec ds, u32 P) {
    __shared__ u32 lh[MAX_BINS + 1];
    constexpr int KPT = Tile<W>::KPT;
    const u32 nchunks = *d_nchunks;
    for (u32 g = blockIdx.x; g < nchunks; g += gridDim.x) {
        const ChunkDesc d = descs[g];
        for (u32 b = threadIdx.x; b <= P; b += SC_NT) lh[b] = 0;
        __syncthreads();
        const u64 step = SRC == 0 ? Tile<W>::WORDS : Tile<W>::KEYS;
        typename KeyT<W>::T ha[KPT], hb[KPT]; u32 vma = 0, vmb = 0;
        auto process = [&](typename KeyT<W>::T (&h)[KPT], u32 vm) {
            u32 dg[KPT];
#pragma unroll
            for (int j = 0; j < KPT; ++j)
                dg[j] = ((vm & (1u << j)) && key_in_pass<MODE>(digit_word(h[j]), ds)) ? key_digit<MODE>(digit_word(h[j]), ds) : P;
#pragma unroll
            for (int j = 0; j < KPT; ++j) atomicAdd(&lh[dg[j]], 1u);
        };
        if (SRC == 0) {
            for (u64 t0 = d.begin; t0 < d.end; t0 += step) {
                vma = tile_keys_reads(packed, inval, t0, d.end, k, ha);
                process(ha, vma);
            }
        } else {
            if (d.begin < d.end) vma = tile_keys_array<W>(keys, d.begin, d.end, ha);
            for (u64 t0 = d.begin; t0 < d.end; t0 += 2 * step) {
                if (t0 + step < d.end) vmb = tile_keys_array<W>(keys, t0 + step, d.end, hb);
                process(ha, vma);
                const u64 t1 = t0 + step;
                if (t1 >= d.end) break;
                if (t1 + step < d.end) vma = tile_keys_array<W>(keys, t1 + step, d.end, ha);
                process(hb, vmb);
            }
        }
        __syncthreads();
        for (u32 b = threadIdx.x; b < P; b += SC_NT) matrix[d.flat_base + (u64)b * d.stride] = lh[b];
        __syncthreads();
    }
}

#define SCAN_NT 256
#define SCAN_IPT 16
#define SCAN_BLK (SCAN_NT * SCAN_IPT)

__global__ __launch_bounds__(SCAN_NT) void k_scan_reduce(const u32* __restrict__ a, const u32* __restrict__ d_len,
                                                         u32* __restrict__ sums) {
    __shared__ u32 ws[SCAN_NT / 64];
    const u64 len = *d_len;
    const u64 b0 = (u64)blockIdx.x * SCAN_BLK;
    if (b0 >= len) return;
    u32 s = 0;
#pragma unroll
    for (int j = 0; j < SCAN_IPT; ++j) {
        const u64 i = b0 + threadIdx.x + (u64)j * SCAN_NT;
        if (i < len) s += a[i];
    }
#pragma unroll
    for (int d = 32; d >= 1; d >>= 1) s += __shfl_down(s, d);
    if ((threadIdx.x & 63) == 0) ws[threadIdx.x >> 6] = s;
    __syncthreads();
    if (threadIdx.x == 0) { u32 t = 0; for (int i = 0; i < SCAN_NT / 64; ++i) t += ws[i]; sums[blockIdx.x] = t; }
}

__global__ __launch_bounds__(1024) void k_scan_sums(u32* __restrict__ sums, const u32* __restrict__ d_len,
                                                    u32* __restrict__ a) {
    __shared__ u32 ws[16]; __shared__ u32 carry_s;
    const u64 len = *d_len;
    const u32 nb = (u32)((len + SCAN_BLK - 1) / SCAN_BLK);
    const int lane = threadIdx.x & 63, wave = threadIdx.x >> 6;
    if (threadIdx.x == 0) carry_s = 0;
    __syncthreads();
    for (u32 c0 = 0; c0 < nb; c0 += 1024) {
        const u32 i = c0 + threadIdx.x;
        const u32 x = i < nb ? sums[i] : 0u;
        u32 y = x;
#pragma unroll
        for (int d = 1; d < 64; d <<= 1) { const u32 t = __shfl_up(y, d); if (lane >= d) y += t; }
        if (lane == 63) ws[wave] = y;
        __syncthreads();
        if (wave == 0) {
            const u32 wx = lane < 16 ? ws[lane] : 0u; u32 wy = wx;
#pragma unroll
            for (int d = 1; d < 16; d <<= 1) { const u32 t = __shfl_up(wy, d); if (lane >= d) wy += t; }
            if (lane < 16) ws[lane] = wy - wx;
        }
        __syncthreads();
        const u32 carry = carry_s;
        const u32 excl = carry + ws[wave] + y - x;
        if (i < nb) sums[i] = excl;
        __syncthreads();
        if (threadIdx.x == 1023) carry_s = excl + x;
        __syncthreads();
    }
    if (threadIdx.x == 0) a[len] = carry_s;
}

__global__ __launch_bounds__(SCAN_NT) void k_scan_apply(u32* __restrict__ a, const u32* __restrict__ d_len,
                                                        const u32* __restrict__ sums) {
    __shared__ u32 ws[SCAN_NT / 64];
    const u64 len = *d_len;
    const u64 b0 = (u64)blockIdx.x * SCAN_BLK;
    if (b0 >= len) return;
    const u64 i0 = b0 + (u64)threadIdx.x * SCAN_IPT;
    u32 v[SCAN_IPT]; u32 s = 0;
#pragma unroll
    for (int j = 0; j < SCAN_IPT; ++j) { v[j] = (i0 + j < len) ? a[i0 + j] : 0u; s += v[j]; }
    const int lane = threadIdx.x & 63, wave = threadIdx.x >> 6;
    u32 y = s;
#pragma unroll
    for (int d = 1; d < 64; d <<= 1) { const u32 t = __shfl_up(y, d); if (lane >= d) y += t; }
    if (lane == 63) ws[wave] = y;
    __syncthreads();
    u32 wpre = 0;
    for (int w = 0; w < wave; ++w) wpre += ws[w];
    u32 run = sums[blockIdx.x] + wpre + y - s;
#pragma unroll
    for (int j = 0; j < SCAN_IPT; ++j) { if (i0 + j < len) a[i0 + j] = run; run += v[j]; }
}


struct OptSpec { u32 cap; u32* subcnt; u32* ovf; const u32* fill; u32 slice, nsl; u64 sstride;
                 u32 F, max_ext; u32* next; u32* ext_cursor; u32* chain_list; u32* chain_cnt;
                 u32* work;
                 unsigned long long* dbg; };
#define CHAIN_BIT 0x80000000u
#define HV_KEYS 4
__device__ __forceinline__ bool is_empty_key(u64 h) { return h == DSK_EMPTY; }
template <int W> __device__ __forceinline__ bool is_empty_key(const KN<W>& h) {
    bool e = true;
#pragma unroll
    for (int x = 0; x < W; ++x) e = e && (h.w[x] == DSK_EMPTY);
    return e;
}
template <int W> __device__ __forceinline__ typename KeyT<W>::T empty_key();
template <> __device__ __forceinline__ u64 empty_key<1>() { return DSK_EMPTY; }
template <> __device__ __forceinline__ K2 empty_key<2>() { K2 k; k.w[0] = k.w[1] = DSK_EMPTY; return k; }
template <> __device__ __forceinline__ KN<4> empty_key<4>() { KN<4> k; k.w[0] = k.w[1] = k.w[2] = k.w[3] = DSK_EMPTY; return k; }


__device__ __forceinline__ u64 sk_key1(const u64* r, int j, int k);
__device__ __forceinline__ K2 sk_key2(const u64* r, int j, int k);
__device__ __forceinline__ void sk_key(const u64* r, int j, int k, u64& out) { out = sk_key1(r, j, k); }
__device__ __forceinline__ void sk_key(const u64* r, int j, int k, K2& out) { out = sk_key2(r, j, k); }
template <int W> __device__ __forceinline__ void sk_key(const u64*, int, int, KN<W>&) {}

template <int W> struct RecTile { static constexpr int NR = W == 1 ? 3 * SC_NT : SC_NT; static constexpr int RPT = NR / SC_NT;
                                  static constexpr int RS = W == 1 ? 2 : 3; };
template <int W> struct RecPre { u64 w[RecTile<W>::RPT * RecTile<W>::RS]; };
template <int W>
__device__ __forceinline__ void rec_prefetch(RecPre<W>& pre, const u64* __restrict__ rec, u32 R, u64 r0, u64 rend) {
    constexpr int RPT = RecTile<W>::RPT, RS = RecTile<W>::RS;
#pragma unroll
    for (int u = 0; u < RPT; ++u) {
        const u64 r = r0 + (u64)threadIdx.x * RPT + u;
        const u64* p = rec + (r < rend ? r : r0) * R;
        pre.w[u * RS] = p[0]; pre.w[u * RS + 1] = p[1];
        if (RS == 3) pre.w[u * RS + 2] = (R == 3) ? p[2] : 0ull;
    }
}
template <int W>
__device__ __forceinline__ u32 tile_keys_records(const RecPre<W>& pre, u32 R, u64 r0, u64 rend, int k,
                                                 typename KeyT<W>::T (&h)[Tile<W>::KPT], char* scratch, u32* wsum, u32* taken) {
    constexpr int KPT = Tile<W>::KPT, KEYS = Tile<W>::KEYS, NR = RecTile<W>::NR, RPT = RecTile<W>::RPT, RS = RecTile<W>::RS;
    u64* srec = reinterpret_cast<u64*>(scratch);
    u32* first = reinterpret_cast<u32*>(srec + (size_t)NR * RS);
    u32* info = first + SC_NT;
    const int tid = threadIdx.x, lane = tid & 63, wave = tid >> 6;
    const u64 left = rend - r0;
    u32 n[RPT], s = 0;
#pragma unroll
    for (int u = 0; u < RPT; ++u) {
        const u32 l = (u32)tid * RPT + u;
        n[u] = l < left ? (u32)(pre.w[u * RS + ((RS == 3 && R == 3) ? 2 : 1)] & 0xFFu) : 0u;
        s += n[u] + (n[u] ? 0x40000u : 0u);
    }
    const u32 inc = wave_incl_scan(s);
    if (lane == 63) wsum[wave] = inc;
    lds_barrier();
    u32 run = inc - s;
#pragma unroll
    for (int x = 0; x < SC_NT / 64; ++x) { const u32 v = wsum[x]; if (x < wave) run += v; }
#pragma unroll
    for (int u = 0; u < RPT; ++u) {
        const u32 l = (u32)tid * RPT + u;
        const u32 start = run & 0x3FFFFu, dense = run >> 18;
        const bool exists = l < left;
        const bool fit = exists && start + n[u] <= (u32)KEYS;
        if (!fit && start <= (u32)KEYS && (exists || l == left)) *info = (l << 16) | start;
        if (fit && n[u]) {
#pragma unroll
            for (int x = 0; x < RS; ++x) srec[dense * RS + x] = pre.w[u * RS + x];
            const u32 bnd = (start + KPT - 1) & ~(u32)(KPT - 1);
            for (u32 q = bnd; q < start + n[u]; q += KPT) first[q / KPT] = (dense << 5) | (q - start);
        }
        run += n[u] + (n[u] ? 0x40000u : 0u);
        if (u == RPT - 1 && tid == SC_NT - 1 && fit) *info = ((u32)NR << 16) | (run & 0x3FFFFu);
    }
    lds_barrier();
    const u32 inf = *info;
    *taken = inf >> 16;
    const u32 nkeys = inf & 0xFFFFu;
    u32 vm = 0;
    const u32 slot0 = (u32)tid * KPT;
    if (slot0 < nkeys) {
        const u32 e = first[tid];
        u32 rl = e >> 5, jj = e & 31u;
        u64 r[3]; r[2] = 0ull;
#pragma unroll
        for (int x = 0; x < RS; ++x) r[x] = srec[rl * RS + x];
        u32 nn = (u32)(r[(RS == 3 && R == 3) ? 2 : 1] & 0xFFu);
#pragma unroll
        for (int j = 0; j < KPT; ++j) {
            if (slot0 + j < nkeys) {
                if (jj == nn) {
                    ++rl; jj = 0;
#pragma unroll
                    for (int x = 0; x < RS; ++x) r[x] = srec[rl * RS + x];
                    nn = (u32)(r[(RS == 3 && R == 3) ? 2 : 1] & 0xFFu);
                }
                sk_key(r, (int)jj, k, h[j]);
                ++jj;
                vm |= 1u << j;
            }
        }
    }
    return vm;
}

struct Opt1Spec { const u32* boff; u32 area, dump; u32* ovf; u32* fill; u32 R; u64* nkeys;
                  const u64* hv_keys; unsigned long long* hv_cnt; u32 slice_len; const u64* obase; u64 obase0;
                  u64 anchor[4];
                  u32 uslice;
                  u32* cur_state; u32 g0, gn, resume, last;
                  };
#define L0_MAX_PASSES 16

template <int W, int SRC, int MODE, bool OPT = false, bool HEAVY = false>
__global__ __launch_bounds__(SC_NT, 4) void k_scatter(const u64* __restrict__ packed, const u32* __restrict__ inval,
                                                   const typename KeyT<W>::T* __restrict__ keys,
                                                   const ChunkDesc* __restrict__ descs, const u32* __restrict__ d_nchunks,
                                                   const u32* __restrict__ scanned,
                                                   typename KeyT<W>::T* __restrict__ out, int k, DigitSpec ds, u32 P, Opt1Spec o1) {
    typedef typename KeyT<W>::T Key;
    constexpr int KPT = Tile<W>::KPT;
    extern __shared__ __attribute__((aligned(16))) char smem[];
    Key* stage = reinterpret_cast<Key*>(smem);
    u32* cnt = reinterpret_cast<u32*>(smem + sizeof(Key) * Tile<W>::KEYS);
    u32* off = cnt + (P + 1);
    u32* cur = off + (P + 1);
    u32* delta = cur + P;
    u32* wsum = delta + P;
    u32* tot = wsum + 16;
    u32* lim = tot + 1;
    u64* lob = MODE == 4 ? reinterpret_cast<u64*>(smem + ((reinterpret_cast<char*>(lim + P) - smem + 7) & ~size_t(7))) : nullptr;
    const u32 nchunks = *d_nchunks;
    const u32 first = OPT ? blockIdx.x * o1.area : 0u;
    if (OPT && o1.uslice) for (u32 b = threadIdx.x; b < P; b += SC_NT) cur[b] = first + b * o1.uslice;
    else if (OPT && MODE == 4) for (u32 b = threadIdx.x; b < P; b += SC_NT) { const u32 sl = o1.boff[b]; cur[b] = blockIdx.x * sl; lim[b] = cur[b] + sl; lob[b] = o1.obase[b]; }
    else if (OPT) for (u32 b = threadIdx.x; b < P; b += SC_NT) { cur[b] = first + o1.boff[b]; lim[b] = first + o1.boff[b + 1]; }
    u32 gbeg = blockIdx.x, gend = nchunks;
    if constexpr (SRC == 2 && OPT) {
        if (o1.cur_state) { gbeg += o1.g0; gend = o1.g0 + o1.gn; }
        if (o1.resume) for (u32 b = threadIdx.x; b < P; b += SC_NT) cur[b] = o1.cur_state[(u64)blockIdx.x * P + b];
    }
    Key hvk[HV_KEYS]; u32 hc[HV_KEYS]; int nhk = 0;
    if constexpr (HEAVY) {
#pragma unroll
        for (int x = 0; x < HV_KEYS; ++x) { hvk[x] = reinterpret_cast<const Key*>(o1.hv_keys)[x]; hc[x] = 0; if (!is_empty_key(hvk[x])) nhk = x + 1; }
    }
    for (u32 g = gbeg; g < gend; g += gridDim.x) {
// ... 1488 lines not shown
__global__ __launch_bounds__(256) void k_enumerate(const u64* __restrict__ packed, const u32* __restrict__ inval,
                                                   u64 nwords, u64 nbytes, int k, u64* __restrict__ out, uint8_t* __restrict__ valid, int ow) {
    const u64 t = (u64)blockIdx.x * blockDim.x + threadIdx.x;
    const u64 wi = t >> 1;
    if (wi >= nwords) return;
    const int t0 = (int)(t & 1) * 16;
    u32 vm;
    if (W == 1) {
        u64 c[16];
        vm = gen_kmers1<16>(packed, inval, wi, t0, k, c);
        for (int j = 0; j < 16; ++j) {
            const u64 p = wi * 32 + t0 + j;
            if (p < nbytes) { const bool v = vm & (1u << j); out[p] = v ? c[j] : 0ull; valid[p] = v; }
        }
    } else {
        constexpr int WW = W > 1 ? W : 2;
        KN<WW> c[16];
        vm = gen_kmers_multi(packed, inval, wi, t0, k, c);
        for (int j = 0; j < 16; ++j) {
            const u64 p = wi * 32 + t0 + j;
            if (p < nbytes) {
                const bool v = vm & (1u << j);
                for (int x = 0; x < WW; ++x) if (x < ow) out[(u64)ow * p + x] = v ? c[j].w[x] : 0ull;
                valid[p] = v;
            }
        }
    }
}

__global__ __launch_bounds__(256) void k_minimizers(const u64* __restrict__ packed, const u32* __restrict__ inval,
                                                    u64 nwords, u64 nbytes, int k, int m,
                                                    u32* __restrict__ minim, uint8_t* __restrict__ valid) {
    const u64 t = (u64)blockIdx.x * blockDim.x + threadIdx.x;
    const u64 p0 = t * 16;
    if (p0 >= nbytes) return;
    const u32 mmask = (m == 16) ? 0xFFFFFFFFu : ((1u << (2 * m)) - 1);
    const int halo = k - 1;
    const long long s0 = (long long)p0 - halo;
    u32 cm[16 + 127];
    u32 f = 0, r = 0; int run = 0;
    int runs[16];
    for (int i = 0; i < halo + 16; ++i) {
        const long long pos = s0 + i;
        bool ok = false; u32 c = 0;
        if (pos >= 0 && (u64)pos < nbytes) {
            const u64 w = (u64)pos >> 5; const int j = (int)(pos & 31);
            ok = !((inval[w] >> (31 - j)) & 1u);
            c = (u32)(packed[w] >> (62 - 2 * j)) & 3u;
        }
        if (!ok) { run = 0; f = 0; r = 0; }
        else { f = ((f << 2) | c) & mmask; r = (r >> 2) | ((c ^ 2u) << (2 * (m - 1))); ++run; }
        cm[i] = f < r ? f : r;
        if (i >= halo) runs[i - halo] = run;
    }
    for (int j = 0; j < 16; ++j) {
        const u64 p = p0 + j;
        if (p >= nbytes) break;
        const bool v = runs[j] >= k;
        u32 best = 0xFFFFFFFFu;
        if (v) for (int e = halo + j - (k - m); e <= halo + j; ++e) best = cm[e] < best ? cm[e] : best;
        minim[p] = v ? best : 0u;
        valid[p] = v ? 1 : 0;
    }
}

struct MergeParams { u32 nbanks, kind, mask, amin, amax, hmax, want2d; };
#define MB_LH 256
#define MB_L2 32
template <int W>
__device__ __forceinline__ bool rows_same(const RowsIn& r, u64 a, u64 b) {
    bool e = true;
#pragma unroll
    for (int x = 0; x < W; ++x) e = e && (r.w[x][a] == r.w[x][b]);
    return e;
}
template <int W>
__global__ __launch_bounds__(256) void k_merge_banks(RowsIn rows, const u64* __restrict__ val,
                                                     u64 n, MergeParams mp, u32* __restrict__ flag, u32* __restrict__ sumv,
                                                     u64* __restrict__ ghist, u64* __restrict__ gh2d, u64* __restrict__ gstats) {
    __shared__ u32 lh[MB_LH];
    __shared__ u32 l2[MB_L2 * 11];
    for (int b = threadIdx.x; b < MB_LH; b += 256) lh[b] = 0;
    for (int b = threadIdx.x; b < MB_L2 * 11; b += 256) l2[b] = 0;
    __syncthreads();
    const u64 i = (u64)blockIdx.x * 256 + threadIdx.x;
    u32 ndist = 0;
    if (i < n) {
        const bool head = i == 0 || !rows_same<W>(rows, i - 1, i);
        u32 f = 0, sv = 0;
        if (head) {
            u64 sum = 0; u32 mx = 0, genome = 0, present = 0, inwin = 0, nonzero = 0, nb = 0; u32 mn = 0xFFFFFFFFu;
            for (u64 j = i; j < n && rows_same<W>(rows, i, j) && nb < mp.nbanks; ++j, ++nb) {
                const u64 v = val[j]; const u32 bank = (u32)(v >> 32), c = (u32)v;
                sum += c; mx = c > mx ? c : mx; mn = c < mn ? c : mn;
                if (bank == 0) genome = c;
                nonzero |= 1u << bank;
                if (c >= mp.amin) present |= 1u << bank;
                if (c >= mp.amin && c <= mp.amax) inwin |= 1u << bank;
            }
            if (nb < mp.nbanks) mn = 0;
            const u32 all = mp.nbanks >= 32 ? 0xFFFFFFFFu : ((1u << mp.nbanks) - 1);
            const u32 s32 = sum > 0xFFFFFFFFull ? 0xFFFFFFFFu : (u32)sum;
            bool solid;
            switch (mp.kind) {
                case 1: solid = mn >= mp.amin && mn <= mp.amax; break;
                case 2: solid = mx >= mp.amin && mx <= mp.amax; break;
                case 3: solid = inwin != 0; break;
                case 4: solid = inwin == all; break;
                case 5: solid = (present & mp.mask) == (mp.mask & all) && (nonzero & ~mp.mask) == 0; break;
                default: solid = s32 >= mp.amin && s32 <= mp.amax;
            }
            f = solid ? 1u : 0u; sv = s32; ndist = 1;
            const u32 hb = s32 < mp.hmax ? s32 : mp.hmax;
            if (hb < MB_LH) atomicAdd(&lh[hb], 1u); else atomicAdd(&ghist[hb], 1ull);
            if (mp.want2d) {
                const u64 reads = sum - genome;
                const u32 r = reads < mp.hmax ? (u32)reads : mp.hmax, gcol = genome < 10 ? genome : 10u;
                if (r < MB_L2) atomicAdd(&l2[r * 11 + gcol], 1u); else atomicAdd(&gh2d[(u64)r * 11 + gcol], 1ull);
            }
        }
        flag[i] = f; sumv[i] = sv;
    }
    for (int d = 32; d >= 1; d >>= 1) ndist += __shfl_down(ndist, d);
    if ((threadIdx.x & 63) == 0 && ndist) atomicAdd(&gstats[0], (u64)ndist);
    __syncthreads();
    for (int b = threadIdx.x; b < MB_LH; b += 256) if (lh[b]) atomicAdd(&ghist[b < (int)mp.hmax ? b : (int)mp.hmax], (u64)lh[b]);
    if (mp.want2d) for (int b = threadIdx.x; b < MB_L2 * 11; b += 256) if (l2[b]) atomicAdd(&gh2d[b], (u64)l2[b]);
}

template <int W>
__global__ __launch_bounds__(256) void k_pick_rows(RowsIn rows, const u32* __restrict__ sumv,
                                                   const u32* __restrict__ flag_in, const u32* __restrict__ posx, u64 n,
                                                   RowsOut out, u32* __restrict__ out_ab) {
    const u64 i = (u64)blockIdx.x * 256 + threadIdx.x;
    if (i >= n || !flag_in[i]) return;
    const u32 p = posx[i];
#pragma unroll
    for (int x = 0; x < W; ++x) out.w[x][p] = rows.w[x][i];
    out_ab[p] = sumv[i];
}
__global__ void k_pack_bank(u64* __restrict__ dst, const u32* __restrict__ ab, u64 n, u32 bank) {
    const u64 i = (u64)blockIdx.x * blockDim.x + threadIdx.x;
    if (i < n) dst[i] = ((u64)bank << 32) | ab[i];
}
__global__ __launch_bounds__(256) void k_bin_moments(const u32* __restrict__ matrix, u32 nch, u32 P, u64* __restrict__ mom) {
    const u32 b = blockIdx.x * 4 + (threadIdx.x >> 6), lane = threadIdx.x & 63;
    if (b >= P) return;
    u64 s = 0, q = 0;
    for (u32 c = lane; c < nch; c += 64) { const u64 x = matrix[(u64)b * nch + c]; s += x; q += x * x; }
#pragma unroll
    for (int d = 32; d >= 1; d >>= 1) { s += __shfl_down(s, d); q += __shfl_down(q, d); }
    if (lane == 0) { mom[2 * b] = s; mom[2 * b + 1] = q; }
}
#define HV_SLOTS 16
#define HV_COLLECT 2048
#define HV_BLOCK_KEYS 32
template <int W, int SRC, int MODE>
__global__ __launch_bounds__(SC_NT) void k_collect_heavy(const u64* __restrict__ packed, const u32* __restrict__ inval, const typename KeyT<W>::T* __restrict__ keys,
                                                         const ChunkDesc* __restrict__ descs, const u32* __restrict__ d_nchunks, int k, DigitSpec ds, u32 P,
                                                         const unsigned char* __restrict__ lut, u32* __restrict__ kept, typename KeyT<W>::T* __restrict__ out, const u32* __restrict__ keep_step) {
    typedef typename KeyT<W>::T Key;
    constexpr int KPT = Tile<W>::KPT;
    __shared__ unsigned char slut[MAX_BINS + 8];
    __shared__ u32 lcnt[HV_SLOTS], lstep[HV_SLOTS];
    const int lane = threadIdx.x & 63;
    for (u32 b = threadIdx.x; b < P; b += SC_NT) slut[b] = lut[b];
    if (threadIdx.x < HV_SLOTS) { const u32 st = keep_step[threadIdx.x]; lstep[threadIdx.x] = st; lcnt[threadIdx.x] = (blockIdx.x * 7919u) % st; }
    __syncthreads();
    const u32 nchunks = *d_nchunks;
    for (u32 g = blockIdx.x; g < nchunks; g += gridDim.x) {
        const ChunkDesc d = descs[g];
        const u64 step = SRC == 0 ? Tile<W>::WORDS : Tile<W>::KEYS;
        for (u64 t0 = d.begin; t0 < d.end; t0 += step) {
            Key h[KPT];
            u32 vm;
            if constexpr (SRC == 0) vm = tile_keys_reads(packed, inval, t0, d.end, k, h); else vm = tile_keys_array<W>(keys, t0, d.end, h);
#pragma unroll
            for (int j = 0; j < KPT; ++j) {
                u32 f = 0xFFu;
                if ((vm & (1u << j)) && key_in_pass<MODE>(digit_word(h[j]), ds)) f = slut[key_digit<MODE>(digit_word(h[j]), ds)];
                u64 todo = __ballot(f != 0xFFu);
                while (todo) {
                    const int lead = __ffsll((unsigned long long)todo) - 1;
                    const u32 fl = (u32)__shfl((int)f, lead);
                    const u64 grp = __ballot(f == fl);
                    u32 base = 0;
                    if (lane == lead) base = atomicAdd(&lcnt[fl], (u32)__popcll(grp));
                    base = (u32)__shfl((int)base, lead);
                    if (f == fl) {
                        const u32 idx = base + (u32)__popcll(grp & ((1ull << lane) - 1)), st = lstep[fl];
                        const u32 p0 = ((blockIdx.x * 7919u) % st + st - 1) / st;
                        if (idx % st == 0u && idx / st - p0 < HV_BLOCK_KEYS) out[((u64)fl * gridDim.x + blockIdx.x) * HV_BLOCK_KEYS + idx / st - p0] = h[j];
                    }
                    todo &= ~grp;
                }
            }
        }
    }
    __syncthreads();
    if (threadIdx.x < HV_SLOTS) {
        const u32 st = lstep[threadIdx.x];
        const u32 n = (lcnt[threadIdx.x] + st - 1) / st - ((blockIdx.x * 7919u) % st + st - 1) / st;
        kept[threadIdx.x * gridDim.x + blockIdx.x] = n < HV_BLOCK_KEYS ? n : HV_BLOCK_KEYS;
    }
}
template <int W>
__global__ void k_heavy_rows(const typename KeyT<W>::T* __restrict__ hv_keys, const unsigned long long* __restrict__ hv_cnt, u32 nslots, u32 amin, u32 amax, u32 histo_max,
                             u64* __restrict__ ghist, u64* __restrict__ gstats, u64* __restrict__ rows_k , u32* __restrict__ rows_ab) {
    const u32 i = blockIdx.x * blockDim.x + threadIdx.x;
    if (i >= nslots) return;
    const typename KeyT<W>::T key = hv_keys[i];
    const unsigned long long c64 = hv_cnt[i];
    if (is_empty_key(key) || c64 == 0ull) return;
    const u32 c = c64 > 0xFFFFFFFFull ? 0xFFFFFFFFu : (u32)c64;
    atomicAdd(&ghist[c < histo_max ? c : histo_max], 1ull);
    atomicAdd(&gstats[0], 1ull);
    atomicAdd(&gstats[2], c64);
    if (c >= amin && c <= amax) {
        const u64 at = atomicAdd(&gstats[1], 1ull);
        if constexpr (W == 1) rows_k[at] = kunmix(key);
        else {
            KN<W> kx = key; kunmixN(kx);
#pragma unroll
            for (int x = 0; x < W; ++x) rows_k[(u64)x * nslots + at] = kx.w[x];
        }
        rows_ab[at] = c;
    }
}
__global__ void k_copy_u32(u32* __restrict__ dst, const u32* __restrict__ src, u64 n) {
    const u64 i = (u64)blockIdx.x * blockDim.x + threadIdx.x;
    if (i < n) dst[i] = src[i];
}
```

Before: 26.97 billion.

## Plan level-1 bins on device and fuse sample, readback and descriptor uploads

Moves the level-1 partition planning to a device kernel that reads the valid-window count directly, so the level-1 positional sample histogram and its moments can run in the same round trip as the nvalid readback instead of needing a separate host sync. Level-1 and sample chunk descriptors are staged together in one pinned upload and reused when the host later asks for them. The stats gather kernel is folded into the scan-apply kernel, and level-2 segment descriptors are built and uploaded alongside the bin offsets. This adds state that must stay consistent between the device plan and the host plan, with a fallback that samples again when the two disagree.

```diff
diff --git a/dsk_amd/csrc/dskgpu.hip b/dsk_amd/csrc/dskgpu.hip
--- a/dsk_amd/csrc/dskgpu.hip
+++ b/dsk_amd/csrc/dskgpu.hip
@@ -74,12 +74,15 @@
 
 namespace {
 
-__global__ void k_gather_back(const u32* __restrict__ sc, const u32* __restrict__ nsolid_total, const u32* __restrict__ nk, const u64* __restrict__ gstats,
-                              u64* __restrict__ out) {
-    if (threadIdx.x == 0) {
-        out[0] = sc[SC_OVERFLOW]; out[1] = *nsolid_total; out[2] = nk ? *nk : 0u; out[3] = sc[SC_OVF2]; out[4] = sc[SC_OVF1]; out[5] = sc[SC_EXT];
-        out[6] = gstats[0]; out[7] = gstats[1]; out[8] = gstats[2]; out[9] = gstats[3];
-    }
+struct CountBack { const u32* sc; const u32* total; const u32* nk; const u64* gstats; u64* out; };
+__global__ __launch_bounds__(SCAN_NT) void k_scan_apply_back(u32* __restrict__ a, const u32* __restrict__ d_len,
+                                                             const u32* __restrict__ sums, CountBack cb) {
+    if (blockIdx.x == 0 && threadIdx.x == 0) {
+        u64* out = cb.out;
+        out[0] = cb.sc[SC_OVERFLOW]; out[1] = *cb.total; out[2] = cb.nk ? *cb.nk : 0u; out[3] = cb.sc[SC_OVF2]; out[4] = cb.sc[SC_OVF1]; out[5] = cb.sc[SC_EXT];
+        out[6] = cb.gstats[0]; out[7] = cb.gstats[1]; out[8] = cb.gstats[2]; out[9] = cb.gstats[3];
+    }
+    scan_apply_block(a, d_len, sums);
 }
 struct ScalarSet { u32 v[SC_COUNT]; };
 __global__ __launch_bounds__(256) void k_setup_pass(u32* __restrict__ sc, ScalarSet h, u64* __restrict__ ghist, u32 nh, u64* __restrict__ gstats, u32 nstats,
@@ -99,6 +102,17 @@
     if (bytes > LAND_BYTES) return nullptr;
     if (!ctx->land && hipHostMalloc(reinterpret_cast<void**>(&ctx->land), LAND_BYTES, hipHostMallocDefault) != hipSuccess) { ctx->land = nullptr; (void)hipGetLastError(); }
     return ctx->land;
+}
+
+char* upload_block(dskgpu_ctx* ctx, size_t bytes) {
+    if (bytes > ctx->up_pin_cap) {
+        if (ctx->up_pin) (void)hipHostFree(ctx->up_pin);
+        ctx->up_pin = nullptr; ctx->up_pin_cap = 0;
+        const size_t want = std::max<size_t>(bytes * 2, 128u << 10);
+        if (hipHostMalloc(reinterpret_cast<void**>(&ctx->up_pin), want, hipHostMallocDefault) != hipSuccess) { ctx->up_pin = nullptr; (void)hipGetLastError(); return nullptr; }
+        ctx->up_pin_cap = want;
+    }
+    return ctx->up_pin;
 }
 
 bool sentinel_is_a_kmer(int W, unsigned k) {
@@ -152,6 +166,15 @@
     hipLaunchKernelGGL(k_scan_reduce, dim3((unsigned)nb), dim3(SCAN_NT), 0, ctx->stream, a, d_len, ctx->sums.as<u32>());
     hipLaunchKernelGGL(k_scan_sums, dim3(1), dim3(1024), 0, ctx->stream, ctx->sums.as<u32>(), d_len, a);
     hipLaunchKernelGGL(k_scan_apply, dim3((unsigned)nb), dim3(SCAN_NT), 0, ctx->stream, a, d_len, ctx->sums.as<u32>());
+    CKL("k_scan");
+    return DSKGPU_OK;
+}
+int run_scan_back(dskgpu_ctx* ctx, u32* a, const u32* d_len, u64 max_len, const CountBack& cb) {
+    const u64 nb = std::max<u64>(1, (max_len + SCAN_BLK - 1) / SCAN_BLK);
+    CK(ctx->sums.ensure((nb + 1) * 4));
+    hipLaunchKernelGGL(k_scan_reduce, dim3((unsigned)nb), dim3(SCAN_NT), 0, ctx->stream, a, d_len, ctx->sums.as<u32>());
+    hipLaunchKernelGGL(k_scan_sums, dim3(1), dim3(1024), 0, ctx->stream, ctx->sums.as<u32>(), d_len, a);
+    hipLaunchKernelGGL(k_scan_apply_back, dim3((unsigned)nb), dim3(SCAN_NT), 0, ctx->stream, a, d_len, ctx->sums.as<u32>(), cb);
     CKL("k_scan");
     return DSKGPU_OK;
 }
@@ -281,11 +304,11 @@
 #define CH2 65536u
 #define OPT_GROUPS 545u
 #define OPT_GROUPS2 1023u
-inline u32 opt_groups(int W) { return W == 2 ? (AL_G2 == 8 ? 1022u : OPT_GROUPS2) : (W == 1 && AL_G1 == 16) ? 546u : W == 4 ? OPT_GROUPS4 : OPT_GROUPS; }
-inline u64 target_keys(int W) { return W == 1 ? TARGET_KEYS : W == 2 ? TARGET_KEYS2 : TARGET_KEYS4; }
+__host__ __device__ inline u32 opt_groups(int W) { return W == 2 ? (AL_G2 == 8 ? 1022u : OPT_GROUPS2) : (W == 1 && AL_G1 == 16) ? 546u : W == 4 ? OPT_GROUPS4 : OPT_GROUPS; }
+__host__ __device__ inline u64 target_keys(int W) { return W == 1 ? TARGET_KEYS : W == 2 ? TARGET_KEYS2 : TARGET_KEYS4; }
 #define OPT_CAP 4360u
 
-bool make_plan(u64 n_upper, int extra_bits, int W, u32 num_cu, Plan* pl) {
+__host__ __device__ bool make_plan(u64 n_upper, int extra_bits, int W, u32 num_cu, Plan* pl) {
     const u64 target = target_keys(W);
     u64 F = ((n_upper + target - 1) / target) << extra_bits;
     if (F < 2) F = 2;
@@ -295,7 +318,8 @@
         u64 p1 = 1; while (p1 * p1 < F) ++p1;
         const bool large = F >= (u64)num_cu * 64;
         if (large) {
-            p1 = std::max<u64>((F + p2max - 2) / (p2max - 1), num_cu);
+            p1 = (F + p2max - 2) / (p2max - 1);
+            if (p1 < num_cu) p1 = num_cu;
             p1 = (p1 + num_cu - 1) / num_cu * num_cu;
             if (p1 > MAX_LEVEL_BINS - 8) p1 = MAX_LEVEL_BINS - 8;
         }
@@ -308,6 +332,23 @@
     pl->d1 = DigitSpec{1u, pl->P1, 0u, 1u, 1u, 0u};
     pl->d2 = DigitSpec{2u, pl->P1, pl->P2, 1u, 1u, 0u};
     return true;
+}
+
+__global__ void k_plan_level1(const u64* __restrict__ nvalid_p, u64 n_upper, u64 max_keys, int W, u32 num_cu, u32 world, u32 max_bins, SamplePlan* __restrict__ sp) {
+    if (blockIdx.x || threadIdx.x) return;
+    const u64 nvalid = *nvalid_p;
+    SamplePlan o;
+    o.bins = 0; o.levels = 0; o.P2 = 0; o.pad = 0; o.d1 = DigitSpec{1u, 0u, 0u, world, 1u, 0u}; o.nvalid = nvalid;
+    const u64 n_keys = nvalid ? nvalid : 1;
+    if (n_keys <= max_keys && n_upper < 0xFFFF0000ull) {
+        const u64 plan_n = nvalid + 1 < n_upper ? nvalid + 1 : n_upper;
+        Plan pl;
+        if (make_plan(plan_n, 0, W, num_cu, &pl)) {
+            o.levels = (u32)pl.levels; o.P2 = pl.P2;
+            if (pl.levels == 2 && pl.P1 <= max_bins) { o.bins = pl.P1; o.d1.pa = pl.P1; }
+        }
+    }
+    *sp = o;
 }
 
 void build_descs1(dskgpu_ctx* ctx, u64 n_units_total, u64 tile, u64 max_chunks, u32* nch_out) {
@@ -440,11 +481,10 @@
     for (size_t f = 0; f < flagged.size(); ++f) ctx->h_hv_step[f] = (u32)std::max<u64>(1, ctx->h_mom[2 * (size_t)flagged[f]] / HV_COLLECT);
     CK(hipMemcpyAsync(ctx->hv_lut.p, ctx->h_hv_lut.data(), P1, hipMemcpyHostToDevice, ctx->stream));
     CK(hipMemcpyAsync(d_step, ctx->h_hv_step.data(), HV_SLOTS * 4, hipMemcpyHostToDevice, ctx->stream));
-    u32* sc = ctx->scalars.as<u32>();
     const bool mp = pl.d1.npass > 1;
     auto launch = [&](auto kern) {
         hipLaunchKernelGGL(kern, dim3(grid), dim3(SC_NT), 0, ctx->stream, (const u64*)ctx->packed.as<u64>(), (const u32*)ctx->inval.as<u32>(), d_keys_in,
-                           (const ChunkDesc*)ctx->smp_descs.as<ChunkDesc>(), (const u32*)(sc + SC_NCH_S), (int)ctx->cfg.kmer_size, pl.d1, P1,
+                           ctx->d_smp_descs, ctx->d_smp_nch, (int)ctx->cfg.kmer_size, pl.d1, P1,
                            (const unsigned char*)ctx->hv_lut.as<unsigned char>(), d_kept, ctx->hv_collect.as<Key>(), (const u32*)d_step);
     };
     if (from_reads) { if (mp) launch(k_collect_heavy<W, 0, 3>); else launch(k_collect_heavy<W, 0, 1>); }
@@ -514,7 +554,23 @@
     Key* solid_keys = nullptr; u32* solid_ab = nullptr;
     u32 flags = 0, nsolid = 0, nkeys = 0, ovf2 = 0, ovf1 = 0, ext = 0; u64 stats[4] = {0, 0, 0, 0};
     bool too_big = false; u64 rows = 0;
+    const ChunkDesc* d_descs2 = nullptr;
+    bool first_attempt = true;
 };
+
+void segment_descs(dskgpu_ctx* ctx, const Plan& pl, const std::vector<double>& load) {
+    ctx->h_descs2.resize(pl.P1);
+    std::vector<u32> order(pl.P1);
+    for (u32 sgm = 0; sgm < pl.P1; ++sgm) order[sgm] = sgm;
+    double mean_work = 0.0; for (double w : load) mean_work += w; mean_work = std::max(1.0, mean_work / pl.P1);
+    auto wclass = [&](u32 a) { return (long long)(load[a] / (0.05 * mean_work)); };
+    std::stable_sort(order.begin(), order.end(), [&](u32 a, u32 b) { return wclass(a) > wclass(b); });
+    for (u32 i = 0; i < pl.P1; ++i) {
+        const u32 sgm = order[i];
+        ChunkDesc d; d.begin = ctx->h_boff[sgm]; d.end = ctx->h_boff[sgm + 1]; d.flat_base = sgm * pl.P2; d.stride = 1;
+        ctx->h_descs2[i] = d;
+    }
+}
 
 template <int W>
 int upload_descs1(dskgpu_ctx* ctx, PassState<W>& ps) {
@@ -524,6 +580,9 @@
     else if (src.from_rec && ctx->rec_slice_end.size() > 1) build_descs1_slices(ctx, RecTile<W>::NR, max_chunks1, &ps.nch1);
     else if (src.from_rec) build_descs1(ctx, ctx->rec_n, RecTile<W>::NR, max_chunks1, &ps.nch1);
     else build_descs1(ctx, src.nkeys, Tile<W>::KEYS, max_chunks1, &ps.nch1);
+    const bool there = src.from_reads && ctx->pre_d1_words == src.nwords + 1 && ctx->pre_d1_nch == ps.nch1 && ctx->descs1.cap >= ctx->h_descs1.size() * sizeof(ChunkDesc);
+    ctx->pre_d1_words = 0;
+    if (there) return DSKGPU_OK;
     CK(ctx->descs1.ensure(ctx->h_descs1.size() * sizeof(ChunkDesc)));
     CK(hipMemcpyAsync(ctx->descs1.p, ctx->h_descs1.data(), ctx->h_descs1.size() * sizeof(ChunkDesc), hipMemcpyHostToDevice, ctx->stream));
     return DSKGPU_OK;
@@ -537,21 +596,32 @@
     return upload_descs1(ctx, ps);
 }
 
-template <class Hist>
-int positional_sample(dskgpu_ctx* ctx, u64 units, u64 tile, u32 P, Hist&& hist, u64* ntiles_out, u64* nts_out, u64* stot_out) {
-    u32* sc = ctx->scalars.as<u32>();
+void sample_descs(dskgpu_ctx* ctx, u64 units, u64 tile, u64* ntiles_out, u64* nts_out) {
     const u64 ntiles = std::max<u64>(1, (units + tile - 1) / tile);
     const u64 nts = std::min<u64>(ntiles, 1024);
-    ctx->h_descs_s.resize(nts);
+    ctx->h_descs_s.resize(nts + 1);
     for (u64 i = 0; i < nts; ++i) {
         const u64 t = i * ntiles / nts;
         ChunkDesc d; d.begin = t * tile; d.end = std::min<u64>(units, (t + 1) * tile); d.flat_base = (u32)i; d.stride = (u32)nts;
         ctx->h_descs_s[i] = d;
     }
+    ChunkDesc last; last.begin = nts; last.end = 0; last.flat_base = 0; last.stride = 0;
+    ctx->h_descs_s[nts] = last;
+    *ntiles_out = ntiles; *nts_out = nts;
+}
+
+template <class Hist>
+int positional_sample(dskgpu_ctx* ctx, u64 units, u64 tile, u32 P, Hist&& hist, u64* ntiles_out, u64* nts_out, u64* stot_out) {
+    u32* sc = ctx->scalars.as<u32>();
+    ctx->pre.valid = false;
+    u64 ntiles = 0, nts = 0;
+    sample_descs(ctx, units, tile, &ntiles, &nts);
+    ctx->d_smp_nch = sc + SC_NCH_S;
     const u64 Ms = (u64)P * nts;
     CK(ctx->smp_descs.ensure(nts * sizeof(ChunkDesc)));
     CK(ctx->smp_mat.ensure((Ms + 4) * 4 + (size_t)P * 16));
     CK(hipMemcpyAsync(ctx->smp_descs.p, ctx->h_descs_s.data(), nts * sizeof(ChunkDesc), hipMemcpyHostToDevice, ctx->stream));
+    ctx->d_smp_descs = ctx->smp_descs.as<ChunkDesc>();
     ctx->h_sc[SC_NCH_S] = (u32)nts;
     CK(hipMemcpyAsync(sc + SC_NCH_S, &ctx->h_sc[SC_NCH_S], 4, hipMemcpyHostToDevice, ctx->stream));
     { const int e = hist(ctx->smp_descs.as<ChunkDesc>(), (const u32*)(sc + SC_NCH_S), nts, ctx->smp_mat.as<u32>()); if (e) return e; }
@@ -566,6 +636,57 @@
     u64 stot = 0;
     for (u32 b = 0; b < P; ++b) stot += ctx->h_mom[2 * b];
     *ntiles_out = ntiles; *nts_out = nts; *stot_out = stot;
+    return DSKGPU_OK;
+}
+
+template <int W>
+int presample_level1(dskgpu_ctx* ctx, u64 nwords, u64 n_upper, u64 max_keys) {
+    ctx->pre = PreSample{};
+    const u64 units = nwords, tile = Tile<W>::WORDS;
+    u64 ntiles = 0, nts = 0;
+    sample_descs(ctx, units, tile, &ntiles, &nts);
+    u32 max_bins = MAX_LEVEL_BINS;
+    { Plan ub; if (make_plan(n_upper, 0, W, (u32)ctx->num_cu, &ub)) max_bins = ub.levels == 2 ? std::max<u32>(128u, ub.P1) : 128u; }
+    const size_t back_bytes = 64 + (size_t)max_bins * 16;
+    static_assert(sizeof(SamplePlan) <= 64, "read-back header");
+    void* lz = landing(ctx, back_bytes);
+    if (!lz) return fail(ctx, DSKGPU_E_NOMEM, "pinned landing zone of the sample");
+    u32 nch1 = 0;
+    build_descs1(ctx, nwords, Tile<W>::WORDS, (u64)ctx->num_cu * 8, &nch1);
+    const size_t up_bytes = ((size_t)nch1 + nts + 1) * sizeof(ChunkDesc);
+    if (!upload_block(ctx, up_bytes)) return fail(ctx, DSKGPU_E_NOMEM, "pinned staging of the level-1 chunks");
+    std::memcpy(ctx->up_pin, ctx->h_descs1.data(), (size_t)nch1 * sizeof(ChunkDesc));
+    std::memcpy(ctx->up_pin + (size_t)nch1 * sizeof(ChunkDesc), ctx->h_descs_s.data(), (nts + 1) * sizeof(ChunkDesc));
+    CK(ctx->descs1.ensure(up_bytes));
+    CK(ctx->smp_mat.ensure(((u64)max_bins * nts + 4) * 4 + (size_t)max_bins * 16));
+    CK(ctx->smp_back.ensure(back_bytes));
+    CK(hipMemcpyAsync(ctx->descs1.p, ctx->up_pin, up_bytes, hipMemcpyHostToDevice, ctx->stream));
+    ctx->d_smp_descs = ctx->descs1.as<ChunkDesc>() + nch1;
+    ctx->d_smp_nch = reinterpret_cast<const u32*>(ctx->d_smp_descs + nts);
+    ctx->pre_d1_words = nwords + 1; ctx->pre_d1_nch = nch1;
+    SamplePlan* d_sp = ctx->smp_back.as<SamplePlan>();
+    u64* d_mom = reinterpret_cast<u64*>(ctx->smp_back.as<char>() + 64);
+    hipLaunchKernelGGL(k_plan_level1, dim3(1), dim3(64), 0, ctx->stream, (const u64*)(ctx->gstats.as<u64>() + 3), n_upper, max_keys, W, (u32)ctx->num_cu,
+                       (u32)ctx->cfg.world_size, max_bins, d_sp);
+    CKL("k_plan_level1");
+    const unsigned grid = (unsigned)std::max<u64>(1, std::min<u64>(nts, (u64)ctx->num_cu));
+    hipLaunchKernelGGL((k_hist_planned<W, 0, 1>), dim3(grid), dim3(SC_NT), 0, ctx->stream, (const u64*)ctx->packed.as<u64>(), (const u32*)ctx->inval.as<u32>(),
+                       (const typename KeyT<W>::T*)nullptr, ctx->d_smp_descs, ctx->d_smp_nch, ctx->smp_mat.as<u32>(),
+                       (int)ctx->cfg.kmer_size, (const SamplePlan*)d_sp);
+    CKL("k_hist_planned");
+    hipLaunchKernelGGL(k_bin_moments_planned, dim3((max_bins + 3) / 4), dim3(256), 0, ctx->stream, (const u32*)ctx->smp_mat.as<u32>(), (u32)nts, (const SamplePlan*)d_sp, d_mom);
+    CKL("k_bin_moments_planned");
+    CK(hipMemcpyAsync(lz, ctx->smp_back.p, back_bytes, hipMemcpyDeviceToHost, ctx->stream));
+    CK(hipStreamSynchronize(ctx->stream));
+    SamplePlan sp;
+    std::memcpy(&sp, lz, sizeof sp);
+    ctx->h_nvalid = sp.nvalid;
+    if (sp.bins && sp.bins <= max_bins) {
+        ctx->h_mom.resize((size_t)sp.bins * 2);
+        std::memcpy(ctx->h_mom.data(), static_cast<const char*>(lz) + 64, (size_t)sp.bins * 16);
+        ctx->pre = PreSample{true, sp.bins, sp.d1.world, units, tile, ntiles, nts};
+    }
+    if (ctx->tune.verbose) fprintf(stderr, "[dskgpu] plan on the device: %llu valid windows, %u level(s), %u level-1 bins sampled\n", (unsigned long long)sp.nvalid, sp.levels, sp.bins);
     return DSKGPU_OK;
 }
 
@@ -610,6 +731,8 @@
     Opt1Spec& o1 = ps.o1;
     o1 = Opt1Spec{nullptr, 0u, 0u, ps.sc + SC_OVF1, nullptr, ctx->sk_sp.R, ctx->gstats.as<u64>() + 2, nullptr, nullptr, 0u, nullptr, 0ull, {0ull, 0ull, 0ull, 0ull}, 0u};
     const bool uniform1 = scatter_lds(W, pl.P1, true) > 160 * 1024;
+    const PreSample pre = ctx->pre;
+    ctx->pre.valid = false;
     if (ps.opt1) {
         const u32 nch1 = ps.nch1;
         const unsigned grid1 = ps.grid1 = scatter_grid(ctx, W, pl.P1, nch1, !uniform1);
@@ -662,7 +785,18 @@
                 return src.from_reads ? launch_hist<W, 0>(ctx, nullptr, dd, d_nch, n, mat, pl.d1, pl.P1) : launch_hist<W, 1>(ctx, d_keys_s, dd, d_nch, n, mat, pl.d1, pl.P1);
             };
             u64 ntiles = 0, nts = 0, stot = 0;
-            { const int e = positional_sample(ctx, units, tile, pl.P1, hist, &ntiles, &nts, &stot); if (e) return e; }
+            const bool planned = pre.valid && src.from_reads && ps.npass == 1 && pre.P == pl.P1 && pl.d1.mode == 1u && pl.d1.pa == pre.P && pl.d1.world == pre.world &&
+                                 pl.d1.npass == 1u && pl.d1.pass == 0u && pre.units == units && pre.tile == tile;
+            if (planned) {
+                ntiles = pre.ntiles; nts = pre.nts;
+                for (u32 b = 0; b < pl.P1; ++b) stot += ctx->h_mom[2 * b];
+            } else {
+                if (pre.valid && src.from_reads && ps.npass == 1 && ps.first_attempt) {
+                    if (ctx->tune.verbose || ctx->tune.plan_strict) fprintf(stderr, "[dskgpu] the device planned %u level-1 bins, the host %u: sampling again\n", pre.P, pl.P1);
+                    if (ctx->tune.plan_strict) return fail(ctx, DSKGPU_E_STATE, "the plan made on the device differs from the host's");
+                }
+                const int e = positional_sample(ctx, units, tile, pl.P1, hist, &ntiles, &nts, &stot); if (e) return e;
+            }
             if (stot >= (u64)pl.P1 * 64) {
                 const double scale = (src.from_reads && ps.npass > 1) ? (double)ntiles / (double)nts : pass_keys / (double)stot;
                 if (smp_rec) smp_density = std::max(0.05, (double)stot / ((double)nts * (double)Tile<W>::KEYS));
@@ -700,8 +834,19 @@
         if (area < 8 || area * grid1 + tail >= 0xFFFF0000ull) ps.opt1 = false;
         else {
             o1.area = (u32)area; o1.dump = (u32)(area * grid1);
-            CK(ctx->boff.ensure(((size_t)pl.P1 + 1) * 4));
-            CK(hipMemcpyAsync(ctx->boff.p, ctx->h_boff.data(), ((size_t)pl.P1 + 1) * 4, hipMemcpyHostToDevice, ctx->stream));
+            const bool with_d2 = pl.levels == 2 && ps.opt_cap && grid1 + 1 <= SLICED_MAX;
+            const size_t off_bytes = (((size_t)pl.P1 + 1) * 4 + 7) & ~size_t(7), d2_bytes = with_d2 ? (size_t)pl.P1 * sizeof(ChunkDesc) : 0;
+            if (with_d2) segment_descs(ctx, pl, ps.load);
+            CK(ctx->boff.ensure(off_bytes + d2_bytes));
+            if (char* up = upload_block(ctx, off_bytes + d2_bytes)) {
+                std::memcpy(up, ctx->h_boff.data(), ((size_t)pl.P1 + 1) * 4);
+                if (with_d2) std::memcpy(up + off_bytes, ctx->h_descs2.data(), d2_bytes);
+                CK(hipMemcpyAsync(ctx->boff.p, up, off_bytes + d2_bytes, hipMemcpyHostToDevice, ctx->stream));
+            } else {
+                CK(hipMemcpyAsync(ctx->boff.p, ctx->h_boff.data(), ((size_t)pl.P1 + 1) * 4, hipMemcpyHostToDevice, ctx->stream));
+                if (with_d2) CK(hipMemcpyAsync(ctx->boff.as<char>() + off_bytes, ctx->h_descs2.data(), d2_bytes, hipMemcpyHostToDevice, ctx->stream));
+            }
+            if (with_d2) ps.d_descs2 = reinterpret_cast<const ChunkDesc*>(ctx->boff.as<char>() + off_bytes);
             o1.boff = ctx->boff.as<u32>();
             CK(ctx->mat1.ensure((cells + 1) * 4));
             o1.fill = ctx->mat1.as<u32>();
@@ -812,18 +957,10 @@
         CK(ctx->seg.ensure((size_t)pl.P1 * sizeof(SegInfo)));
         CK(ctx->mat2.ensure(((size_t)ps.nregions + 1) * 4));
         CK(ctx->chain_next.ensure(((size_t)ps.nregions + 1 + ps.max_ext + 1) * 4));
-        if (ps.opt1) {
-            ctx->h_descs2.resize(pl.P1);
-            std::vector<u32> order(pl.P1);
-            for (u32 sgm = 0; sgm < pl.P1; ++sgm) order[sgm] = sgm;
-            double mean_work = 0.0; for (double w : ps.load) mean_work += w; mean_work = std::max(1.0, mean_work / pl.P1);
-            auto wclass = [&](u32 a) { return (long long)(ps.load[a] / (0.05 * mean_work)); };
-            std::stable_sort(order.begin(), order.end(), [&](u32 a, u32 b) { return wclass(a) > wclass(b); });
-            for (u32 i = 0; i < pl.P1; ++i) {
-                const u32 sgm = order[i];
-                ChunkDesc d; d.begin = ctx->h_boff[sgm]; d.end = ctx->h_boff[sgm + 1]; d.flat_base = sgm * pl.P2; d.stride = 1;
-                ctx->h_descs2[i] = d;
-            }
+        const ChunkDesc* dd2 = ctx->descs2.as<ChunkDesc>();
+        if (ps.opt1 && ps.d_descs2) dd2 = ps.d_descs2;
+        else if (ps.opt1) {
+            segment_descs(ctx, pl, ps.load);
             CK(hipMemcpyAsync(ctx->descs2.p, ctx->h_descs2.data(), (size_t)pl.P1 * sizeof(ChunkDesc), hipMemcpyHostToDevice, ctx->stream));
         } else {
             hipLaunchKernelGGL(k_plan, dim3(1), dim3(1024), 0, ctx->stream, ctx->mat1.as<u32>(), ps.nch1, pl.P1, 0x7FFFFFFFu, pl.P2,
@@ -835,7 +972,7 @@
                    pl.F, ps.max_ext, ctx->chain_next.as<u32>(), ps.sc + SC_EXT, ctx->chain_next.as<u32>() + ps.nregions + 1, ps.sc + SC_NCHAINED,
                    ps.sc + SC_WORK2, nullptr};
         if (ctx->tune.verbose && ps.opt1) { CK(ctx->dbg.ensure((size_t)pl.P1 * 24)); os.dbg = ctx->dbg.as<unsigned long long>(); }
-        if (ps.opt1) rc = launch_scatter_al<W, 2, true, true>(ctx, ctx->bufA.as<typename KeyT<W>::T>(), ctx->descs2.as<ChunkDesc>(), ps.sc + SC_NCH2, (u64)pl.P1 * 2, nullptr,
+        if (ps.opt1) rc = launch_scatter_al<W, 2, true, true>(ctx, ctx->bufA.as<typename KeyT<W>::T>(), dd2, ps.sc + SC_NCH2, (u64)pl.P1 * 2, nullptr,
                                                               ctx->bufB.as<typename KeyT<W>::T>(), pl.d2, pl.P2, os);
         else rc = launch_scatter_al<W, 2, true, false>(ctx, ctx->bufA.as<typename KeyT<W>::T>(), ctx->descs2.as<ChunkDesc>(), ps.sc + SC_NCH2, (u64)pl.P1 * 2, nullptr,
                                                        ctx->bufB.as<typename KeyT<W>::T>(), pl.d2, pl.P2, os);
@@ -910,14 +1047,12 @@
         }
     }
     ctx->mark("count");
-    if (int e = run_scan(ctx, ctx->nsolid.as<u32>(), ps.sc + SC_F, pl.F)) return e;
-    ctx->mark("scan_solid");
     CK(ctx->back_dev.ensure(16 * 8));
     if (!ctx->back_host) CK(hipHostMalloc(reinterpret_cast<void**>(&ctx->back_host), 16 * 8, hipHostMallocDefault));
     const u32* nkp = ps.opt1 ? nullptr : (ps.opt_cap ? ctx->mat1.as<u32>() + (u64)pl.P1 * ps.nch1 : ctx->fstart.as<u32>() + pl.F);
-    hipLaunchKernelGGL(k_gather_back, dim3(1), dim3(64), 0, ctx->stream, (const u32*)ps.sc, (const u32*)(ctx->nsolid.as<u32>() + pl.F), nkp,
-                       (const u64*)ctx->gstats.as<u64>(), ctx->back_dev.as<u64>());
-    CKL("k_gather_back");
+    const CountBack cb{(const u32*)ps.sc, (const u32*)(ctx->nsolid.as<u32>() + pl.F), nkp, (const u64*)ctx->gstats.as<u64>(), ctx->back_dev.as<u64>()};
+    if (int e = run_scan_back(ctx, ctx->nsolid.as<u32>(), ps.sc + SC_F, pl.F, cb)) return e;
+    ctx->mark("scan_solid");
     CK(hipMemcpyAsync(ctx->back_host, ctx->back_dev.p, 10 * 8, hipMemcpyDeviceToHost, ctx->stream));
     CK(hipStreamSynchronize(ctx->stream));
     const u64* bh = ctx->back_host;
@@ -1033,8 +1168,10 @@
     KeySource<W> src{from_reads, !from_reads && d_keys_in == nullptr, d_keys_in, nkeys_in, nwords};
     const u64 nvalid = from_reads ? ctx->h_nvalid : nkeys_in;
     int extra_bits = 0, table_retries = 0;
+    int attempt = 0;
     for (;;) {
         PassState<W> ps{src, pass, npass, cap, nvalid, ctx->scalars.as<u32>()};
+        ps.first_attempt = attempt++ == 0;
         int e;
         if ((e = pass_plan<W>(ctx, ps, extra_bits)) || (e = pass_layout1<W>(ctx, ps)) || (e = pass_scatter1<W>(ctx, ps))) return e;
         if (ps.too_big) { ctx->resolve_marks(); res->too_big = true; res->keys_seen = ps.nkeys; return DSKGPU_OK; }
@@ -1246,12 +1383,16 @@
     CK(ctx->ghist.ensure(((size_t)ctx->cfg.histo_max + 1 + 2) * 8));
     CK(ctx->gstats.ensure(4 * 8));
     ctx->have_nvalid = false;
+    ctx->pre = PreSample{}; ctx->pre_d1_words = 0;
     if (from_reads && nwords) {
         CK(hipMemsetAsync(ctx->gstats.p, 0, 4 * 8, ctx->stream));
         hipLaunchKernelGGL(k_count_valid, dim3((unsigned)std::min<u64>((nwords + 255) / 256, (u64)ctx->num_cu * 8)), dim3(256), 0, ctx->stream,
                            ctx->inval.as<u32>(), nwords, (int)ctx->cfg.kmer_size, ctx->gstats.as<u64>() + 3);
         CKL("k_count_valid");
-        {
+        const u64 max_keys1 = ctx->max_keys_per_pass ? ctx->max_keys_per_pass : 0xD0000000ull;
+        const bool presample = !ctx->tune.no_sample && !ctx->tune.no_opt1 && !ctx->tune.no_opt2 && !ctx->tune.no_presample && !ctx->opt1_off && !ctx->opt2_off && ctx->sentinel_ok && landing(ctx, 8);
+        if (presample) { if (const int rc = presample_level1<W>(ctx, nwords, n_upper, max_keys1)) return rc; }
+        else {
             void* lz = landing(ctx, 8);
             CK(hipMemcpyAsync(lz ? lz : (void*)&ctx->h_nvalid, ctx->gstats.as<u64>() + 3, 8, hipMemcpyDeviceToHost, ctx->stream));
             CK(hipStreamSynchronize(ctx->stream));
@@ -1915,7 +2056,7 @@
     (void)hipSetDevice(ctx->cfg.device);
     (void)hipStreamSynchronize(ctx->stream);
     DevBuf* bufs[] = {&ctx->reads_own, &ctx->raw_in, &ctx->raw_blk, &ctx->raw_boff, &ctx->raw_bstate, &ctx->raw_state, &ctx->packed, &ctx->inval, &ctx->bufA, &ctx->bufB, &ctx->mat1, &ctx->mat2, &ctx->sums,
-                      &ctx->descs1, &ctx->descs2, &ctx->seg, &ctx->fstart, &ctx->nsolid, &ctx->scalars, &ctx->ghist, &ctx->gstats, &ctx->chain_next, &ctx->smp_mat, &ctx->smp_descs, &ctx->boff, &ctx->hv_lut, &ctx->hv_collect, &ctx->hv_buf, &ctx->dbg, &ctx->l0buf,
+                      &ctx->descs1, &ctx->descs2, &ctx->seg, &ctx->fstart, &ctx->nsolid, &ctx->scalars, &ctx->ghist, &ctx->gstats, &ctx->chain_next, &ctx->smp_mat, &ctx->smp_descs, &ctx->smp_back, &ctx->boff, &ctx->hv_lut, &ctx->hv_collect, &ctx->hv_buf, &ctx->dbg, &ctx->l0buf,
                       &ctx->out_ab, &ctx->srt_ab, &ctx->srt_tmp,
                       &ctx->srt_idx, &ctx->srt_idx2, &ctx->srt_k, &ctx->srt_k2, &ctx->abund2, &ctx->acc_ab, &ctx->u_val,
                       &ctx->s_val, &ctx->m_flag, &ctx->m_pos, &ctx->m_sum, &ctx->gh2d,
@@ -1925,6 +2066,7 @@
     ctx->query.release();
     ctx->unitigs.release();
     if (ctx->land) (void)hipHostFree(ctx->land);
+    if (ctx->up_pin) (void)hipHostFree(ctx->up_pin);
     for (DevBuf* b : bufs) b->release();
     for (int i = 0; i < 4; ++i) { ctx->out_w[i].release(); ctx->srt_w[i].release(); ctx->acc_w[i].release(); ctx->u_w[i].release(); ctx->s_w[i].release(); }
     for (hipEvent_t e : ctx->ev_pool) (void)hipEventDestroy(e);
diff --git a/dsk_amd/csrc/engine.h b/dsk_amd/csrc/engine.h
--- a/dsk_amd/csrc/engine.h
+++ b/dsk_amd/csrc/engine.h
@@ -62,6 +62,8 @@
     bool l0_keys = false;
     u32 mp_pass_mkeys = 0;
     u64 rs_slab_rows = 0;
+    bool no_presample = false;
+    bool plan_strict = false;
     bool unitig_stages = false;
     void read() {
         auto on = [](const char* n) { return getenv(n) != nullptr; };
@@ -76,6 +78,7 @@
         no_sample = on("DSKGPU_NO_SAMPLE"); no_heavy = on("DSKGPU_NO_HEAVY"); verbose = on("DSKGPU_VERBOSE"); no_level0 = on("DSKGPU_NO_LEVEL0"); l0_passes = (u32)num("DSKGPU_L0_PASSES", 0); mp_pass_mkeys = (u32)num("DSKGPU_MP_PASS_MKEYS", 0); rs_max_rows = num("DSKGPU_RS_MAX_ROWS", 0); l0_keys = on("DSKGPU_L0_KEYS"); sk_generic = on("DSKGPU_SK_GENERIC"); ps_maxc = (u32)num("DSKGPU_PS_MAXC", 0);
         rs_slab_rows = num("DSKGPU_RS_SLAB_ROWS", 0);
         unitig_stages = on("DSKGPU_UNITIG_STAGES");
+        no_presample = on("DSKGPU_NO_PRESAMPLE"); plan_strict = on("DSKGPU_PLAN_STRICT");
         rs_block_rows = (u32)num("DSKGPU_RS_BLOCK_ROWS", 0); rs_bbits = (u32)num("DSKGPU_RS_BBITS", 0); rs_heavy = (u32)num("DSKGPU_RS_HEAVY", 0);
     }
 };
@@ -131,6 +134,8 @@
     void release() { for (DevBuf* b : {&unitig, &pos, &offsets, &ab_sum, &kind}) b->release(); stats = dskgpu_unitig_stats{}; valid = false; release_edges(); }
 };
 
+struct PreSample { bool valid = false; u32 P = 0, world = 0; u64 units = 0, tile = 0, ntiles = 0, nts = 0; };
+
 struct BankJob { dskgpu_config cfg; const uint8_t* base; u64 total; std::vector<u64> ends; u64 nu, tot_kmers; u32 passes, retries; bool active = false; };
 
 struct dskgpu_ctx {
@@ -155,6 +160,10 @@
     DevBuf mat1, mat2, sums, descs1, descs2, seg, fstart, nsolid, scalars, ghist, gstats, chain_next;
     RowSort rs;
     DevBuf smp_keys;
+    DevBuf smp_back; PreSample pre;
+    const ChunkDesc* d_smp_descs = nullptr; const u32* d_smp_nch = nullptr;
+    char* up_pin = nullptr; size_t up_pin_cap = 0;
+    u64 pre_d1_words = 0; u32 pre_d1_nch = 0;
     DevBuf smp_mat, smp_descs, boff;
     DevBuf dbg, l0buf; DevBuf hv_lut, hv_collect, hv_buf;
     std::vector<unsigned char> h_hv_lut; std::vector<u32> h_hv_cnt, h_hv_step; std::vector<u64> h_hv_coll, h_hv_keys;
diff --git a/dsk_amd/csrc/kernels.h b/dsk_amd/csrc/kernels.h
--- a/dsk_amd/csrc/kernels.h
+++ b/dsk_amd/csrc/kernels.h
@@ -139,10 +139,10 @@
 }
 
 template <int W, int SRC, int MODE>
-__global__ __launch_bounds__(SC_NT) void k_hist(const u64* __restrict__ packed, const u32* __restrict__ inval,
-                                                const typename KeyT<W>::T* __restrict__ keys,
-                                                const ChunkDesc* __restrict__ descs, const u32* __restrict__ d_nchunks,
-                                                u32* __restrict__ matrix, int k, DigitSpec ds, u32 P) {
+__device__ __forceinline__ void hist_chunks(const u64* __restrict__ packed, const u32* __restrict__ inval,
+                                            const typename KeyT<W>::T* __restrict__ keys,
+                                            const ChunkDesc* __restrict__ descs, const u32* __restrict__ d_nchunks,
+                                            u32* __restrict__ matrix, int k, const DigitSpec& ds, u32 P) {
     __shared__ u32 lh[MAX_BINS + 1];
     constexpr int KPT = Tile<W>::KPT;
     const u32 nchunks = *d_nchunks;
@@ -180,6 +180,24 @@
         for (u32 b = threadIdx.x; b < P; b += SC_NT) matrix[d.flat_base + (u64)b * d.stride] = lh[b];
         __syncthreads();
     }
+}
+template <int W, int SRC, int MODE>
+__global__ __launch_bounds__(SC_NT) void k_hist(const u64* __restrict__ packed, const u32* __restrict__ inval,
+                                                const typename KeyT<W>::T* __restrict__ keys,
+                                                const ChunkDesc* __restrict__ descs, const u32* __restrict__ d_nchunks,
+                                                u32* __restrict__ matrix, int k, DigitSpec ds, u32 P) {
+    hist_chunks<W, SRC, MODE>(packed, inval, keys, descs, d_nchunks, matrix, k, ds, P);
+}
+struct SamplePlan { u32 bins, levels, P2, pad; DigitSpec d1; u64 nvalid; };
+template <int W, int SRC, int MODE>
+__global__ __launch_bounds__(SC_NT) void k_hist_planned(const u64* __restrict__ packed, const u32* __restrict__ inval,
+                                                        const typename KeyT<W>::T* __restrict__ keys,
+                                                        const ChunkDesc* __restrict__ descs, const u32* __restrict__ d_nchunks,
+                                                        u32* __restrict__ matrix, int k, const SamplePlan* __restrict__ sp) {
+    const u32 P = sp->bins;
+    if (P == 0 || P > MAX_BINS) return;
+    const DigitSpec ds = sp->d1;
+    hist_chunks<W, SRC, MODE>(packed, inval, keys, descs, d_nchunks, matrix, k, ds, P);
 }
 
 #define SCAN_NT 256
@@ -238,8 +256,7 @@
     if (threadIdx.x == 0) a[len] = carry_s;
 }
 
-__global__ __launch_bounds__(SCAN_NT) void k_scan_apply(u32* __restrict__ a, const u32* __restrict__ d_len,
-                                                        const u32* __restrict__ sums) {
+__device__ __forceinline__ void scan_apply_block(u32* __restrict__ a, const u32* __restrict__ d_len, const u32* __restrict__ sums) {
     __shared__ u32 ws[SCAN_NT / 64];
     const u64 len = *d_len;
     const u64 b0 = (u64)blockIdx.x * SCAN_BLK;
@@ -259,6 +276,10 @@
     u32 run = sums[blockIdx.x] + wpre + y - s;
 #pragma unroll
     for (int j = 0; j < SCAN_IPT; ++j) { if (i0 + j < len) a[i0 + j] = run; run += v[j]; }
+}
+__global__ __launch_bounds__(SCAN_NT) void k_scan_apply(u32* __restrict__ a, const u32* __restrict__ d_len,
+                                                        const u32* __restrict__ sums) {
+    scan_apply_block(a, d_len, sums);
 }
 
 
@@ -2053,6 +2074,15 @@
     for (int d = 32; d >= 1; d >>= 1) { s += __shfl_down(s, d); q += __shfl_down(q, d); }
     if (lane == 0) { mom[2 * b] = s; mom[2 * b + 1] = q; }
 }
+__global__ __launch_bounds__(256) void k_bin_moments_planned(const u32* __restrict__ matrix, u32 nch, const SamplePlan* __restrict__ sp, u64* __restrict__ mom) {
+    const u32 b = blockIdx.x * 4 + (threadIdx.x >> 6), lane = threadIdx.x & 63;
+    if (b >= sp->bins) return;
+    u64 s = 0, q = 0;
+    for (u32 c = lane; c < nch; c += 64) { const u64 x = matrix[(u64)b * nch + c]; s += x; q += x * x; }
+#pragma unroll
+    for (int d = 32; d >= 1; d >>= 1) { s += __shfl_down(s, d); q += __shfl_down(q, d); }
+    if (lane == 0) { mom[2 * b] = s; mom[2 * b + 1] = q; }
+}
 #define HV_SLOTS 16
 #define HV_COLLECT 2048
 #define HV_BLOCK_KEYS 32
```

Result: slower. 26.03 billion (-3.5%).
